# ChantalMP/RaDialog

Measured on AMD Instinct MI355X. Metric: reports_per_sec (448px CXR encode + 160-tok prefill + 256-tok greedy decode), higher is better.
Workload: dtype bf16; 1 GPU; configs[1]: per-GPU batch 1 BioViL-T(ResNet-50)+Q-Former encode 448px, Vicuna-7B prefill T=160, 256-token greedy decode (LoRA r=8 un-merged, hipGraph ; per_gpu_batch=1, global_batch=1, prompt_len=160, parallelism=dp1

## Files before the change

### include/rdx_hooks.h

```cpp
#ifndef RDX_HOOKS_H
#define RDX_HOOKS_H
#include "rdx.h"
#ifdef __cplusplus
extern "C" {
#endif

int rdx_attn_trace(rdx_ctx* ctx, int layer, long long* host);
int rdx_quant_test(rdx_ctx* ctx, const void* X, int M, int K, int groups, int mode, const void* norm_w, float eps, void* out8, float* scales);
int rdx_gemv_trace(rdx_ctx* ctx, int what, int layer, long long* host, int max_tiles);

int rdx_gemm_test(rdx_ctx* ctx, const void* X, const float* W, const float* bias, const void* resid, void* out, int M, int N,
                  int K, int epi, const void* norm_w, float eps, int force);

int rdx_kernel_bench(rdx_ctx* ctx, int rows, int N, int K, int H, int ksize, int stride, int epi, int iters, float* ms_host,
                     long long* trace_host , int trace_wgs);

int rdx_conv_test(rdx_ctx* ctx, const void* X, const float* W, const float* bias, const void* resid, void* out, int B, int H, int Cin, int Cout,
                  int ksize, int stride, int epi, int path, int iters, float* ms_host);

int rdx_l2_bench(rdx_ctx* ctx, int mode, long long bytes_per_wg, int shared, int reps, int wgs, float* gbps_host);

int rdx_logits_test(rdx_ctx* ctx, const void* X, const float* W, int M, int N, int n_valid, int K, void* out_logits,
                    int32_t* argmax_host, int fp8);

#ifdef __cplusplus
}
#endif
#endif
```

### radialog_amd/_lib.py

```python
from __future__ import annotations

import ctypes as C
import os

import torch

HERE = os.path.dirname(os.path.abspath(__file__))
LIB_PATH = os.environ.get("RDX_LIB_PATH") or os.path.join(HERE, "librdx.so")
HOOKS_PATH = os.environ.get("RDX_HOOKS_PATH") or os.path.join(HERE, "librdx_hooks.so")

RDX_DTYPE_F16, RDX_DTYPE_BF16 = 0, 1
RDX_W_GEMM, RDX_W_TENSOR, RDX_W_F32, RDX_W_GEMM_FP8 = 0, 1, 2, 3
RDX_SRC_F32, RDX_SRC_F16, RDX_SRC_BF16 = 0, 1, 2


class RdxLibraryError(RuntimeError):
    pass


class RdxError(RuntimeError):
    pass


class RdxLogitsRules(C.Structure):
    _fields_ = [("repetition_penalty", C.c_float), ("no_repeat_ngram_size", C.c_int), ("min_new_tokens", C.c_int)]


class RdxConfig(C.Structure):
    _fields_ = [
        ("dtype", C.c_int),
        ("vocab", C.c_int), ("hidden", C.c_int), ("inter", C.c_int), ("layers", C.c_int), ("heads", C.c_int),
        ("max_pos", C.c_int),
        ("rms_eps", C.c_float),
        ("lora_r", C.c_int), ("lora_scale", C.c_float),
        ("qformer_dim", C.c_int),
        ("q_hidden", C.c_int), ("q_layers", C.c_int), ("q_heads", C.c_int), ("q_inter", C.c_int),
        ("q_enc_width", C.c_int), ("q_nquery", C.c_int), ("q_cross_freq", C.c_int),
        ("q_ln_eps", C.c_float),
        ("v_img", C.c_int), ("v_stem", C.c_int), ("v_planes", C.c_int * 4), ("v_blocks", C.c_int * 4),
        ("v_b2v", C.c_int), ("v_proj", C.c_int),
        ("v_ln_eps", C.c_float),
        ("max_batch", C.c_int), ("max_len", C.c_int),
        ("enable_vision", C.c_int), ("enable_llama", C.c_int),
        ("enable_cls", C.c_int), ("cls_hidden", C.c_int), ("cls_classes", C.c_int), ("cls_pool", C.c_int),
    ]


_P = C.c_void_p
SYMBOLS = {
    "rdx_create": (C.c_int, [C.POINTER(_P), C.c_int, C.POINTER(RdxConfig)]),
    "rdx_destroy": (None, [_P]),
    "rdx_last_error": (C.c_char_p, [_P]),
    "rdx_build_hash": (C.c_char_p, []),
    "rdx_sync": (C.c_int, [_P]),
    "rdx_stream": (_P, [_P]),
    "rdx_set_weight": (C.c_int, [_P, C.c_char_p, _P, C.c_int64, C.c_int64, C.c_int]),
    "rdx_set_weight_typed": (C.c_int, [_P, C.c_char_p, _P, C.c_int, C.c_int64, C.c_int64, C.c_int]),
    "rdx_finalize_weights": (C.c_int, [_P]),
    "rdx_transform_image": (C.c_int, [_P, _P, C.c_int, C.c_int, C.c_int, C.c_int, _P]),
    "rdx_encode_image": (C.c_int, [_P, _P, C.c_int, _P, _P]),
    "rdx_encode_image2": (C.c_int, [_P, _P, _P, C.c_int, _P, _P]),
    "rdx_classify_findings": (C.c_int, [_P, _P, C.c_int, _P]),
    "rdx_generate": (C.c_int, [_P, _P, _P, C.c_int, C.c_int, _P, C.c_int, C.c_int, C.c_int, _P, _P,
                               C.POINTER(C.c_int), C.c_int]),
    "rdx_prefill": (C.c_int, [_P, _P, _P, C.c_int, C.c_int, _P, C.c_int, C.c_int, C.c_int, _P, _P]),
    "rdx_decode_step": (C.c_int, [_P, _P]),
    "rdx_decode_step_ids": (C.c_int, [_P, _P, _P]),
    "rdx_set_logits_rules": (C.c_int, [_P, C.POINTER(RdxLogitsRules)]),
    "rdx_prefill_append": (C.c_int, [_P, _P, C.c_int, C.c_int, C.c_int, C.c_int, C.c_int, C.c_int, _P, _P]),
    "rdx_generate_append": (C.c_int, [_P, _P, C.c_int, C.c_int, C.c_int, C.c_int, C.c_int, C.c_int, _P, _P,
                                      C.POINTER(C.c_int), C.c_int]),
    "rdx_beam_search": (C.c_int, [_P, _P, _P, C.c_int, C.c_int, C.c_int, _P, C.c_int, C.c_int, C.c_int, C.c_float, C.c_int, _P, _P, _P, _P,
                                  C.POINTER(C.c_int)]),
    "rdx_comm_unique_id": (C.c_int, [_P]),
    "rdx_comm_init": (C.c_int, [_P, _P, C.c_int, C.c_int]),
    "rdx_allgather_tokens": (C.c_int, [_P, _P, _P, C.c_int, C.c_int]),
    "rdx_comm_world": (C.c_int, [_P]),
    "rdx_kv_read": (C.c_int, [_P, C.c_int, C.c_int, _P]),
    "rdx_hidden_read": (C.c_int, [_P, _P]),
    "rdx_time": (C.c_int, [_P, C.c_int, C.c_int, C.POINTER(C.c_float)]),
    "rdx_set_option": (C.c_int, [_P, C.c_char_p, C.c_int]),
}

HOOK_SYMBOLS = {
    "rdx_attn_trace": (C.c_int, [_P, C.c_int, _P]),
    "rdx_quant_test": (C.c_int, [_P, _P, C.c_int, C.c_int, C.c_int, C.c_int, _P, C.c_float, _P, _P]),
    "rdx_gemv_trace": (C.c_int, [_P, C.c_int, C.c_int, _P, C.c_int]),
    "rdx_gemm_test": (C.c_int, [_P, _P, _P, _P, _P, _P, C.c_int, C.c_int, C.c_int, C.c_int, _P, C.c_float, C.c_int]),
    "rdx_kernel_bench": (C.c_int, [_P, C.c_int, C.c_int, C.c_int, C.c_int, C.c_int, C.c_int, C.c_int, C.c_int, C.POINTER(C.c_float), _P, C.c_int]),
    "rdx_conv_test": (C.c_int, [_P, _P, _P, _P, _P, _P, C.c_int, C.c_int, C.c_int, C.c_int, C.c_int, C.c_int, C.c_int, C.c_int, C.c_int, C.POINTER(C.c_float)]),
    "rdx_l2_bench": (C.c_int, [_P, C.c_int, C.c_longlong, C.c_int, C.c_int, C.c_int, C.POINTER(C.c_float)]),
    "rdx_logits_test": (C.c_int, [_P, _P, _P, C.c_int, C.c_int, C.c_int, C.c_int, _P, _P, C.c_int]),
}

ENC_HOOK_SYMBOLS = {
    "rdx_stem_test": (C.c_int, [_P, _P, _P, _P, _P, C.c_int, C.c_int, C.c_int, C.c_int]),
    "rdx_norm_test": (C.c_int, [_P, C.c_int, _P, _P, _P, _P, _P, _P, C.c_int, C.c_int, C.c_longlong, C.c_longlong, C.c_int, C.c_int, C.c_float]),
    "rdx_attn_test": (C.c_int, [_P, _P, _P, _P, _P, _P, C.c_int, C.c_int, C.c_int, C.c_int, C.c_int, C.c_int, _P, C.c_longlong, C.c_int, C.c_int]),
}

_F = C.c_float
DEC_HOOK_SYMBOLS = {
    "rdx_xstat16_test": (C.c_int, [_P, _P, _P, _F, _P, C.c_int, C.c_int, C.c_int, C.c_int, _P, C.c_int, C.c_int, _P]),
    "rdx_xrow16_test": (C.c_int, [_P, _P, C.c_int, _P, _P, C.c_int, C.c_int, C.c_int, _P, C.c_int]),
    "rdx_xstat_blk_test": (C.c_int, [_P, _P, _P, _F, _P, _P, C.c_int, C.c_int, C.c_int, C.c_int, _P, C.c_int, C.c_int, _P, _P]),
    "rdx_xsplit_blk_test": (C.c_int, [_P, _P, _P, _P, _P, _F, C.c_int, C.c_int, _P, _P]),
    "rdx_xstat_blk8_test": (C.c_int, [_P, _P, _P, _F, _P, C.c_int, C.c_int, C.c_int, C.c_int, _P, C.c_int, C.c_int, _P, _P, _P]),
    "rdx_xsplit_blk8_test": (C.c_int, [_P, _P, _P, _P, _P, _F, C.c_int, C.c_int, C.c_int, _P, _P, _P]),
    "rdx_rmsnorm_test": (C.c_int, [_P, _P, _P, _F, C.c_int, C.c_int, C.c_int, C.c_int, _P, C.c_int, _P, C.c_longlong, _P, C.c_int]),
    "rdx_select_test": (C.c_int, [_P, _P, C.c_int, C.c_int, _P, _P, _P, C.c_int, C.POINTER(RdxLogitsRules), C.c_int, _P]),
}
ALL_HOOK_SYMBOLS = {**HOOK_SYMBOLS, **ENC_HOOK_SYMBOLS, **DEC_HOOK_SYMBOLS}

_lib = None
_hooks = None


def hooks_enabled() -> bool:
    return os.environ.get("RDX_DEBUG_HOOKS", "0") not in ("", "0")


def _missing_hook(name):
    def raiser(*_a, **_k):
        raise RdxLibraryError(f"{name} is a kernel-test hook of librdx_hooks.so (include/rdx_hooks.h, rdx_enc_hooks.h, rdx_dec_hooks.h), not part of the product library: "
                              "set RDX_DEBUG_HOOKS=1 before radialog_amd is loaded (tests/conftest.py and the tools/ scripts do)")
    return raiser


def load_hooks(lib):
    global _hooks
    if not hooks_enabled():
        for name in ALL_HOOK_SYMBOLS:
            setattr(lib, name, _missing_hook(name))
        return
    src = lib
    if not hasattr(lib, next(iter(HOOK_SYMBOLS))):
        if os.environ.get("RDX_LIB_PATH") and os.path.realpath(LIB_PATH) != os.path.realpath(os.path.join(HERE, "librdx.so")):
            raise RdxLibraryError(f"RDX_DEBUG_HOOKS is set, but RDX_LIB_PATH={LIB_PATH} does not link the hooks in and {HOOKS_PATH} would load a "
                                  "second librdx.so next to it: build the alternative library with api_debug.hip (tools/sanitize_host.sh does)")
        if not os.path.exists(HOOKS_PATH):
            raise RdxLibraryError(f"RDX_DEBUG_HOOKS is set but {HOOKS_PATH} is missing: build it with `python -m radialog_amd.build`")
        try:
            src = C.CDLL(HOOKS_PATH, mode=C.RTLD_GLOBAL)
        except OSError as e:
            raise RdxLibraryError(f"cannot load {HOOKS_PATH}: {e}") from e
        _hooks = src
    for name, (res, args) in ALL_HOOK_SYMBOLS.items():
        try:
            fn = getattr(src, name)
        except AttributeError as e:
            raise RdxLibraryError(f"{HOOKS_PATH} does not export {name}") from e
        fn.restype = res
        fn.argtypes = args
        if src is not lib:
            setattr(lib, name, fn)


def load():
    global _lib
    if _lib is not None:
        return _lib
    if not os.path.exists(LIB_PATH):
        raise RdxLibraryError(
            f"{LIB_PATH} not found: build it with `python -m radialog_amd.build` (hipcc, gfx950). "
            "There is no CPU fallback for the RaDialog hot path.")
    try:
        lib = C.CDLL(LIB_PATH, mode=C.RTLD_GLOBAL if hooks_enabled() else C.RTLD_LOCAL)
    except OSError as e:
        raise RdxLibraryError(f"cannot load {LIB_PATH}: {e}") from e
    for name, (res, args) in SYMBOLS.items():
        try:
            fn = getattr(lib, name)
        except AttributeError as e:
            raise RdxLibraryError(f"{LIB_PATH} does not export {name}") from e
        fn.restype = res
        fn.argtypes = args
    check_build_hash(lib)
    load_hooks(lib)
    _lib = lib
    return lib


def build_hash() -> str:
    return load().rdx_build_hash().decode()


def check_build_hash(lib):
    from . import build as _b
    try:
        want = _b.source_hash()
    except OSError:
        return
    got = lib.rdx_build_hash().decode()
    if got != want:
        msg = (f"{LIB_PATH} was built from sources with hash {got}, the tree's radialog_amd/csrc hashes to {want}: the library is stale -- "
               "rebuild it with `python -m radialog_amd.build`")
        if os.environ.get("RDX_ALLOW_STALE_LIB", "0") not in ("", "0"):
            import warnings
            warnings.warn(msg)
        else:
            raise RdxLibraryError(msg)


def check(ctx, rc: int, what: str):
    if rc != 0:
        msg = load().rdx_last_error(ctx)
        raise RdxError(f"{what} failed ({rc}): {msg.decode() if msg else '?'}")
```

### radialog_amd/csrc/api.hip

```cpp
#include "rdx_ctx.h"

static std::string g_create_err;

int fail(rdx_ctx* c, int code, const char* fmt, ...) {
    char buf[512];
    va_list ap;
    va_start(ap, fmt);
    vsnprintf(buf, sizeof(buf), fmt, ap);
    va_end(ap);
    if (c) c->err = buf; else g_create_err = buf;
    return code;
}

const char* create_error() { return g_create_err.c_str(); }

int dalloc(rdx_ctx* c, void** p, size_t bytes) {
    if (bytes == 0) bytes = 16;
    hipError_t e = hipMalloc(p, bytes);
    if (e != hipSuccess) return fail(c, -3, "hipMalloc(%zu bytes) failed: %s", bytes, hipGetErrorString(e));
    c->allocs.push_back(*p);
    return 0;
}

extern "C" int rdx_create(rdx_ctx** out, int device_id, const rdx_config* cfg) {
    if (!out || !cfg) return fail(nullptr, -1, "rdx_create: null argument");
    if (cfg->dtype != RDX_DTYPE_F16 && cfg->dtype != RDX_DTYPE_BF16) return fail(nullptr, -1, "rdx_create: bad dtype %d", cfg->dtype);
    int ndev = 0;
    hipError_t e = hipGetDeviceCount(&ndev);
    if (e != hipSuccess || ndev <= 0) return fail(nullptr, -2, "rdx_create: no HIP device (%s)", hipGetErrorString(e));
    if (device_id < 0 || device_id >= ndev) return fail(nullptr, -1, "rdx_create: device %d out of range (%d devices)", device_id, ndev);
    if (cfg->enable_llama) {
        if (cfg->hidden % cfg->heads || cfg->hidden / cfg->heads != 128)
            return fail(nullptr, -1, "rdx_create: Llama head_dim must be 128 (hidden %d / heads %d)", cfg->hidden, cfg->heads);
        if (cfg->hidden % 32 || cfg->inter % 32 || cfg->inter % 8 || cfg->qformer_dim % 32)
            return fail(nullptr, -1, "rdx_create: hidden/inter/qformer_dim must be multiples of 32");
        if (cfg->max_len % 32 || cfg->max_len <= 0 || cfg->max_len > 1536)
            return fail(nullptr, -1, "rdx_create: max_len must be a multiple of 32 in (0, 1536]");
        if (cfg->max_batch <= 0 || cfg->max_batch > RDX_MAX_ROWS) return fail(nullptr, -1, "rdx_create: max_batch must be in [1, %d]", RDX_MAX_ROWS);
        if (cfg->lora_r != 0 && cfg->lora_r != 8) return fail(nullptr, -1, "rdx_create: lora_r must be 0 or 8");
    }
    if (cfg->enable_vision) {
        if (cfg->q_hidden / cfg->q_heads != 64 || cfg->q_hidden % cfg->q_heads)
            return fail(nullptr, -1, "rdx_create: Q-Former head_dim must be 64");
    }
    if (cfg->enable_vision || cfg->enable_cls) {
        if (cfg->v_img % 4 || cfg->v_img < 32) return fail(nullptr, -1, "rdx_create: image size must be a multiple of 4, >= 32");
    }
    if (cfg->enable_cls) {
        if (cfg->enable_vision) return fail(nullptr, -1, "rdx_create: a classifier context has enable_vision = 0 (its projector differs)");
        if (cfg->cls_pool <= 0 || cfg->cls_hidden % 32 || cfg->cls_classes <= 0 || cfg->cls_classes > 16)
            return fail(nullptr, -1, "rdx_create: classifier needs pool > 0, hidden %% 32 == 0, 1..16 classes");
    }
    rdx_ctx* c = new rdx_ctx();
    c->cfg = *cfg;
    c->device = device_id;
    if (const char* e = getenv("RDX_FUSE_AO")) c->fuse_attn_oproj = atoi(e) != 0;
    if (const char* e = getenv("RDX_CHAIN")) c->chain_mlp = atoi(e) != 0;
    if (hipSetDevice(device_id) != hipSuccess || hipStreamCreateWithFlags(&c->stream, hipStreamNonBlocking) != hipSuccess) {
        delete c;
        return fail(nullptr, -2, "rdx_create: cannot create stream on device %d", device_id);
    }
    { const char* e = getenv("RDX_FLASH_MIN"); if (e) c->flash_min = atoi(e); }
    { const char* e = getenv("RDX_XS16"); if (e) c->xs16 = atoi(e) != 0; }
    { const char* e = getenv("RDX_PBLK"); if (e) c->prompt_blk = atoi(e) != 0; }
    { const char* e = getenv("RDX_BLK_DOWN"); c->blk_down = !(e && atoi(e) == 0); }
    { const char* e = getenv("RDX_PCONV_KSPLIT"); c->pconv_noks = e && atoi(e) == 0; }
    { const char* e = getenv("RDX_PCONV"); c->trunk_packed = !(e && atoi(e) == 0); }
    if (hipMalloc(&c->zero16, 64) == hipSuccess) { hipMemset(c->zero16, 0, 64); c->allocs.push_back(c->zero16); } else c->zero16 = nullptr;
    c->gemm_ws_floats = (size_t)16 << 20;
    if (hipMalloc((void**)&c->gemm_ws, c->gemm_ws_floats * sizeof(float)) != hipSuccess) { c->gemm_ws = nullptr; c->gemm_ws_floats = 0; }
    else c->allocs.push_back(c->gemm_ws);
    *out = c;
    return 0;
}

void rdx_comm_release(rdx_ctx* c);

extern "C" void rdx_destroy(rdx_ctx* c) {
    if (!c) return;
    hipSetDevice(c->device);
    hipStreamSynchronize(c->stream);
    rdx_comm_release(c);
    if (c->graph) hipGraphExecDestroy(c->graph);
    for (void* p : c->allocs) hipFree(p);
    hipStreamDestroy(c->stream);
    delete c;
}

extern "C" const char* rdx_last_error(rdx_ctx* c) { return c ? c->err.c_str() : g_create_err.c_str(); }

#ifndef RDX_BUILD_HASH
#define RDX_BUILD_HASH "unstamped"
#endif
extern "C" const char* rdx_build_hash(void) { return RDX_BUILD_HASH; }

extern "C" int rdx_sync(rdx_ctx* c) {
    if (!c) return -1;
    HIPCHK(c, hipStreamSynchronize(c->stream));
    HIPCHK(c, hipGetLastError());
    return 0;
}

extern "C" void* rdx_stream(rdx_ctx* c) { return c ? (void*)c->stream : nullptr; }

extern "C" int rdx_set_weight(rdx_ctx* c, const char* name, const float* data, int64_t rows, int64_t cols, int kind) {
    if (!c || !name || !data) return fail(c, -1, "rdx_set_weight: null argument");
    if (c->finalized) return fail(c, -1, "rdx_set_weight(%s): weights already finalized", name);
    if (rows <= 0 || cols <= 0) return fail(c, -1, "rdx_set_weight(%s): bad shape [%lld,%lld]", name, (long long)rows, (long long)cols);
    HIPCHK(c, hipSetDevice(c->device));
    const std::string key(name);
    if (kind == RDX_W_GEMM) {
        if (cols % 32) return fail(c, -1, "rdx_set_weight(%s): GEMM K=%lld must be a multiple of 32", name, (long long)cols);
        if (c->gemm.count(key)) return fail(c, -1, "rdx_set_weight(%s): duplicate", name);
        GemmW w;
        w.N = (int)rows; w.K = (int)cols; w.Npad = (int)((rows + 15) / 16 * 16);
        ALLOC(c, w.w, (size_t)w.Npad * w.K * esz(c));
        launch_pack_weight(c->cfg.dtype, data, w.w, w.N, w.K, w.Npad, nullptr, c->stream);
        c->gemm[key] = w;
    } else if (kind == RDX_W_GEMM_FP8) {
        if (cols % 64) return fail(c, -1, "rdx_set_weight(%s): fp8 GEMM K=%lld must be a multiple of 64", name, (long long)cols);
        if (c->gemm.count(key)) return fail(c, -1, "rdx_set_weight(%s): duplicate", name);
        GemmW w;
        w.N = (int)rows; w.K = (int)cols; w.Npad = (int)((rows + 15) / 16 * 16);
        ALLOC(c, w.w8, (size_t)w.Npad * w.K);
        ALLOC(c, w.scale, (size_t)w.Npad * sizeof(float));
        launch_pack_weight_fp8(c->cfg.dtype, data, w.w8, w.scale, nullptr, w.N, w.K, w.Npad, c->stream);
        c->gemm[key] = w;
    } else if (kind == RDX_W_TENSOR) {
        if (c->tens.count(key)) return fail(c, -1, "rdx_set_weight(%s): duplicate", name);
        RawW r; r.rows = rows; r.cols = cols;
        ALLOC(c, r.p, (size_t)rows * cols * esz(c) + 16);
        launch_from_f32(c->cfg.dtype, data, r.p, (size_t)rows * cols, c->stream);
        c->tens[key] = r;
    } else if (kind == RDX_W_F32) {
        if (c->f32.count(key)) return fail(c, -1, "rdx_set_weight(%s): duplicate", name);
        RawW r; r.rows = rows; r.cols = cols;
        ALLOC(c, r.p, (size_t)rows * cols * sizeof(float));
        HIPCHK(c, hipMemcpyAsync(r.p, data, (size_t)rows * cols * sizeof(float), hipMemcpyDeviceToDevice, c->stream));
        c->f32[key] = r;
    } else {
        return fail(c, -1, "rdx_set_weight(%s): unknown kind %d", name, kind);
    }
    HIPCHK(c, hipStreamSynchronize(c->stream));
    HIPCHK(c, hipGetLastError());
    return 0;
}

extern "C" int rdx_set_weight_typed(rdx_ctx* c, const char* name, const void* data, int src_dtype, int64_t rows, int64_t cols, int kind) {
    if (src_dtype == RDX_SRC_F32) return rdx_set_weight(c, name, (const float*)data, rows, cols, kind);
    if (!c || !name || !data) return fail(c, -1, "rdx_set_weight_typed: null argument");
    if (src_dtype != RDX_SRC_F16 && src_dtype != RDX_SRC_BF16) return fail(c, -1, "rdx_set_weight_typed(%s): unknown source dtype %d", name, src_dtype);
    if (rows <= 0 || cols <= 0) return fail(c, -1, "rdx_set_weight_typed(%s): bad shape [%lld,%lld]", name, (long long)rows, (long long)cols);
    HIPCHK(c, hipSetDevice(c->device));
    float* wide = nullptr;
    const size_t n = (size_t)rows * cols;
    hipError_t e = hipMalloc((void**)&wide, n * sizeof(float));
    if (e != hipSuccess) return fail(c, -3, "rdx_set_weight_typed(%s): hipMalloc(%zu bytes) failed: %s", name, n * sizeof(float), hipGetErrorString(e));
    launch_to_f32(src_dtype == RDX_SRC_F16 ? DT_F16 : DT_BF16, data, wide, n, c->stream);
    const int rc = rdx_set_weight(c, name, wide, rows, cols, kind);
    hipFree(wide);
    return rc;
}

namespace {
struct Resolver {
    rdx_ctx* c;
    int rc = 0;
    GemmW g(const std::string& n, int N, int K) {
        auto it = c->gemm.find(n);
        if (it == c->gemm.end()) { if (!rc) rc = fail(c, -4, "missing GEMM weight '%s'", n.c_str()); return GemmW(); }
        if (it->second.N != N || it->second.K != K) {
            if (!rc) rc = fail(c, -4, "weight '%s' has shape [%d,%d], expected [%d,%d]", n.c_str(), it->second.N, it->second.K, N, K);
        }
        return it->second;
    }
    const void* t(const std::string& n, int64_t elems) {
        auto it = c->tens.find(n);
        if (it == c->tens.end()) { if (!rc) rc = fail(c, -4, "missing tensor '%s'", n.c_str()); return nullptr; }
        if (it->second.rows * it->second.cols != elems) { if (!rc) rc = fail(c, -4, "tensor '%s' has %lld elements, expected %lld", n.c_str(), (long long)(it->second.rows * it->second.cols), (long long)elems); }
        return it->second.p;
    }
    const float* f(const std::string& n, int64_t elems) {
        auto it = c->f32.find(n);
        if (it == c->f32.end()) { if (!rc) rc = fail(c, -4, "missing fp32 tensor '%s'", n.c_str()); return nullptr; }
        if (it->second.rows * it->second.cols != elems) { if (!rc) rc = fail(c, -4, "fp32 tensor '%s' has %lld elements, expected %lld", n.c_str(), (long long)(it->second.rows * it->second.cols), (long long)elems); }
        return (const float*)it->second.p;
    }
};
std::string S(const char* fmt, ...) {
    char buf[128];
    va_list ap; va_start(ap, fmt); vsnprintf(buf, sizeof(buf), fmt, ap); va_end(ap);
    return buf;
}
}

extern "C" int rdx_finalize_weights(rdx_ctx* c) {
    if (!c) return -1;
    if (c->finalized) return fail(c, -1, "rdx_finalize_weights: already finalized");
    HIPCHK(c, hipSetDevice(c->device));
    const rdx_config& f = c->cfg;
    Resolver R{c};
    if (f.enable_llama) {
        const int H = f.hidden, I = f.inter, r2 = 2 * f.lora_r;
        c->embed = R.t("embed", (int64_t)f.vocab * H);
        c->final_norm = R.t("final_norm", H);
        c->rope_cos = R.t("rope.cos", (int64_t)f.max_pos * 128);
        c->rope_sin = R.t("rope.sin", (int64_t)f.max_pos * 128);
        c->lm_head = R.g("lm_head", f.vocab, H);
        c->img_proj_w = R.g("img_proj.w", H, f.qformer_dim);
        c->img_proj_b = R.f("img_proj.b", H);
        c->ll.resize(f.layers);
        for (int l = 0; l < f.layers; ++l) {
            LlamaLayer& L = c->ll[l];
            L.attn_norm = R.t(S("l%d.attn_norm", l), H);
            L.mlp_norm = R.t(S("l%d.mlp_norm", l), H);
            L.wqkv = R.g(S("l%d.wqkv", l), 3 * H + r2, H);
            L.wo = R.g(S("l%d.wo", l), H, H);
            L.wgu = R.g(S("l%d.wgu", l), 2 * I, H);
            L.wdown = R.g(S("l%d.wdown", l), H, I);
            L.lora_bq = L.lora_bv = nullptr;
            if (f.lora_r) {
                L.lora_bq = R.t(S("l%d.lora_bq", l), (int64_t)H * f.lora_r);
                L.lora_bv = R.t(S("l%d.lora_bv", l), (int64_t)H * f.lora_r);
            }
        }
        if (R.rc) return R.rc;
        c->ld.hidden = H; c->ld.heads = f.heads; c->ld.head_dim = 128; c->ld.qkv_ld = c->ll[0].wqkv.Npad;
        c->ld.lora_r = f.lora_r; c->ld.lora_scale = f.lora_scale; c->ld.max_len = f.max_len; c->ld.max_pos = f.max_pos;
        c->ld.k_perm = (getenv("RDX_KPERM") ? atoi(getenv("RDX_KPERM")) : (f.max_batch * f.heads <= 256)) ? 1 : 0;
        const int B = f.max_batch;
        c->kv_layer_elems = (size_t)B * f.heads * f.max_len * 128;
        ALLOC(c, c->kcache, c->kv_layer_elems * f.layers * 2);
        ALLOC(c, c->vcache, c->kv_layer_elems * f.layers * 2);
        HIPCHK(c, hipMemset(c->kcache, 0, c->kv_layer_elems * f.layers * 2));
        HIPCHK(c, hipMemset(c->vcache, 0, c->kv_layer_elems * f.layers * 2));
        ALLOC(c, c->key_mask, (size_t)B * f.max_len);
        HIPCHK(c, hipMemset(c->key_mask, 0, (size_t)B * f.max_len));
        ALLOC(c, c->d_img_pos, B * sizeof(int)); ALLOC(c, c->d_pos, B * sizeof(int)); ALLOC(c, c->d_slot, B * sizeof(int));
        ALLOC(c, c->d_step, B * sizeof(int)); ALLOC(c, c->d_unf, B * sizeof(int));
        ALLOC(c, c->d_ctr, ((size_t)f.layers * 256 + chain_ctr_ints(f.layers)) * sizeof(int)); ALLOC(c, c->d_err, sizeof(int));
        HIPCHK(c, hipMemset(c->d_ctr, 0, ((size_t)f.layers * 256 + chain_ctr_ints(f.layers)) * sizeof(int)));
        c->d_cctr = c->d_ctr + (size_t)f.layers * 256;
        HIPCHK(c, hipMemset(c->d_err, 0, sizeof(int)));
        {
            std::vector<ChainLayer> cl(f.layers);
            for (int l = 0; l < f.layers; ++l) {
                const LlamaLayer& L = c->ll[l];
                cl[l] = ChainLayer{L.wqkv.w, L.wdown.w, L.attn_norm, L.wqkv.w8, L.wdown.w8, L.wqkv.scale, L.wdown.scale};
            }
            ALLOC(c, c->d_clayers, cl.size() * sizeof(ChainLayer));
            HIPCHK(c, hipMemcpy(c->d_clayers, cl.data(), cl.size() * sizeof(ChainLayer), hipMemcpyHostToDevice));
        }
        ALLOC(c, c->d_cur_rope, (size_t)B * 256 * 2);
        ALLOC(c, c->d_pos_ids, (size_t)B * f.max_len * sizeof(int));
        c->n_vtiles = c->lm_head.Npad / 16;
        ALLOC(c, c->part_val, (size_t)B * c->n_vtiles * sizeof(float));
        ALLOC(c, c->part_idx, (size_t)B * c->n_vtiles * sizeof(int));
        const int Bp = B > 2 ? (B + 31) / 32 * 32 : B;
        ALLOC(c, c->dx, (size_t)B * H * 2); ALLOC(c, c->dxn, (size_t)Bp * H * 2);
        if (B > 2) ALLOC(c, c->kslab, (size_t)4 * Bp * H * sizeof(float));
        ALLOC(c, c->dqkv, (size_t)B * c->ld.qkv_ld * 2);
        ALLOC(c, c->dxs, (size_t)std::max(32, Bp) * sizeof(float));
        ALLOC(c, c->datt, (size_t)Bp * H * 2); ALLOC(c, c->dgu, (size_t)Bp * I * 2);
        ALLOC(c, c->pqe, (size_t)B * 32 * f.qformer_dim * 2); ALLOC(c, c->pimg, (size_t)B * 32 * H * 2);
        if (B > 32 && !blk64_ok(c, B))
            return fail(c, -1, "rdx_finalize_weights: max_batch %d > 32 needs the Vicuna-7B widths (hidden 4096, inter 11008: the row-block decode family, model-dtype "
                               "or fp8 weights); this model (hidden %d, inter %d) holds at most 32 rows per context", B, H, I);
    }
    if (f.enable_vision) {
        const int H = f.q_hidden, I = f.q_inter;
        c->q_query_ln = R.t("q.query_ln", (int64_t)f.q_nquery * H);
        c->n_cross = 0;
        c->ql.resize(f.q_layers);
        for (int l = 0; l < f.q_layers; ++l) {
            QLayer& L = c->ql[l];
            L.s_wqkv = R.g(S("q%d.self.wqkv", l), 3 * H, H); L.s_bqkv = R.f(S("q%d.self.bqkv", l), 3 * H);
            L.s_wo = R.g(S("q%d.self.wo", l), H, H); L.s_bo = R.f(S("q%d.self.bo", l), H);
            L.s_g = R.f(S("q%d.self.ln_g", l), H); L.s_b = R.f(S("q%d.self.ln_b", l), H);
            L.cross_idx = -1;
            if (l % f.q_cross_freq == 0) {
                L.cross_idx = c->n_cross++;
                L.c_wq = R.g(S("q%d.cross.wq", l), H, H); L.c_bq = R.f(S("q%d.cross.bq", l), H);
                L.c_wo = R.g(S("q%d.cross.wo", l), H, H); L.c_bo = R.f(S("q%d.cross.bo", l), H);
                L.c_g = R.f(S("q%d.cross.ln_g", l), H); L.c_b = R.f(S("q%d.cross.ln_b", l), H);
            }
            L.w1 = R.g(S("q%d.ffn.w1", l), I, H); L.b1 = R.f(S("q%d.ffn.b1", l), I);
            L.w2 = R.g(S("q%d.ffn.w2", l), H, I); L.b2 = R.f(S("q%d.ffn.b2", l), H);
            L.f_g = R.f(S("q%d.ffn.ln_g", l), H); L.f_b = R.f(S("q%d.ffn.ln_b", l), H);
        }
        c->q_wkv = R.g("q.cross.wkv", c->n_cross * 2 * H, f.q_enc_width);
        c->q_bkv = R.f("q.cross.bkv", (int64_t)c->n_cross * 2 * H);
    }
    if (f.enable_vision || f.enable_cls) {
        c->v_conv1 = R.g("v.conv1.w", f.v_stem, 7 * 8 * 4); c->v_conv1_b = R.f("v.conv1.b", f.v_stem);
        int cin = f.v_stem;
        for (int li = 0; li < 4; ++li) {
            for (int b = 0; b < f.v_blocks[li]; ++b) {
                VBlock vb;
                vb.planes = f.v_planes[li];
                vb.stride = (b == 0 && li > 0) ? 2 : 1;
                vb.has_ds = (b == 0);
                const std::string p = S("v.l%d.%d.", li + 1, b);
                vb.c1 = R.g(p + "c1.w", vb.planes, cin); vb.b1 = R.f(p + "c1.b", vb.planes);
                vb.c2 = R.g(p + "c2.w", vb.planes, 9 * vb.planes); vb.b2 = R.f(p + "c2.b", vb.planes);
                vb.c3 = R.g(p + "c3.w", 4 * vb.planes, vb.planes); vb.b3 = R.f(p + "c3.b", 4 * vb.planes);
                vb.bds = nullptr;
                if (vb.has_ds) { vb.ds = R.g(p + "ds.w", 4 * vb.planes, cin); vb.bds = R.f(p + "ds.b", 4 * vb.planes); }
                cin = 4 * vb.planes;
                c->vb.push_back(vb);
            }
        }
        c->v_b2v = R.g("v.b2v.w", f.v_b2v, cin);
        c->v_p1 = R.g("v.proj1.w", f.v_proj, f.v_b2v); c->v_p1_b = R.f("v.proj1.b", f.v_proj);
        c->v_p2 = R.g("v.proj2.w", f.v_proj, f.v_proj); c->v_p2_b = R.f("v.proj2.b", f.v_proj);
    }
    if (f.enable_cls) {
        const int gp = v_grid(f) / f.cls_pool;
        if (gp <= 0 || (f.v_proj * gp * gp) % 32) return fail(c, -1, "classifier: pooled feature width %d must be a positive multiple of 32", f.v_proj * gp * gp);
        c->cls_fc1 = R.g("cls.fc1.w", f.cls_hidden, f.v_proj * gp * gp); c->cls_fc1_b = R.f("cls.fc1.b", f.cls_hidden);
        c->cls_fc2 = R.g("cls.fc2.w", f.cls_classes, f.cls_hidden); c->cls_fc2_b = R.f("cls.fc2.b", f.cls_classes);
    }
    if (f.enable_vision) {
        c->v_ln_g = R.f("v.ln.g", f.v_proj); c->v_ln_b = R.f("v.ln.b", f.v_proj);
        if (f.q_enc_width != f.v_proj) return fail(c, -1, "q_enc_width %d != v_proj %d", f.q_enc_width, f.v_proj);
        if (c->tens.count("v.pool.emb")) {
            const int Cv = f.v_b2v, Pn = v_grid(f) * v_grid(f);
            if (Cv % 32) return fail(c, -1, "ViT pooler needs b2v %% 32 == 0");
            c->pool_emb = R.t("v.pool.emb", (int64_t)2 * Pn * Cv);
            c->pool_ng = R.f("v.pool.norm_g", Cv); c->pool_nb = R.f("v.pool.norm_b", Cv);
            c->v_p1f = R.g("v.proj1f.w", f.v_proj, 2 * Cv); c->v_p1f_b = R.f("v.proj1f.b", f.v_proj);
            for (int i = 0; c->gemm.count(S("v.pool.%d.wqkv", i)); ++i) {
                PoolBlock pb;
                const std::string p = S("v.pool.%d.", i);
                pb.n1_g = R.f(p + "n1_g", Cv); pb.n1_b = R.f(p + "n1_b", Cv); pb.n2_g = R.f(p + "n2_g", Cv); pb.n2_b = R.f(p + "n2_b", Cv);
                pb.wqkv = R.g(p + "wqkv", 3 * Cv, Cv);
                pb.wo = R.g(p + "wo", Cv, Cv); pb.bo = R.f(p + "bo", Cv);
                pb.w1 = R.g(p + "w1", Cv, Cv); pb.b1 = R.f(p + "b1", Cv);
                pb.w2 = R.g(p + "w2", Cv, Cv); pb.b2 = R.f(p + "b2", Cv);
                c->pool.push_back(pb);
            }
        }
    }
    if (R.rc) return R.rc;
    c->finalized = true;
    return 0;
}

extern "C" int rdx_set_option(rdx_ctx* c, const char* name, int value) {
    if (!c || !name) return -1;
    if (!strcmp(name, "flash_min")) { c->flash_min = value; return 0; }
    if (!strcmp(name, "pconv")) { c->trunk_packed = value != 0; return 0; }
    if (!strcmp(name, "prompt_blk")) { c->prompt_blk = value != 0; return 0; }
    if (!strcmp(name, "xs16")) {
        c->xs16 = value != 0;
        if (c->graph) { hipGraphExecDestroy(c->graph); c->graph = nullptr; c->gkey = GraphKey(); }
        return 0;
    }
    return fail(c, -1, "rdx_set_option: unknown option '%s'", name);
}
```

### radialog_amd/csrc/api_debug.hip

```cpp
#include "rdx_ctx.h"
#include "../../include/rdx_hooks.h"
#include "../../include/rdx_enc_hooks.h"

extern "C" int rdx_attn_trace(rdx_ctx* c, int layer, long long* host) {
    if (!c || !c->finalized || c->cur_B <= 0 || !host) return fail(c, -1, "rdx_attn_trace: run a prefill first");
    HIPCHK(c, hipSetDevice(c->device));
    long long* dtr = nullptr;
    HIPCHK(c, hipMalloc(&dtr, 8 * sizeof(long long)));
    HIPCHK(c, hipMemsetAsync(dtr, 0, 8 * sizeof(long long), c->stream));
    DecAttnArgs at = dec_attn_args(c, layer);
    at.trace = dtr;
    launch_decode_attention(c->cfg.dtype, at, c->cur_B, c->stream);
    hipError_t e = hipStreamSynchronize(c->stream);
    if (e == hipSuccess) e = hipMemcpy(host, dtr, 8 * sizeof(long long), hipMemcpyDeviceToHost);
    hipFree(dtr);
    HIPCHK(c, e);
    return 0;
}

extern "C" int rdx_quant_test(rdx_ctx* c, const void* X, int M, int K, int groups, int mode, const void* norm_w, float eps, void* out8, float* scales) {
    if (!c || !X || !out8 || !scales || M <= 0 || K <= 0 || K % 128) return fail(c, -1, "rdx_quant_test: bad arguments (K %% 128 == 0)");
    if (mode == 0 && (groups < 1 || groups > 4)) return fail(c, -1, "rdx_quant_test: 1..4 K groups");
    if (mode == 1 && !norm_w) return fail(c, -1, "rdx_quant_test: mode 1 needs the norm weight");
    HIPCHK(c, hipSetDevice(c->device));
    if (mode == 0) launch_quant_rows(c->cfg.dtype, X, K, out8, scales, M, K, groups, c->stream);
    else run_rmsnorm(c, NormArgs{const_cast<void*>(X), norm_w, out8, scales, M, K, eps, ACT_ROWS_E4M3, 0, nullptr, 0});
    HIPCHK(c, hipStreamSynchronize(c->stream));
    HIPCHK(c, hipGetLastError());
    return take_unsupported(c);
}

extern "C" int rdx_gemv_trace(rdx_ctx* c, int what, int layer, long long* host, int max_tiles) {
    if (!c || !c->finalized || c->cur_B <= 0 || !host) return fail(c, -1, "rdx_gemv_trace: run a prefill first");
    HIPCHK(c, hipSetDevice(c->device));
    const rdx_config& f = c->cfg;
    const int H = f.hidden, B = c->cur_B;
    if (what == 7) {
        if (layer < 0 || layer >= f.layers) return fail(c, -1, "rdx_gemv_trace(7): layer %d of %d", layer, f.layers);
        if (c->cur_T + c->cur_steps + 1 > f.max_len || c->cur_T + c->cur_steps + 1 > f.max_pos)
            return fail(c, -1, "rdx_gemv_trace(7): no room for one more decode step in the KV cache");
        const int wgs = H / 16 + ((c->ll[0].wqkv.Npad + 15) / 16 + 3) / 4;
        if (wgs > max_tiles) return fail(c, -1, "rdx_gemv_trace(7): need room for %d workgroups", wgs);
        long long* dtr = nullptr;
        const size_t bytes = (size_t)max_tiles * 8 * sizeof(long long);
        HIPCHK(c, hipMalloc(&dtr, bytes));
        HIPCHK(c, hipMemsetAsync(dtr, 0, bytes, c->stream));
        c->chain_trace = dtr; c->chain_trace_layer = layer;
        const bool chained = decode_step_launch(c, nullptr, nullptr, 0);
        c->chain_trace = nullptr; c->chain_trace_layer = -1;
        c->cur_steps = std::max(c->cur_steps + 1, c->cur_max_new);
        hipError_t e = hipStreamSynchronize(c->stream);
        if (e == hipSuccess) e = hipMemcpy(host, dtr, bytes, hipMemcpyDeviceToHost);
        hipFree(dtr);
        HIPCHK(c, e);
        if (!chained) return fail(c, -1, "rdx_gemv_trace(7): the chained down -> QKV launch is not active in this configuration (batch > 2, RDX_CHAIN=0)");
        return 0;
    }
    const LlamaLayer& L = c->ll[layer];
    long long* dtr = nullptr;
    const size_t bytes = (size_t)max_tiles * 8 * sizeof(long long);
    HIPCHK(c, hipMalloc(&dtr, bytes));
    HIPCHK(c, hipMemsetAsync(dtr, 0, bytes, c->stream));
    GemmArgs a = unit_args(c, &L, what == 1 ? UNIT_GATE_UP : what == 2 ? UNIT_QKV : UNIT_DOWN, B);
    if (what != 1 && what != 2) { a.out = c->dqkv; a.resid = nullptr; a.ldr = 0; }
    if ((a.N + 15) / 16 > max_tiles) { hipFree(dtr); return fail(c, -1, "rdx_gemv_trace: need room for %d tiles", (a.N + 15) / 16); }
    a.trace = dtr;
    skinny(c, a, what == 1 ? EPI_SILU_MUL : EPI_NONE);
    hipError_t e = hipStreamSynchronize(c->stream);
    if (e == hipSuccess) e = hipMemcpy(host, dtr, bytes, hipMemcpyDeviceToHost);
    hipFree(dtr);
    HIPCHK(c, e);
    return 0;
}


extern "C" int rdx_kernel_bench(rdx_ctx* c, int rows, int N, int K, int H, int ksize, int stride, int epi, int iters, float* ms_host,
                                long long* trace_host, int trace_wgs) {
    if (!c || !ms_host || iters <= 0 || rows <= 0) return fail(c, -1, "rdx_kernel_bench: bad arguments");
    HIPCHK(c, hipSetDevice(c->device));
    const int Kg = ksize ? ksize * ksize * K : K;
    if (Kg % 32 || N % 16) return fail(c, -1, "rdx_kernel_bench: need K %% 32 == 0 and N %% 16 == 0");
    const int Ho = ksize ? (H + 2 * (ksize / 2) - ksize) / stride + 1 : 0;
    const size_t M = ksize ? (size_t)rows * Ho * Ho : (size_t)rows, Min = ksize ? (size_t)rows * H * H : (size_t)rows;
    char* buf = nullptr;
    const bool kb_wstat = getenv("RDX_KB_WSTAT") && atoi(getenv("RDX_KB_WSTAT")) && !ksize;
    const size_t xb = ((Min + 15) & ~(size_t)15) * K * 2 + 64, wb = (size_t)N * Kg * 2, ob = M * N * 2 + 64, bb = (size_t)N * 4;
    HIPCHK(c, hipMalloc((void**)&buf, xb + wb + 2 * ob + bb));
    HIPCHK(c, hipMemsetAsync(buf, 0, xb + wb + 2 * ob + bb, c->stream));
    GemmW w; w.N = N; w.K = Kg; w.Npad = N; w.w = buf + xb;
    void *out = buf + xb + wb, *res = buf + xb + wb + ob;
    const float* bias = (const float*)(buf + xb + wb + 2 * ob);
    const bool need_res = epi == EPI_RESID || epi == EPI_RESID_RELU;
    hipEvent_t e0, e1;
    HIPCHK(c, hipEventCreate(&e0)); HIPCHK(c, hipEventCreate(&e1));
    struct WsScope { rdx_ctx* c; ~WsScope() { c->ws_ok = false; } } ws_scope{c};
    c->ws_ok = true;
    long long* dtr = nullptr;
    if (trace_host && trace_wgs > 0) { HIPCHK(c, hipMalloc((void**)&dtr, (size_t)trace_wgs * 8 * sizeof(long long))); HIPCHK(c, hipMemset(dtr, 0, (size_t)trace_wgs * 64)); }
    auto once = [&]() {
        if (ksize) conv_gemm(c, buf, w, bias, need_res ? res : nullptr, out, rows, H, H, K, ksize, ksize, stride, ksize / 2, Ho, Ho, epi);
        else {
            GemmArgs a = gargs(buf, K, w, bias, out, N, (int)M); a.resid = need_res ? res : nullptr; a.ldr = N; a.trace = dtr;
            if (kb_wstat) {
                a.xpacked = ACT_TILES32; a.mtiles = (int)((M + 15) / 16); a.bias = nullptr;
                if (wstat_supported(a, epi)) { launch_wstat(c->cfg.dtype, a, epi, c->stream); return; }
            }
            run_gemm(c, a, epi);
        }
    };
    once();
    HIPCHK(c, hipEventRecord(e0, c->stream));
    for (int i = 0; i < iters; ++i) once();
    HIPCHK(c, hipEventRecord(e1, c->stream));
    HIPCHK(c, hipEventSynchronize(e1));
    float ms = 0.f;
    HIPCHK(c, hipEventElapsedTime(&ms, e0, e1));
    hipEventDestroy(e0); hipEventDestroy(e1);
    if (dtr) { hipMemcpy(trace_host, dtr, (size_t)trace_wgs * 64, hipMemcpyDeviceToHost); hipFree(dtr); }
    hipFree(buf);
    HIPCHK(c, hipGetLastError());
    *ms_host = ms / (float)iters;
    return 0;
}

extern "C" int rdx_conv_test(rdx_ctx* c, const void* X, const float* W, const float* bias, const void* resid, void* out, int B, int H, int Cin,
                             int Cout, int ksize, int stride, int epi, int path, int iters, float* ms_host) {
    if (!c || !X || !W || !out || B <= 0) return fail(c, -1, "rdx_conv_test: bad arguments");
    if (!(ksize == 1 || ksize == 3)) return fail(c, -1, "rdx_conv_test: ksize 1 or 3");
    HIPCHK(c, hipSetDevice(c->device));
    const int K = ksize * ksize * Cin, Ho = (H + 2 * (ksize / 2) - ksize) / stride + 1;
    const int M = B * Ho * Ho, Min = B * H * H, dt = c->cfg.dtype;
    if (K % 32 || Cout % 16) return fail(c, -1, "rdx_conv_test: need K %% 32 == 0 and Cout %% 16 == 0");
    const bool need_res = epi == EPI_RESID || epi == EPI_RESID_RELU;
    if (need_res && !resid) return fail(c, -1, "rdx_conv_test: epilogue needs a residual");
    const int mt_in = (Min + 15) / 16, mt_out = (M + 15) / 16;
    const size_t wb = (size_t)Cout * K * 2, xpb = (size_t)mt_in * 16 * Cin * 2, opb = (size_t)mt_out * 16 * Cout * 2;
    char* buf = nullptr;
    HIPCHK(c, hipMalloc((void**)&buf, wb + xpb + 2 * opb + 256));
    GemmW w; w.N = Cout; w.K = K; w.Npad = Cout; w.w = buf;
    launch_pack_weight(dt, W, buf, Cout, K, Cout, nullptr, c->stream);
    char *xp = buf + wb, *rp = xp + xpb, *op = rp + opb;
    struct WsScope { rdx_ctx* c; ~WsScope() { c->ws_ok = false; } } ws_scope{c};
    c->ws_ok = true;
    PConvArgs pa;
    memset(&pa, 0, sizeof(pa));
    if (path) {
        launch_pack_rows(dt, X, Cin, xp, Min, Cin, c->stream);
        if (need_res) launch_pack_rows(dt, resid, Cout, rp, M, Cout, c->stream);
        pa.X = xp; pa.W = buf; pa.bias = bias; pa.resid = need_res ? rp : nullptr; pa.out = path == 2 ? out : (void*)op; pa.zero16 = c->zero16;
        pa.Hin = H; pa.Win = H; pa.Cin = Cin; pa.Hout = Ho; pa.Wout = Ho; pa.N = Cout; pa.M = M; pa.mt_in = mt_in; pa.mt_out = mt_out; pa.ldo = Cout;
        pa.no_ksplit = c->pconv_noks;
        if (const char* e = getenv("RDX_PCONV_TILE")) {
            if (e[0] >= '1' && e[0] <= '8' && e[1] == 'x' && (e[2] == '2' || e[2] == '4')) {
                pa.tile_m = e[0] - '0'; pa.tile_n = e[2] - '0';
                if (e[3] == 'k' && (e[4] == '4' || e[4] == '8')) pa.tile_k = e[4] - '0';
            }
        }
        if (!c->zero16 || !pconv_supported(pa, ksize * ksize, stride, epi)) { hipFree(buf); return fail(c, -1, "rdx_conv_test: shape not supported by pconv"); }
    }
    bool refused = false;
    auto once = [&]() {
        if (path) { if (!launch_pconv(dt, pa, ksize * ksize, stride, epi, path == 2, c->stream)) refused = true; }
        else conv_gemm(c, X, w, bias, need_res ? resid : nullptr, out, B, H, H, Cin, ksize, ksize, stride, ksize / 2, Ho, Ho, epi);
    };
    once();
    if (refused) { hipStreamSynchronize(c->stream); hipFree(buf); return fail(c, -1, "rdx_conv_test: pconv refused the tiling (1 x 1 stride-1 with different input / output row tilings)"); }
    if (ms_host && iters > 0) {
        hipEvent_t e0, e1;
        hipEventCreate(&e0); hipEventCreate(&e1);
        hipEventRecord(e0, c->stream);
        for (int i = 0; i < iters; ++i) once();
        hipEventRecord(e1, c->stream);
        hipEventSynchronize(e1);
        float ms = 0.f;
        hipEventElapsedTime(&ms, e0, e1);
        hipEventDestroy(e0); hipEventDestroy(e1);
        *ms_host = ms / (float)iters;
    }
    if (path == 1) launch_unpack_rows(dt, op, out, Cout, M, Cout, c->stream);
    hipError_t e = hipStreamSynchronize(c->stream);
    hipFree(buf);
    HIPCHK(c, e);
    HIPCHK(c, hipGetLastError());
    return 0;
}

extern "C" int rdx_l2_bench(rdx_ctx* c, int mode, long long bytes_per_wg, int shared, int reps, int wgs, float* gbps_host) {
    if (!c || !gbps_host || bytes_per_wg < 65536 || wgs <= 0 || reps <= 0) return fail(c, -1, "rdx_l2_bench: bad arguments");
    HIPCHK(c, hipSetDevice(c->device));
    char* buf = nullptr;
    const size_t total = shared ? (size_t)bytes_per_wg : (size_t)bytes_per_wg * wgs;
    HIPCHK(c, hipMalloc((void**)&buf, total + 64));
    HIPCHK(c, hipMemsetAsync(buf, 1, total + 64, c->stream));
    hipEvent_t e0, e1;
    HIPCHK(c, hipEventCreate(&e0)); HIPCHK(c, hipEventCreate(&e1));
    launch_l2_bench(mode, buf, (size_t)bytes_per_wg, shared, 1, wgs, (unsigned*)(buf + total), c->stream);
    HIPCHK(c, hipEventRecord(e0, c->stream));
    launch_l2_bench(mode, buf, (size_t)bytes_per_wg, shared, reps, wgs, (unsigned*)(buf + total), c->stream);
    HIPCHK(c, hipEventRecord(e1, c->stream));
    HIPCHK(c, hipEventSynchronize(e1));
    float ms = 0.f;
    HIPCHK(c, hipEventElapsedTime(&ms, e0, e1));
    hipEventDestroy(e0); hipEventDestroy(e1);
    hipFree(buf);
    HIPCHK(c, hipGetLastError());
    *gbps_host = (float)((double)bytes_per_wg * wgs * reps / (ms * 1e-3) / 1e9);
    return 0;
}

static int fp8_block_for_test(rdx_ctx* c, GemmArgs& a, int epi, char** tmp) {
    *tmp = nullptr;
    if (!(a.W8 && a.wscale) || a.M < xs_min_rows()) return 0;
    GemmArgs t = a; t.norm_w = nullptr;
    if (!xstat32_supported(t, epi)) return 0;
    HIPCHK(c, hipMalloc((void**)tmp, (size_t)32 * a.K + 32 * sizeof(float)));
    float* xs = (float*)(*tmp + (size_t)32 * a.K);
    run_rmsnorm(c, NormArgs{const_cast<void*>(a.X), a.norm_w, *tmp, xs, a.M, a.K, a.eps, ACT_BLK64_E4M3, 0, nullptr, 0});
    a.X = *tmp; a.ldx = a.K; a.xpacked = ACT_BLK64_E4M3; a.xscale = xs; a.xgroups = 1; a.norm_w = nullptr;
    return 0;
}

extern "C" int rdx_gemm_test(rdx_ctx* c, const void* X, const float* W, const float* bias, const void* resid, void* out,
                             int M, int N, int K, int epi, const void* norm_w, float eps, int force) {
    if (!c || !X || !W || !out) return fail(c, -1, "rdx_gemm_test: null argument");
    if (K % 32 || N % 16) return fail(c, -1, "rdx_gemm_test: need K %% 32 == 0 and N %% 16 == 0");
    HIPCHK(c, hipSetDevice(c->device));
    GemmW w;
    w.N = N; w.K = K; w.Npad = N;
    void* wp = nullptr;
    HIPCHK(c, hipMalloc(&wp, (size_t)N * K * 2 + ((force == 4 || (force >= 9 && force <= 11)) ? (size_t)N * K + (size_t)N * 4 : 0)));
    w.w = wp;
    if (force >= 9 && force <= 11) {
        const int G = force == 9 ? 1 : (force == 10 ? 2 : 4);
        if (K % 64 || (norm_w && G != 1)) { hipFree(wp); return fail(c, -1, "rdx_gemm_test: gemm8 needs K %% 64 == 0 (and one K group behind an RMSNorm)"); }
        w.w = nullptr; w.w8 = (char*)wp + (size_t)N * K * 2; w.scale = (float*)((char*)wp + (size_t)N * K * 3);
        launch_pack_weight_fp8(c->cfg.dtype, W, w.w8, w.scale, nullptr, N, K, N, c->stream);
        char* tmp = nullptr;
        if (hipMalloc((void**)&tmp, (size_t)M * K + (size_t)M * 4 * sizeof(float)) != hipSuccess) { hipFree(wp); return fail(c, -2, "rdx_gemm_test: out of device memory"); }
        float* xs = (float*)(tmp + (size_t)M * K);
        if (norm_w) run_rmsnorm(c, NormArgs{const_cast<void*>(X), norm_w, tmp, xs, M, K, eps, ACT_ROWS_E4M3, 0, nullptr, 0});
        else launch_quant_rows(c->cfg.dtype, X, K, tmp, xs, M, K, G, c->stream);
        GemmArgs a = gargs(tmp, K, w, nullptr, out, epi == EPI_SILU_MUL ? N / 2 : N, M);
        a.resid = resid; a.ldr = N; a.xscale = xs; a.xgroups = G;
        int rc = 0;
        if (!gemm8_supported(a, epi)) rc = fail(c, -1, "rdx_gemm_test: shape / epilogue not supported by gemm8");
        else launch_gemm8(c->cfg.dtype, a, epi, c->stream);
        hipError_t se = hipStreamSynchronize(c->stream);
        hipFree(wp); hipFree(tmp);
        if (rc) return rc;
        if (int urc = take_unsupported(c)) return urc;
        HIPCHK(c, se);
        HIPCHK(c, hipGetLastError());
        return 0;
    }
    if (force == 4) {
        if (K % 64) { hipFree(wp); return fail(c, -1, "rdx_gemm_test: fp8 needs K %% 64 == 0"); }
        w.w = nullptr;
        w.w8 = (char*)wp + (size_t)N * K * 2;
        w.scale = (float*)((char*)wp + (size_t)N * K * 3);
        launch_pack_weight_fp8(c->cfg.dtype, W, w.w8, w.scale, nullptr, N, K, N, c->stream);
        force = 1;
    } else
    launch_pack_weight(c->cfg.dtype, W, wp, N, K, N, nullptr, c->stream);
    GemmArgs a = gargs(X, K, w, bias, out, epi == EPI_SILU_MUL ? N / 2 : N, M);
    a.resid = resid; a.ldr = N;
    a.norm_w = norm_w; a.eps = eps;
    void* xn = nullptr;
    bool split8 = false;
    if (force == 6) {
        if (K % 64) { hipFree(wp); return fail(c, -1, "rdx_gemm_test: fp8 needs K %% 64 == 0"); }
        hipFree(wp);
        HIPCHK(c, hipMalloc(&wp, (size_t)N * K * 3 + (size_t)N * 4));
        w.w = nullptr; w.w8 = (char*)wp + (size_t)N * K * 2; w.scale = (float*)((char*)wp + (size_t)N * K * 3);
        launch_pack_weight_fp8(c->cfg.dtype, W, w.w8, w.scale, nullptr, N, K, N, c->stream);
        a = gargs(X, K, w, bias, out, N, M);
        a.resid = resid; a.ldr = N; a.eps = eps;
        split8 = true; force = 5;
    }
    if (force == 5) {
        if (epi != EPI_RESID || !resid || M <= 16 || M > 32) { hipFree(wp); return fail(c, -1, "rdx_gemm_test: force 5 needs epi 3 and 16 < M <= 32"); }
        char* tmp = nullptr;
        const size_t xb = (size_t)32 * K * 2, sb = (size_t)4 * 32 * N * 4;
        if (hipMalloc((void**)&tmp, 2 * xb + sb) != hipSuccess) { hipFree(wp); return fail(c, -2, "rdx_gemm_test: out of device memory"); }
        a.X = tmp; a.xpacked = split8 ? ACT_BLK64 : ACT_BLK32; a.norm_w = nullptr;
        run_rmsnorm(c, NormArgs{const_cast<void*>(X), nullptr, tmp, nullptr, M, K, eps, a.xpacked, 0, nullptr, 0});
        const int kg = xsplit32_groups(a);
        if (!kg) { hipFree(wp); hipFree(tmp); return fail(c, -1, "rdx_gemm_test: shape not supported by xsplit32_k"); }
        launch_xsplit32(c->cfg.dtype, a, (float*)(tmp + 2 * xb), c->stream);
        HIPCHK(c, hipMemcpyAsync(out, resid, (size_t)M * N * 2, hipMemcpyDeviceToDevice, c->stream));
        run_rmsnorm(c, NormArgs{out, nullptr, tmp + xb, nullptr, M, N, eps, ACT_ROWS, 0, (const float*)(tmp + 2 * xb), kg});
        HIPCHK(c, hipStreamSynchronize(c->stream));
        HIPCHK(c, hipGetLastError());
        hipFree(wp); hipFree(tmp);
        return take_unsupported(c);
    }
    if (force == 8) {
        const int mtl = (M + 15) / 16;
        char* tmp = nullptr;
        HIPCHK(c, hipMalloc((void**)&tmp, (size_t)mtl * 16 * K * 2));
        run_rmsnorm(c, NormArgs{const_cast<void*>(X), norm_w, tmp, nullptr, M, K, eps, ACT_TILES32, mtl, nullptr, 0});
        a.X = tmp; a.xpacked = ACT_TILES32; a.mtiles = mtl; a.norm_w = nullptr;
        if (!wstat_supported(a, epi)) { hipFree(wp); hipFree(tmp); return fail(c, -1, "rdx_gemm_test: shape not supported by wstat_k"); }
        launch_wstat(c->cfg.dtype, a, epi, c->stream);
        HIPCHK(c, hipStreamSynchronize(c->stream));
        HIPCHK(c, hipGetLastError());
        hipFree(wp); hipFree(tmp);
        return take_unsupported(c);
    }
    if (force == 7) {
        ConvGeom cg0;
        memset(&cg0, 0, sizeof(cg0));
        a.norm_w = nullptr;
        if (!c->zero16 || a.K % 64 || a.N % 16) { hipFree(wp); return fail(c, -1, "rdx_gemm_test: shape not supported by wsgemm_k"); }
        launch_wsgemm(c->cfg.dtype, a, cg0, epi, c->zero16, c->stream);
        HIPCHK(c, hipStreamSynchronize(c->stream));
        HIPCHK(c, hipGetLastError());
        hipFree(wp);
        return 0;
    }
    const bool use_skinny = force == 1 || (force == 0 && M <= 32);
    if (use_skinny) {
        if (M > 32) { hipFree(wp); return fail(c, -1, "rdx_gemm_test: skinny path needs M <= 32"); }
        void* keep = c->dxn;
        char* blk = nullptr;
        int brc = fp8_block_for_test(c, a, epi, &blk);
        if (brc) { hipFree(wp); return brc; }
        if (a.norm_w && !skinny_fits_lds(M, K)) {
            HIPCHK(c, hipMalloc(&xn, (size_t)32 * K * 2));
            c->dxn = xn;
        }
        skinny(c, a, epi == EPI_RESID_RELU ? EPI_RESID : epi);
        c->dxn = keep;
        hipError_t se = hipStreamSynchronize(c->stream);
        if (blk) hipFree(blk);
        if (int urc = take_unsupported(c)) { hipFree(wp); if (xn) hipFree(xn); return urc; }
        HIPCHK(c, se);
    } else {
        if (a.norm_w) {
            HIPCHK(c, hipMalloc(&xn, (size_t)M * K * 2));
            run_rmsnorm(c, NormArgs{const_cast<void*>(X), norm_w, xn, nullptr, M, K, eps, ACT_ROWS, 0, nullptr, 0});
            a.X = xn; a.norm_w = nullptr;
        }
        ConvGeom cg;
        memset(&cg, 0, sizeof(cg));
        if (force == 3 || (force == 0 && gemm_dma_supported(a))) {
            if (!gemm_dma_supported(a)) { hipFree(wp); if (xn) hipFree(xn); return fail(c, -1, "rdx_gemm_test: shape not supported by gemm_dma_k"); }
            launch_gemm_dma(c->cfg.dtype, a, epi, c->gemm_ws, c->gemm_ws_floats, c->stream);
        } else {
            launch_tiled_gemm(c->cfg.dtype, a, cg, epi, c->stream);
        }
    }
    HIPCHK(c, hipStreamSynchronize(c->stream));
    HIPCHK(c, hipGetLastError());
    hipFree(wp);
    if (xn) hipFree(xn);
    return take_unsupported(c);
}

// ... 176 lines not shown
```

### radialog_amd/csrc/api_llama.hip

```cpp
#include <cmath>

#include "rdx_ctx.h"

static int ensure_prefill_ws(rdx_ctx* c, size_t rows) {
    rows = (rows + 15) & ~(size_t)15;
    if (rows <= c->prefill_rows) return 0;
    const rdx_config& f = c->cfg;
    HIPCHK(c, hipStreamSynchronize(c->stream));
    c->prefill_rows = 0;
    dfree(c, c->px); dfree(c, c->pxn); dfree(c, c->pqkv); dfree(c, c->pq); dfree(c, c->patt); dfree(c, c->pgu); dfree(c, c->pxq); dfree(c, c->pxs); dfree(c, c->pslab);
    if (fp8_weights(c->ll[0].wqkv)) {
        ALLOC(c, c->pxq, rows * (size_t)std::max(f.hidden, f.inter));
        ALLOC(c, c->pxs, rows * 4 * sizeof(float));
    }
    ALLOC(c, c->px, rows * f.hidden * 2); ALLOC(c, c->pxn, rows * f.hidden * 2);
    ALLOC(c, c->pslab, (size_t)4 * std::min<size_t>(rows, 192) * f.hidden * sizeof(float));
    ALLOC(c, c->pqkv, rows * c->ld.qkv_ld * 2); ALLOC(c, c->pq, rows * f.hidden * 2);
    ALLOC(c, c->patt, rows * f.hidden * 2); ALLOC(c, c->pgu, rows * f.inter * 2);
    c->prefill_rows = rows;
    return 0;
}

static const char* const k_need_blk = "more than 32 decoder rows need hidden 4096 / inter 11008 (the row-block family)";

static void lm_head_and_greedy(rdx_ctx* c, const void* x, int B, void* logits, const int* out_step, long step_stride,
                               int advance) {
    const rdx_config& f = c->cfg;
    if (c->rules_on && !logits) { logits = c->rule_logits; out_step = nullptr; }
    auto lm = [&](GemmArgs a) { a.X = x; a.out = logits; a.out_step = out_step; a.out_step_stride = step_stride; return a; };
    switch (decode_family(c, B)) {
    case DEC_UNSUPPORTED: c->unsupported = k_need_blk; return;
    case DEC_BLK: launch_xstat_blk(f.dtype, norm_in_front(c, lm(blk_unit(c, nullptr, UNIT_LM_HEAD, B))), EPI_LOGITS, c->stream); break;
    case DEC_BLK8: launch_xstat_blk8(f.dtype, norm_in_front(c, lm(blk8_unit(c, nullptr, UNIT_LM_HEAD, B))), EPI_LOGITS, c->stream); break;
    case DEC_XS16:
        if (x == c->dx) { launch_xstat16(f.dtype, lm(xs16_unit(c, nullptr, UNIT_LM_HEAD, B)), EPI_LOGITS, c->stream); break; }
        [[fallthrough]];
    default: skinny(c, lm(unit_args(c, nullptr, UNIT_LM_HEAD, B)), EPI_LOGITS);
    }
    StepTail t = {};
    t.eos_id = c->cur_eos; t.pad_id = c->cur_pad; t.max_new = c->cur_max_new; t.out_tokens = c->cur_tokens; t.unfinished = c->d_unf;
    t.pos = advance ? c->d_pos : nullptr; t.slot_b = advance ? c->d_slot : nullptr; t.step_b = c->d_step;
    t.embed = c->embed; t.vocab = f.vocab; t.x_next = c->dx; t.H = f.hidden; t.pos_ro = c->d_pos; t.cos_t = c->rope_cos; t.sin_t = c->rope_sin;
    t.cur_rope = c->d_cur_rope;
    t.ctr_zero = (c->fuse_attn_oproj || c->chain_mlp) ? c->d_ctr : nullptr;
    t.n_zero = f.layers * 256 + (c->chain_mlp ? (int)chain_ctr_ints(f.layers) : 0);
    if (!c->rules_on) { launch_greedy_step(f.dtype, c->part_val, c->part_idx, c->n_vtiles, B, t, c->stream); return; }
    t.hist = c->d_hist; t.hist_len = c->d_hist_len; t.hist_ld = f.max_len;
    SelectArgs sa;
    sa.logits = logits; sa.step_stride = out_step ? step_stride : 0; sa.n_gen = c->d_step;
    sa.penalty = c->rules.repetition_penalty; sa.ngram = c->rules.no_repeat_ngram_size; sa.min_new = c->rules.min_new_tokens; sa.sel_out = nullptr;
    launch_select_step(f.dtype, sa, t, B, c->stream);
}

static const rdx_logits_rules k_neutral_rules = {1.0f, 0, 0};

extern "C" int rdx_set_logits_rules(rdx_ctx* c, const rdx_logits_rules* rules) {
    if (!c) return -1;
    const rdx_logits_rules r = rules ? *rules : k_neutral_rules;
    if (!(r.repetition_penalty > 0.f) || !std::isfinite(r.repetition_penalty))
        return fail(c, -1, "rdx_set_logits_rules: repetition_penalty must be a finite float > 0 (1.0 = off)");
    if (r.no_repeat_ngram_size < 0) return fail(c, -1, "rdx_set_logits_rules: no_repeat_ngram_size %d is negative (0 = off)", r.no_repeat_ngram_size);
    if (r.min_new_tokens < 0) return fail(c, -1, "rdx_set_logits_rules: min_new_tokens %d is negative (0 = off)", r.min_new_tokens);
    const bool on = r.repetition_penalty != 1.0f || r.no_repeat_ngram_size != 0 || r.min_new_tokens != 0;
    if (on) {
        if (!c->finalized || !c->cfg.enable_llama) return fail(c, -1, "rdx_set_logits_rules: llama weights not finalized");
        const rdx_config& f = c->cfg;
        if (!select_step_supported(f.vocab)) return fail(c, -1, "rdx_set_logits_rules: vocab %d exceeds the LDS bitmaps of select_step_k", f.vocab);
        HIPCHK(c, hipSetDevice(c->device));
        if (!c->d_hist) ALLOC(c, c->d_hist, (size_t)f.max_batch * f.max_len * sizeof(int));
        if (!c->rule_logits) ALLOC(c, c->rule_logits, (size_t)f.max_batch * f.vocab * 2);
        if (!c->d_hist_len) {
            ALLOC(c, c->d_hist_len, (size_t)f.max_batch * sizeof(int));
            HIPCHK(c, hipMemset(c->d_hist_len, 0, (size_t)f.max_batch * sizeof(int)));
        }
    }
    if (on != c->rules_on) c->hist_ready = false;
    c->rules = on ? r : k_neutral_rules;
    c->rules_on = on;
    return 0;
}

static int rules_need_prefill(rdx_ctx* c, const char* who) {
    if (c->rules_on && !c->hist_ready) return fail(c, -1, "%s: logits rules were set after the last prefill; run a new prefill first", who);
    return 0;
}

int prefill_impl(rdx_ctx* c, const int32_t* ids, const int32_t* mask, int B, int T, const float* qformer_embs, int keep,
                        int max_new, int eos_id, int pad_id, int32_t* out_tokens, void* logits) {
    if (!c) return -1;
    if (!c->finalized || !c->cfg.enable_llama) return fail(c, -1, "rdx_prefill: llama weights not finalized");
    const rdx_config& f = c->cfg;
    if (!ids || !out_tokens || B <= 0 || B > f.max_batch) return fail(c, -1, "rdx_prefill: batch %d outside [1, %d]", B, f.max_batch);
    if (T <= 0 || keep + T + max_new > f.max_len) return fail(c, -1, "rdx_prefill: T (%d) + max_new (%d) exceeds max_len %d", keep + T, max_new, f.max_len);
    if (keep + T + max_new > f.max_pos) return fail(c, -1, "rdx_prefill: sequence exceeds max_position_embeddings %d", f.max_pos);
    if (qformer_embs && T < 32) return fail(c, -1, "rdx_prefill: image splice needs T >= 32");
    HIPCHK(c, hipSetDevice(c->device));
    if (keep > 0) {
        if (B != c->cur_B) return fail(c, -1, "rdx_prefill_append: batch %d differs from the cached conversation's %d", B, c->cur_B);
        std::vector<int> slot(B);
        HIPCHK(c, hipMemcpyAsync(slot.data(), c->d_slot, B * sizeof(int), hipMemcpyDeviceToHost, c->stream));
        HIPCHK(c, hipStreamSynchronize(c->stream));
        for (int b = 0; b < B; ++b)
            if (keep > slot[b]) return fail(c, -1, "rdx_prefill_append: keep_len %d exceeds the %d cached positions of row %d", keep, slot[b], b);
    }
    const size_t M = (size_t)B * T;
    int rc = ensure_prefill_ws(c, M);
    if (rc) return rc;
    const int dt = f.dtype, H = f.hidden;
    hipStream_t s = c->stream;
    c->cur_B = B; c->cur_T = keep + T; c->cur_max_new = max_new; c->cur_eos = eos_id; c->cur_pad = pad_id; c->cur_tokens = out_tokens;
    c->cur_steps = 1;

    if (keep > 0) {
        launch_prep_append(B, T, keep, c->d_img_pos, c->d_pos_ids, c->d_pos, c->d_slot, c->d_step, c->d_unf, s);
        qformer_embs = nullptr;
    } else {
        launch_prep_prompt(ids, mask, B, T, 32000, pad_id, c->d_img_pos, c->d_pos_ids, c->key_mask, f.max_len, c->d_pos, c->d_slot,
                           c->d_step, c->d_unf, s);
    }
    c->hist_ready = c->rules_on;
    if (c->rules_on) launch_hist_init(ids, B, T, c->d_hist, c->d_hist_len, f.max_len, s);
    if (qformer_embs) {
        launch_from_f32(dt, qformer_embs, c->pqe, (size_t)B * 32 * f.qformer_dim, s);
        GemmArgs a = gargs(c->pqe, f.qformer_dim, c->img_proj_w, c->img_proj_b, c->pimg, H, B * 32);
        run_gemm(c, a, EPI_NONE);
    }
    launch_embed_splice(dt, ids, c->d_img_pos, c->embed, f.vocab, c->pimg, 32, c->px, B, T, H, qformer_embs ? 1 : 0, s);

    const bool fp8 = fp8_weights(c->ll[0].wqkv);
    auto prompt_norm = [&](const void* w, void* out, ActLayout layout, int mtiles, int pend) {
        run_rmsnorm(c, NormArgs{c->px, w, out, c->pxs, (int)M, H, f.rms_eps, layout, mtiles, pend ? c->pslab : nullptr, pend});
    };
    if (B > 32 && !blk64_ok(c, B)) return fail(c, -8, "rdx_prefill: more than 32 rows per context need the Vicuna-7B widths (hidden 4096, inter 11008: the row-block decode family)");
    if (fp8) {
        for (int l = 0; l < f.layers; ++l) {
            const LlamaLayer& L = c->ll[l];
            void* kc = kv_ptr(c, c->kcache, l);
            void* vc = kv_ptr(c, c->vcache, l);
            auto g8 = [&](const GemmW& W, int K, int groups, void* out, int ldo, const void* resid, int epi) {
                GemmArgs a = gargs(c->pxq, K, W, nullptr, out, ldo, (int)M);
                a.N = W.Npad; a.xscale = c->pxs; a.xgroups = groups; a.resid = resid; a.ldr = H;
                if (!gemm8_supported(a, epi)) { c->unsupported = "fp8 weights: prefill projection shape not supported by gemm8 (N % 16, K % 64)"; return; }
                launch_gemm8(dt, a, epi, s);
            };
            prompt_norm(L.attn_norm, c->pxq, ACT_ROWS_E4M3, 0, 0);
            g8(L.wqkv, H, 1, c->pqkv, c->ld.qkv_ld, nullptr, EPI_NONE);
            launch_rope_kv_prefill(dt, c->ld, c->pqkv, L.lora_bq, L.lora_bv, c->rope_cos, c->rope_sin, c->d_pos_ids, c->pq, kc, vc, B, T, keep, s);
            launch_attention(dt, 128, prefill_attn_args(c, B, T, keep, l), s);
            launch_quant_rows(dt, c->patt, H, c->pxq, c->pxs, (int)M, H, 2, s);
            g8(L.wo, H, 2, c->px, H, c->px, EPI_RESID);
            prompt_norm(L.mlp_norm, c->pxq, ACT_ROWS_E4M3, 0, 0);
            g8(L.wgu, H, 1, c->pgu, f.inter, nullptr, EPI_SILU_MUL);
            launch_quant_rows(dt, c->pgu, f.inter, c->pxq, c->pxs, (int)M, f.inter, 4, s);
            g8(L.wdown, f.inter, 4, c->px, H, c->px, EPI_RESID);
        }
    } else {
    const int mtl = (int)((M + 15) / 16);
    constexpr int ws_maxm = 384;
    constexpr int ws_minpad = 24;
    bool ws = (int)M > 32 && (int)M <= ws_maxm && (int)((M + 127) / 128 * 128 - M) >= ws_minpad;
    if (ws) {
        GemmArgs p = gargs(c->pxn, H, c->ll[0].wqkv, nullptr, c->pqkv, c->ld.qkv_ld, (int)M); p.xpacked = ACT_TILES32; p.mtiles = mtl;
        GemmArgs d = gargs(c->pgu, f.inter, c->ll[0].wdown, nullptr, c->px, H, (int)M); d.xpacked = ACT_TILES32; d.mtiles = mtl;
        ws = wstat_supported(p, EPI_NONE) && wstat_supported(d, EPI_RESID);
    }
    auto prompt_gemm = [&](GemmArgs a, int epi, bool packed_out) {
        if (!ws) { run_gemm(c, a, epi); return; }
        a.xpacked = ACT_TILES32; a.mtiles = mtl; a.out_packed = packed_out ? ACT_TILES32 : ACT_ROWS;
        if (c->prompt_blk && xstat_blk_supported(a, epi)) { launch_xstat_blk(dt, a, epi, s); return; }
        launch_wstat(dt, a, epi, s);
    };
    int pend = 0;
    const ActLayout xl = ws ? ACT_TILES32 : ACT_ROWS;
    for (int l = 0; l < f.layers; ++l) {
        const LlamaLayer& L = c->ll[l];
        void* kc = kv_ptr(c, c->kcache, l);
        void* vc = kv_ptr(c, c->vcache, l);
        prompt_norm(L.attn_norm, c->pxn, xl, mtl, pend);
        pend = 0;
        { GemmArgs a = gargs(c->pxn, H, L.wqkv, nullptr, c->pqkv, c->ld.qkv_ld, (int)M); a.N = L.wqkv.Npad; prompt_gemm(a, EPI_NONE, false); }
        launch_rope_kv_prefill(dt, c->ld, c->pqkv, L.lora_bq, L.lora_bv, c->rope_cos, c->rope_sin, c->d_pos_ids, c->pq,
                               kc, vc, B, T, keep, s);
        AttnArgs at = prefill_attn_args(c, B, T, keep, l);
        at.o_packed_mt = ws ? mtl : 0;
        launch_attention(dt, 128, at, s);
        { GemmArgs a = gargs(c->patt, H, L.wo, nullptr, c->px, H, (int)M); a.resid = c->px; a.ldr = H; prompt_gemm(a, EPI_RESID, false); }
        prompt_norm(L.mlp_norm, c->pxn, xl, mtl, 0);
        { GemmArgs a = gargs(c->pxn, H, L.wgu, nullptr, c->pgu, f.inter, (int)M); prompt_gemm(a, EPI_SILU_MUL, true); }
        { GemmArgs a = gargs(c->pgu, f.inter, L.wdown, nullptr, c->px, H, (int)M); a.resid = c->px; a.ldr = H;
          GemmArgs b = a; b.xpacked = ACT_TILES32; b.mtiles = mtl;
          if (ws && c->prompt_blk && M <= 128 && xsplit_blk_supported(b)) { launch_xsplit_blk(dt, b, c->pslab, s); pend = 4; }
          else prompt_gemm(a, EPI_RESID, false); }
    }
    if (pend) prompt_norm(c->ll[0].attn_norm, c->pxn, xl, mtl, pend);
    }
    launch_gather_last(dt, c->px, c->datt, B, T, H, s);
    lm_head_and_greedy(c, c->datt, B, logits, nullptr, 0, 0);
    HIPCHK(c, hipGetLastError());
    return take_unsupported(c);
}

extern "C" int rdx_prefill(rdx_ctx* c, const int32_t* ids, const int32_t* mask, int B, int T, const float* qformer_embs,
                           int max_new, int eos_id, int pad_id, int32_t* out_tokens, void* logits) {
    return prefill_impl(c, ids, mask, B, T, qformer_embs, 0, max_new, eos_id, pad_id, out_tokens, logits);
}

extern "C" int rdx_prefill_append(rdx_ctx* c, const int32_t* ids_tail, int B, int T_tail, int keep_len, int max_new, int eos_id,
                                  int pad_id, int32_t* out_tokens, void* logits) {
    if (!c) return -1;
    if (c->rules_on) return fail(c, -1, "rdx_prefill_append: not available under logits rules (the token history is not carried across calls); rdx_set_logits_rules(ctx, NULL) first");
    if (keep_len <= 0 || c->cur_B <= 0) return fail(c, -1, "rdx_prefill_append: no cached conversation to continue (keep_len %d)", keep_len);
    return prefill_impl(c, ids_tail, nullptr, B, T_tail, nullptr, keep_len, max_new, eos_id, pad_id, out_tokens, logits);
}

static int decode_loop(rdx_ctx* c, int B, int max_new, int eos_id, void* scores, int* n_steps_host, int use_graph);

static void step_blk(rdx_ctx* c, int B) {
    const int dt = c->cfg.dtype;
    hipStream_t s = c->stream;
    for (int l = 0; l < c->cfg.layers; ++l) {
        const LlamaLayer* L = &c->ll[l];
        launch_xstat_blk(dt, norm_in_front(c, blk_unit(c, L, UNIT_QKV, B)), EPI_NONE, s);
        DecAttnArgs at = dec_attn_args(c, l);
        at.out_packed = ACT_TILES32; at.out_mt = (B + 15) / 16;
        launch_decode_attention(dt, at, B, s);
        launch_xstat_blk(dt, blk_unit(c, L, UNIT_O, B), EPI_RESID, s);
        launch_xstat_blk(dt, norm_in_front(c, blk_unit(c, L, UNIT_GATE_UP, B)), EPI_SILU_MUL, s);
        const GemmArgs d = blk_unit(c, L, UNIT_DOWN, B);
        if (c->blk_down && xsplit_blk_supported(d)) { launch_xsplit_blk(dt, d, c->kslab, s); c->pend_groups = 4; }
        else launch_wstat(dt, d, EPI_RESID, s);
    }
}

static void step_blk8(rdx_ctx* c, int B) {
    const int dt = c->cfg.dtype;
    hipStream_t s = c->stream;
    auto ksplit = [&](const GemmArgs& a) { launch_xsplit_blk8(dt, a, c->kslab, s); c->pend_groups = xsplit_blk8_groups(a); };
    for (int l = 0; l < c->cfg.layers; ++l) {
        const LlamaLayer* L = &c->ll[l];
        launch_xstat_blk8(dt, norm_in_front(c, blk8_unit(c, L, UNIT_QKV, B)), EPI_NONE, s);
        DecAttnArgs at = dec_attn_args(c, l);
        at.out_packed = ACT_BLK64;
        launch_decode_attention(dt, at, B, s);
        ksplit(blk8_unit(c, L, UNIT_O, B));
        launch_xstat_blk8(dt, norm_in_front(c, blk8_unit(c, L, UNIT_GATE_UP, B)), EPI_SILU_MUL, s);
        ksplit(blk8_unit(c, L, UNIT_DOWN, B));
    }
}

static void step_xs16(rdx_ctx* c, int B) {
    const int dt = c->cfg.dtype;
    hipStream_t s = c->stream;
    for (int l = 0; l < c->cfg.layers; ++l) {
        const LlamaLayer* L = &c->ll[l];
        launch_xstat16(dt, xs16_unit(c, L, UNIT_QKV, B), EPI_NONE, s);
        DecAttnArgs at = dec_attn_args(c, l);
        at.out_packed = ACT_BLK32;
        launch_decode_attention(dt, at, B, s);
        launch_xrow16(dt, xs16_unit(c, L, UNIT_O, B), s);
        launch_xstat16(dt, xs16_unit(c, L, UNIT_GATE_UP, B), EPI_SILU_MUL, s);
        launch_xrow16(dt, xs16_unit(c, L, UNIT_DOWN, B), s);
    }
}

static void attn_oproj(rdx_ctx* c, int l, int B) {
    const int dt = c->cfg.dtype;
    const LlamaLayer& L = c->ll[l];
    DecAttnArgs at = dec_attn_args(c, l);
    const GemmArgs ao = unit_args(c, &L, UNIT_O, B);
    if (c->fuse_attn_oproj && attn_oproj16_supported(c->ld, L.wo.N, L.wo.K, B)) {
        launch_attn_oproj16(dt, at, ao, B, c->d_ctr + (size_t)l * 256, c->d_err, c->stream);
        return;
    }
    const GemmArgs ap = ksplit_args(ao);
    const int kg = (B >= xs_min_rows() && c->kslab) ? xsplit32_groups(ap) : 0;
    at.out_packed = kg > 0 ? ap.xpacked : ACT_ROWS;
    launch_decode_attention(dt, at, B, c->stream);
    if (kg) launch_ksplit(c, ap);
    else skinny(c, ao, EPI_RESID);
}

static void step_generic(rdx_ctx* c, int B) {
    for (int l = 0; l < c->cfg.layers; ++l) {
        const LlamaLayer& L = c->ll[l];
        skinny(c, unit_args(c, &L, UNIT_QKV, B), EPI_NONE);
        attn_oproj(c, l, B);
        const bool split = down_split_ok(c, L, B);
        GemmArgs gu = unit_args(c, &L, UNIT_GATE_UP, B);
        gu.out_packed = split ? ksplit_args(unit_args(c, &L, UNIT_DOWN, B)).xpacked : ACT_ROWS;
        skinny(c, gu, EPI_SILU_MUL);
        launch_down(c, L, B, split);
    }
}

static void step_chained(rdx_ctx* c, int B, std::vector<hipEvent_t>* evs) {
    const rdx_config& f = c->cfg;
    hipStream_t s = c->stream;
    ChainArgs ca;
    memset(&ca, 0, sizeof(ca));
    ca.layers = c->d_clayers; ca.hidden = f.hidden; ca.inter = f.inter; ca.qkv_n = c->ll[0].wqkv.Npad; ca.qkv_ld = c->ld.qkv_ld; ca.B = B; ca.eps = f.rms_eps;
    ca.dx = c->dx; ca.dqkv = c->dqkv; ca.dgu = c->dgu; ca.ctr = c->d_cctr; ca.err = c->d_err; ca.naps = c->chain_naps;
    const LlamaLayer& L0 = c->ll[0];
    ca.w8 = (L0.wqkv.w8 && L0.wdown.w8 && f.hidden % 64 == 0 && f.inter % 64 == 0) ? 1 : 0;
    auto mark = [&] { if (evs) { hipEvent_t e; hipEventCreate(&e); hipEventRecord(e, s); evs->push_back(e); } };
    skinny(c, unit_args(c, &L0, UNIT_QKV, B), EPI_NONE);
    for (int l = 0; l < f.layers; ++l) {
        attn_oproj(c, l, B);
        skinny(c, unit_args(c, &c->ll[l], UNIT_GATE_UP, B), EPI_SILU_MUL);
        mark();
        ca.layer = l;
        ca.trace = l == c->chain_trace_layer ? c->chain_trace : nullptr;
        launch_decode_chain(f.dtype, ca, l + 1 < f.layers, s);
        mark();
    }
}

bool decode_step_launch(rdx_ctx* c, void* logits, const int* out_step, long step_stride, std::vector<hipEvent_t>* evs) {
    const int B = c->cur_B;
    const DecFamily fam = decode_family(c, B);
    switch (fam) {
    case DEC_UNSUPPORTED: c->unsupported = k_need_blk; return false;
    case DEC_BLK: step_blk(c, B); break;
    case DEC_BLK8: step_blk8(c, B); break;
    case DEC_XS16: step_xs16(c, B); break;
    case DEC_CHAINED: step_chained(c, B, evs); break;
    case DEC_GENERIC: step_generic(c, B); break;
    }
    lm_head_and_greedy(c, c->dx, B, logits, out_step, step_stride, 1);
    return fam == DEC_CHAINED;
}

extern "C" int rdx_decode_step(rdx_ctx* c, void* logits) {
    if (!c) return -1;
    if (!c->finalized || c->cur_B <= 0) return fail(c, -1, "rdx_decode_step: no prefill has run");
    if (c->cur_steps >= c->cur_max_new)
        return fail(c, -1, "rdx_decode_step: all %d tokens of this prompt (max_new) have been generated; run a new prefill", c->cur_max_new);
    if (c->cur_T + c->cur_steps > c->cfg.max_len || c->cur_T + c->cur_steps > c->cfg.max_pos)
        return fail(c, -1, "rdx_decode_step: KV cache full (%d prompt + %d generated slots of %d)", c->cur_T, c->cur_steps, c->cfg.max_len);
    if (int rrc = rules_need_prefill(c, "rdx_decode_step")) return rrc;
    HIPCHK(c, hipSetDevice(c->device));
    decode_step_launch(c, logits, nullptr, 0);
    ++c->cur_steps;
    HIPCHK(c, hipGetLastError());
    return take_unsupported(c);
}

extern "C" int rdx_decode_step_ids(rdx_ctx* c, const int32_t* ids, void* logits) {
    if (!c) return -1;
    if (!ids) return fail(c, -1, "rdx_decode_step_ids: null ids");
    if (!c->finalized || c->cur_B <= 0) return fail(c, -1, "rdx_decode_step_ids: no prefill has run");
    if (c->cur_steps >= c->cur_max_new)
        return fail(c, -1, "rdx_decode_step_ids: all %d tokens of this prompt (max_new) have been generated; run a new prefill", c->cur_max_new);
    if (c->cur_T + c->cur_steps > c->cfg.max_len || c->cur_T + c->cur_steps > c->cfg.max_pos)
        return fail(c, -1, "rdx_decode_step_ids: KV cache full (%d prompt + %d generated slots of %d)", c->cur_T, c->cur_steps, c->cfg.max_len);
    if (int rrc = rules_need_prefill(c, "rdx_decode_step_ids")) return rrc;
    HIPCHK(c, hipSetDevice(c->device));
    launch_embed_rows(c->cfg.dtype, ids, c->embed, c->cfg.vocab, c->dx, c->cur_B, c->cfg.hidden, c->stream);
    if (c->rules_on) launch_hist_set_last(ids, c->d_hist, c->d_hist_len, c->cfg.max_len, c->cur_B, c->stream);
    decode_step_launch(c, logits, nullptr, 0);
    ++c->cur_steps;
    HIPCHK(c, hipGetLastError());
    return take_unsupported(c);
}

int build_graph(rdx_ctx* c, void* scores, bool fixed) {
    const rdx_config& f = c->cfg;
    GraphKey k;
    k.B = c->cur_B; k.max_new = c->cur_max_new; k.eos = c->cur_eos; k.pad = c->cur_pad; k.tokens = c->cur_tokens; k.scores = scores; k.fixed = fixed;
    k.rules = c->rules;
    if (int rrc = rules_need_prefill(c, "decode step graph")) return rrc;
    if (c->graph && k == c->gkey) return 0;
    if (c->graph) { hipGraphExecDestroy(c->graph); c->graph = nullptr; }
    hipGraph_t g = nullptr;
    HIPCHK(c, hipStreamBeginCapture(c->stream, hipStreamCaptureModeThreadLocal));
    decode_step_launch(c, scores, (scores && !fixed) ? c->d_step : nullptr, (long)c->cur_B * f.vocab);
    HIPCHK(c, hipStreamEndCapture(c->stream, &g));
    if (int urc = take_unsupported(c)) { hipGraphDestroy(g); return urc; }
    HIPCHK(c, hipGraphInstantiate(&c->graph, g, nullptr, nullptr, 0));
    HIPCHK(c, hipGraphDestroy(g));
    c->gkey = k;
    return 0;
}

extern "C" int rdx_generate(rdx_ctx* c, const int32_t* ids, const int32_t* mask, int B, int T, const float* qformer_embs,
                            int max_new, int eos_id, int pad_id, int32_t* out_tokens, void* scores, int* n_steps_host,
                            int use_graph) {
    if (!c) return -1;
    if (max_new <= 0) return fail(c, -1, "rdx_generate: max_new must be positive");
    int rc = rdx_prefill(c, ids, mask, B, T, qformer_embs, max_new, eos_id, pad_id, out_tokens, scores);
    if (rc) return rc;
    return decode_loop(c, B, max_new, eos_id, scores, n_steps_host, use_graph);
}

extern "C" int rdx_generate_append(rdx_ctx* c, const int32_t* ids_tail, int B, int T_tail, int keep_len, int max_new, int eos_id,
                                   int pad_id, int32_t* out_tokens, void* scores, int* n_steps_host, int use_graph) {
    if (!c) return -1;
    if (max_new <= 0) return fail(c, -1, "rdx_generate_append: max_new must be positive");
    if (c->rules_on) return fail(c, -1, "rdx_generate_append: not available under logits rules (the token history is not carried across calls); rdx_set_logits_rules(ctx, NULL) first");
    int rc = rdx_prefill_append(c, ids_tail, B, T_tail, keep_len, max_new, eos_id, pad_id, out_tokens, scores);
    if (rc) return rc;
    return decode_loop(c, B, max_new, eos_id, scores, n_steps_host, use_graph);
}

static int decode_loop(rdx_ctx* c, int B, int max_new, int eos_id, void* scores, int* n_steps_host, int use_graph) {
    int rc = 0;
    const rdx_config& f = c->cfg;
    int done = 1;
    std::vector<int> unf(B, 1);
    auto all_finished = [&]() -> int {
        if (eos_id < 0) return 0;
        if (hipMemcpyAsync(unf.data(), c->d_unf, B * sizeof(int), hipMemcpyDeviceToHost, c->stream) != hipSuccess) return 0;
        if (hipStreamSynchronize(c->stream) != hipSuccess) return 0;
        for (int b = 0; b < B; ++b) if (unf[b]) return 0;
        return 1;
    };
    if (max_new > 1 && !all_finished()) {
        if (use_graph) {
            rc = build_graph(c, scores);
            if (rc) return rc;
        }
        static const int check_every = [] { const char* e = getenv("RDX_EOS_POLL"); const int v = e ? atoi(e) : 4; return v > 0 ? v : 4; }();
        while (done < max_new) {
            if (use_graph) {
                HIPCHK(c, hipGraphLaunch(c->graph, c->stream));
            } else {
                void* lg = scores ? (char*)scores + (size_t)done * B * f.vocab * 2 : nullptr;
                decode_step_launch(c, lg, nullptr, 0);
            }
            ++done;
            if (eos_id >= 0 && (done % check_every == 0) && done < max_new && all_finished()) break;
        }
    }
    HIPCHK(c, hipStreamSynchronize(c->stream));
    HIPCHK(c, hipGetLastError());
    if (n_steps_host) *n_steps_host = done;
    c->cur_steps = std::max(done, c->cur_max_new);
    int herr = 0;
    HIPCHK(c, hipMemcpy(&herr, c->d_err, sizeof(int), hipMemcpyDeviceToHost));
    if (herr) {
        hipMemset(c->d_err, 0, sizeof(int));
        return fail(c, -5, "rdx_generate: a workgroup hand-off timed out inside a fused/chained launch (results invalid)");
    }
    return 0;
}


namespace {
struct BeamHyp { float score; std::vector<int> toks; };
struct BeamHyps {
    int num_beams; float length_penalty; int early_stopping;
    std::vector<BeamHyp> beams; float worst = 1e9f;
    void add(const std::vector<int>& gen, int full_len, float sum_logprobs) {
        const float score = sum_logprobs / powf((float)full_len, length_penalty);
        if ((int)beams.size() < num_beams || score > worst) {
            beams.push_back(BeamHyp{score, gen});
            if ((int)beams.size() > num_beams) {
                int lo = 0;
                for (int i = 1; i < (int)beams.size(); ++i) if (beams[i].score < beams[lo].score) lo = i;
                beams.erase(beams.begin() + lo);
                float w = beams[0].score;
                for (const BeamHyp& h : beams) w = std::min(w, h.score);
                worst = w;
            } else {
                worst = std::min(score, worst);
            }
        }
    }
    bool is_done(float best_sum_logprobs, int cur_len) const {
        if ((int)beams.size() < num_beams) return false;
        if (early_stopping) return true;
        return worst >= best_sum_logprobs / powf((float)cur_len, length_penalty);
    }
};
}

extern "C" int rdx_beam_search(rdx_ctx* c, const int32_t* ids, const int32_t* mask, int groups, int num_beams, int T,
                               const float* qformer_embs, int max_new, int eos_id, int pad_id, float length_penalty,
                               int early_stopping, int32_t* out_tokens_host, int32_t* out_len_host, float* out_score_host,
                               void* step_scores, int* n_steps_host) {
    if (!c) return -1;
    if (!c->finalized || !c->cfg.enable_llama) return fail(c, -1, "rdx_beam_search: llama weights not finalized");
    const rdx_config& f = c->cfg;
    if (c->rules_on) return fail(c, -1, "rdx_beam_search: not available under logits rules (beam search applies them to log-softmax scores and reorders histories); rdx_set_logits_rules(ctx, NULL) first");
    const int rows = groups * num_beams;
    if (groups <= 0 || num_beams < 2 || num_beams > RDX_MAX_BEAMS) return fail(c, -1, "rdx_beam_search: num_beams must be in [2, %d]", RDX_MAX_BEAMS);
    if (rows > f.max_batch) return fail(c, -1, "rdx_beam_search: batch %d x %d beams exceeds max_batch %d", groups, num_beams, f.max_batch);
    if (max_new <= 0 || !out_tokens_host || !out_len_host) return fail(c, -1, "rdx_beam_search: bad arguments");
    HIPCHK(c, hipSetDevice(c->device));
    hipStream_t s = c->stream;
    const int K2 = 2 * num_beams, V = f.vocab;
    const int p_lo = T / 16 * 16, span = (T + max_new + 15) / 16 * 16 - p_lo;
    if (rows > c->bm_rows || max_new > c->bm_new) {
        HIPCHK(c, hipStreamSynchronize(s));
        dfree(c, c->bm_logits); dfree(c, c->bm_scores); dfree(c, c->bm_cand_s); dfree(c, c->bm_cand_i); dfree(c, c->bm_tok); dfree(c, c->bm_src); dfree(c, c->bm_out);
        const int R = std::max(rows, c->bm_rows), N = std::max(max_new, c->bm_new);
        c->bm_rows = 0;
        ALLOC(c, c->bm_logits, (size_t)R * V * 2); ALLOC(c, c->bm_scores, (size_t)R * 4);
        ALLOC(c, c->bm_cand_s, (size_t)R * 2 * 4); ALLOC(c, c->bm_cand_i, (size_t)R * 2 * 4);
        ALLOC(c, c->bm_tok, (size_t)R * 4); ALLOC(c, c->bm_src, (size_t)R * 2 * 4); ALLOC(c, c->bm_out, (size_t)R * N * 4);
        c->bm_rows = R; c->bm_new = N;
    }
    const size_t need = (size_t)f.layers * 2 * rows * f.heads * span * 256;
    if (need > c->bm_scratch_bytes) {
        HIPCHK(c, hipStreamSynchronize(s));
        dfree(c, c->bm_scratch); c->bm_scratch_bytes = 0;
        ALLOC(c, c->bm_scratch, need);
        c->bm_scratch_bytes = need;
    }
    int rc = prefill_impl(c, ids, mask, rows, T, qformer_embs, 0, max_new, -1, pad_id, c->bm_out, c->bm_logits);
    if (rc) return rc;
    rc = build_graph(c, c->bm_logits, true);
    if (rc) return rc;

    std::vector<float> beam_scores(rows, -1e9f), cs((size_t)groups * K2);
    for (int g = 0; g < groups; ++g) beam_scores[(size_t)g * num_beams] = 0.f;
    std::vector<int> ci((size_t)groups * K2), next_tok(rows), src(2 * (size_t)rows);
    std::vector<std::vector<int>> hist(rows), nh(rows);
    std::vector<BeamHyps> hyps(groups);
    for (BeamHyps& h : hyps) { h.num_beams = num_beams; h.length_penalty = length_penalty; h.early_stopping = early_stopping; }
    std::vector<char> done(groups, 0);
    const bool full_copy = getenv("RDX_BEAM_FULLCOPY") && atoi(getenv("RDX_BEAM_FULLCOPY"));
    int cur_len = T, steps = 0;
    for (int step = 0; step < max_new; ++step) {
        HIPCHK(c, hipMemcpyAsync(c->bm_scores, beam_scores.data(), rows * sizeof(float), hipMemcpyHostToDevice, s));
        void* lp = step_scores ? (char*)step_scores + (size_t)step * rows * V * 2 : nullptr;
        launch_beam_topk(f.dtype, c->bm_logits, c->bm_scores, groups, num_beams, V, c->bm_cand_s, c->bm_cand_i, lp, s);
        HIPCHK(c, hipMemcpyAsync(cs.data(), c->bm_cand_s, cs.size() * sizeof(float), hipMemcpyDeviceToHost, s));
        HIPCHK(c, hipMemcpyAsync(ci.data(), c->bm_cand_i, ci.size() * sizeof(int), hipMemcpyDeviceToHost, s));
        HIPCHK(c, hipStreamSynchronize(s));
        ++steps;
        for (int g = 0; g < groups; ++g) {
            const int r0 = g * num_beams;
            if (done[g]) {
                for (int b = 0; b < num_beams; ++b) { beam_scores[r0 + b] = 0.f; next_tok[r0 + b] = pad_id; src[r0 + b] = r0 + b; }
                continue;
            }
            int nb = 0;
            for (int rank = 0; rank < K2 && nb < num_beams; ++rank) {
                const float sc = cs[(size_t)g * K2 + rank];
                const int flat = ci[(size_t)g * K2 + rank], from = r0 + flat / V, tok = flat % V;
                if (eos_id >= 0 && tok == eos_id) {
                    if (rank >= num_beams) continue;
                    hyps[g].add(hist[from], cur_len, sc);
                } else {
                    beam_scores[r0 + nb] = sc; next_tok[r0 + nb] = tok; src[r0 + nb] = from;
                    ++nb;
                }
            }
            if (nb < num_beams) return fail(c, -7, "rdx_beam_search: fewer than %d live candidates in group %d (eos-only top-2k)", num_beams, g);
            done[g] = done[g] || hyps[g].is_done(cs[(size_t)g * K2], cur_len);
        }
        for (int r = 0; r < rows; ++r) {
            const std::vector<int>& mine = hist[r];
            const std::vector<int>& par = hist[src[r]];
            size_t cpre = 0;
            while (cpre < mine.size() && cpre < par.size() && mine[cpre] == par[cpre]) ++cpre;
            src[rows + r] = full_copy ? 0 : (T + (int)cpre) / 16 * 16;
        }
        for (int r = 0; r < rows; ++r) { nh[r] = hist[src[r]]; nh[r].push_back(next_tok[r]); }
        hist.swap(nh);
        ++cur_len;
        bool all_done = true;
        for (int g = 0; g < groups; ++g) all_done = all_done && done[g];
        if (all_done || cur_len >= T + max_new) break;
        HIPCHK(c, hipMemcpyAsync(c->bm_src, src.data(), 2 * rows * sizeof(int), hipMemcpyHostToDevice, s));
        HIPCHK(c, hipMemcpyAsync(c->bm_tok, next_tok.data(), rows * sizeof(int), hipMemcpyHostToDevice, s));
        bool identity = true;
        for (int r = 0; r < rows; ++r) identity = identity && src[r] == r;
        if (step > 0 && !identity)
            launch_kv_beam_reorder(c->kcache, c->vcache, c->bm_scratch, c->bm_src, c->bm_src + rows, rows, f.heads, f.layers, f.max_len, c->kv_layer_elems * 2,
                                   p_lo, std::min((T + step + 15) / 16 * 16, p_lo + span), s);
        launch_embed_rows(f.dtype, c->bm_tok, c->embed, V, c->dx, rows, f.hidden, s);
        HIPCHK(c, hipGraphLaunch(c->graph, s));
    }
// ... 20 lines not shown
```

### radialog_amd/csrc/attn_body.h

```cpp
#pragma once
#include "rdx_common.h"
#include "rdx_kernels.h"
#include "handoff.h"

namespace rdx {

template <typename T>
__device__ __forceinline__ float rope_one(float x, float partner_signed, float c, float s) {
    return rnd<T>(rnd<T>(x * c) + rnd<T>(partner_signed * s));
}

__host__ __device__ inline size_t decode_attention_smem_floats(int waves, int max_len) { return (size_t)waves * 128 + 128 + max_len; }

template <int N> __device__ __forceinline__ float row_share(float v) { return dpp_mov<0x150 + N>(v); }

template <typename T> __device__ __forceinline__ float dot2(unsigned a, unsigned b, float c);
template <> __device__ __forceinline__ float dot2<bf16>(unsigned a, unsigned b, float c) {
    typedef __bf16 v2b __attribute__((ext_vector_type(2)));
    return __builtin_amdgcn_fdot2_f32_bf16(__builtin_bit_cast(v2b, a), __builtin_bit_cast(v2b, b), c, false);
}
template <> __device__ __forceinline__ float dot2<f16>(unsigned a, unsigned b, float c) {
    typedef _Float16 v2h __attribute__((ext_vector_type(2)));
    return __builtin_amdgcn_fdot2(__builtin_bit_cast(v2h, a), __builtin_bit_cast(v2h, b), c, false);
}

template <typename T, int WAVES, bool DED = (WAVES == 8), typename WaitFn = NoWait, bool V_EARLY_ = !DED, int KG_ = 0, bool COH = false>
__device__ __forceinline__ void decode_attention_body(const DecAttnArgs& a, const int h, const int b, float* dsm,
                                                      WaitFn wait_inputs = WaitFn()) {
    typedef typename Vec8<T>::type V8;
    constexpr int D = 128;
    constexpr int CW = DED ? WAVES - 1 : WAVES;
    constexpr int KG = KG_ ? KG_ : ((DED && WAVES == 8) ? 4 : 2);
    constexpr int VR = 4 * KG;
    constexpr int SPAN = CW * 4;
    constexpr bool V_EARLY = V_EARLY_;
    constexpr int KT = 2, VT = 4;
    const LlamaDims& d = a.d;
    const T* qkv = reinterpret_cast<const T*>(a.qkv);
    const T* lbq = reinterpret_cast<const T*>(a.lbq);
    const T* lbv = reinterpret_cast<const T*>(a.lbv);
    const T* cos_t = reinterpret_cast<const T*>(a.cos_t);
    const T* sin_t = reinterpret_cast<const T*>(a.sin_t);

    const int tid = threadIdx.x, lane = tid & 63, w = __builtin_amdgcn_readfirstlane(tid >> 6);
    float* part = dsm;
    T* qT = reinterpret_cast<T*>(dsm + WAVES * D);
    float* S = dsm + WAVES * D + D;

    const int jsub = lane >> 4, doct = lane & 15;
    const int g = lane >> 4, r = lane & 15;
    const int H = d.hidden;
    const T* x = qkv + (size_t)b * d.qkv_ld;
    T* kc = reinterpret_cast<T*>(a.kcache) + ((size_t)b * d.heads + h) * d.max_len * D;
    T* vc = reinterpret_cast<T*>(a.vcache) + ((size_t)b * d.heads + h) * d.max_len * D;
    const uint8_t* km = a.key_mask + (size_t)b * d.max_len;

    if (a.trace && h == 0 && b == 0 && tid == 0) a.trace[7] = (long long)__builtin_amdgcn_s_memrealtime();
    const int cw = DED ? w - 1 : w;
    const bool owns_rows = !DED || w > 0;
    u4 kr[KG][4], vr[VR];
    unsigned kmw[KG];
    constexpr int KG_LO = (KG + 1) / 2, VR_LO = 4 * KG_LO;
    auto load_k = [&](int u0, int u1, int limit) {
#pragma unroll
        for (int u = 0; u < KG; ++u) {
            const int gb = (u * CW + cw) * 16;
            if (u >= u0 && u < u1 && gb < limit) {
                const int j = min(gb + r, d.max_len - 1);
#pragma unroll
                for (int c = 0; c < 4; ++c) kr[u][c] = ldg16(kc + kperm(j, c * 32 + g * 8, d.k_perm));
                kmw[u] = *reinterpret_cast<const unsigned*>(km + min(gb + 4 * g, d.max_len - 4));
            }
        }
    };
    auto load_v = [&](int u0, int u1, int limit) {
#pragma unroll
        for (int u = 0; u < VR; ++u) {
            if (u >= u0 && u < u1 && (u & ~1) * SPAN + cw * 4 < limit) {
                const int j = min(u * SPAN + cw * 4 + jsub, d.max_len - 1);
                vr[u] = ldg16(vc + (size_t)j * D + doct * 8);
            }
        }
    };
    constexpr bool HAS_WAIT = !__is_same(WaitFn, NoWait);
    const int n0 = h * D + doct * 8;
    u4 nq, nk_, nv, ncos, nsin, naq, nav, nbq0, nbq1, nbv0, nbv1;
    auto load_newtok = [&]() {
        auto ldx = [&](const T* p) -> u4 {
            if (!COH) return ldg16(p);
            const unsigned long long lo = ld8_agent(p), hi = ld8_agent(p + 4);
            return (u4){(unsigned)lo, (unsigned)(lo >> 32), (unsigned)hi, (unsigned)(hi >> 32)};
        };
        nq = ldx(x + n0); nk_ = ldx(x + H + n0); nv = ldx(x + 2 * H + n0);
        const T* cs = reinterpret_cast<const T*>(a.cur_rope);
        const T* cp = cs ? cs + (size_t)b * 2 * D : cos_t + (size_t)a.pos[b] * D;
        const T* sp = cs ? cs + (size_t)b * 2 * D + D : sin_t + (size_t)a.pos[b] * D;
        ncos = ldg16(cp + doct * 8); nsin = ldg16(sp + doct * 8);
        if (d.lora_r == 8) {
            const int e0 = 2 * jsub;
            naq = ldx(x + 3 * H); nav = ldx(x + 3 * H + 8);
            nbq0 = ldg16(lbq + (size_t)(n0 + e0) * 8); nbq1 = ldg16(lbq + (size_t)(n0 + e0 + 1) * 8);
            nbv0 = ldg16(lbv + (size_t)(n0 + e0) * 8); nbv1 = ldg16(lbv + (size_t)(n0 + e0 + 1) * 8);
        }
    };
    if (!HAS_WAIT && w == 0) load_newtok();
    if (owns_rows) {
        load_k(0, KG_LO, 0x7fffffff);
        if (V_EARLY) load_v(0, VR_LO, 0x7fffffff);
    }
    const int slot = a.slot_b[b];
    const int nk = slot + 1;
    long long* trc = (a.trace && h == 0 && b == 0 && tid == 0) ? a.trace : nullptr;
#define ATT_T(i) do { if (trc) trc[i] = (long long)__builtin_amdgcn_s_memrealtime(); } while (0)
    ATT_T(0);
    wait_inputs();
    ATT_T(1);

    float s_new = 0.f;
    if (w == 0) {
        float q8n[8], k8[8], v8[8];
        if (HAS_WAIT) load_newtok();
        const V8 qv = as_vec8<T>(nq), kv = as_vec8<T>(nk_), vv = as_vec8<T>(nv), cv = as_vec8<T>(ncos), sv_ = as_vec8<T>(nsin);
#pragma unroll
        for (int e = 0; e < 8; ++e) { q8n[e] = tof<T>(qv[e]); k8[e] = tof<T>(kv[e]); v8[e] = tof<T>(vv[e]); }
        if (d.lora_r == 8) {
            const V8 aq = as_vec8<T>(naq), av = as_vec8<T>(nav);
            const V8 bq0 = as_vec8<T>(nbq0), bq1 = as_vec8<T>(nbq1), bv0 = as_vec8<T>(nbv0), bv1 = as_vec8<T>(nbv1);
            float sq0 = 0.f, sq1 = 0.f, sv0 = 0.f, sv1 = 0.f;
#pragma unroll
            for (int i = 0; i < 8; ++i) {
                sq0 += tof<T>(bq0[i]) * tof<T>(aq[i]); sq1 += tof<T>(bq1[i]) * tof<T>(aq[i]);
                sv0 += tof<T>(bv0[i]) * tof<T>(av[i]); sv1 += tof<T>(bv1[i]) * tof<T>(av[i]);
            }
            sq0 = rnd<T>(rnd<T>(sq0) * d.lora_scale); sq1 = rnd<T>(rnd<T>(sq1) * d.lora_scale);
            sv0 = rnd<T>(rnd<T>(sv0) * d.lora_scale); sv1 = rnd<T>(rnd<T>(sv1) * d.lora_scale);
#pragma unroll
            for (int e = 0; e < 8; ++e) {
                const int src = ((e >> 1) << 4) | doct;
                const float dq = __shfl((e & 1) ? sq1 : sq0, src, 64), dv = __shfl((e & 1) ? sv1 : sv0, src, 64);
                q8n[e] = rnd<T>(q8n[e] + dq);
                v8[e] = rnd<T>(v8[e] + dv);
            }
        }
        const bool lo = doct < 8;
#pragma unroll
        for (int e = 0; e < 8; ++e) {
            const float qo = dpp_mov<DPP_ROR8>(q8n[e]), ko = dpp_mov<DPP_ROR8>(k8[e]);
            const float c = tof<T>(cv[e]), sn = tof<T>(sv_[e]);
            q8n[e] = rope_one<T>(q8n[e], lo ? -qo : qo, c, sn);
            k8[e] = rope_one<T>(k8[e], lo ? -ko : ko, c, sn);
        }
        if (jsub == 0) {
            V8 qo, ko, vo;
#pragma unroll
            for (int e = 0; e < 8; ++e) { qo[e] = fromf<T>(q8n[e]); ko[e] = fromf<T>(k8[e]); vo[e] = fromf<T>(v8[e]); }
            *reinterpret_cast<u4*>(qT + doct * 8) = as_u4<T>(qo);
            stg16(kc + kperm(slot, doct * 8, d.k_perm), as_u4<T>(ko));
            stg16(vc + (size_t)slot * D + doct * 8, as_u4<T>(vo));
#pragma unroll
            for (int e = 0; e < 8; ++e) part[doct * 8 + e] = v8[e];
        }
        {
            float acc = 0.f;
#pragma unroll
            for (int e = 0; e < 8; ++e) acc += q8n[e] * k8[e];
            s_new = row16_sum(acc);
        }
    }
    if (owns_rows) {
        load_k(KG_LO, KG, slot);
        if (V_EARLY) load_v(VR_LO, VR, slot);
    }
    ATT_T(2);
    __syncthreads();
    ATT_T(3);

    const float div = sqrtf((float)D);
    const int km_new = km[min(slot, d.max_len - 1)];
    u4 qb[4];
#pragma unroll
    for (int c = 0; c < 4; ++c) qb[c] = *reinterpret_cast<const u4*>(qT + c * 32 + g * 8);
    auto score_group = [&](const u4 (&kf)[4], unsigned maskw, int gb) {
        v4f acc = (v4f){0.f, 0.f, 0.f, 0.f};
#pragma unroll
        for (int c = 0; c < 4; ++c) acc = mfma16(as_vec8<T>(kf[c]), as_vec8<T>(qb[c]), acc);
        if (r == 0) {
#pragma unroll
            for (int i = 0; i < 4; ++i) {
                const int j = gb + 4 * g + i;
                if (j < slot) S[j] = ((maskw >> (8 * i)) & 0xffu) ? rnd<T>(rnd<T>(acc[i]) / div) : -INFINITY;
            }
        }
    };
    if (owns_rows) {
#pragma unroll
        for (int u = 0; u < KG; ++u)
            if (u < KG_LO || (u * CW + cw) * 16 < slot) score_group(kr[u], kmw[u], (u * CW + cw) * 16);
        if (!V_EARLY) { load_v(0, VR_LO, 0x7fffffff); load_v(VR_LO, VR, slot); }
        for (int gi = KG * CW + cw; gi * 16 < slot; gi += KT * CW) {
            u4 kf[KT][4];
            unsigned mw[KT];
#pragma unroll
            for (int t = 0; t < KT; ++t) {
                if (t > 0 && !((gi + t * CW) * 16 < slot)) break;
                const int gb = (gi + t * CW) * 16;
                const int j = min(gb + r, d.max_len - 1);
#pragma unroll
                for (int c = 0; c < 4; ++c) kf[t][c] = ldg16(kc + kperm(j, c * 32 + g * 8, d.k_perm));
                mw[t] = *reinterpret_cast<const unsigned*>(km + min(gb + 4 * g, d.max_len - 4));
            }
#pragma unroll
            for (int t = 0; t < KT; ++t)
                if (t == 0 || (gi + t * CW) * 16 < slot) score_group(kf[t], mw[t], (gi + t * CW) * 16);
        }
    }
    if (w == 0 && lane == 0) S[slot] = km_new ? rnd<T>(rnd<T>(s_new) / div) : -INFINITY;
    __syncthreads();
    ATT_T(4);

    float mx = -INFINITY;
    for (int j = lane; j < nk; j += 64) mx = fmaxf(mx, S[j]);
    mx = wave_max(mx);
    float sum = 0.f;
    for (int j = lane; j < nk; j += 64) sum += expf(S[j] - mx);
    sum = wave_sum(sum);
    ATT_T(5);

    float o8[8];
#pragma unroll
    for (int e = 0; e < 8; ++e) o8[e] = 0.f;
    if (owns_rows) {
        float myp = 0.f;
        {
            const int j = doct * SPAN + cw * 4 + jsub;
            if (doct < VR && j < slot) myp = rnd<T>(expf(S[j] - mx) / sum);
        }
        float pu[16];
        pu[0] = row_share<0>(myp);   pu[1] = row_share<1>(myp);   pu[2] = row_share<2>(myp);   pu[3] = row_share<3>(myp);
        pu[4] = row_share<4>(myp);   pu[5] = row_share<5>(myp);   pu[6] = row_share<6>(myp);   pu[7] = row_share<7>(myp);
        pu[8] = row_share<8>(myp);   pu[9] = row_share<9>(myp);   pu[10] = row_share<10>(myp); pu[11] = row_share<11>(myp);
        pu[12] = row_share<12>(myp); pu[13] = row_share<13>(myp); pu[14] = row_share<14>(myp); pu[15] = row_share<15>(myp);
#pragma unroll
        for (int u = 0; u < VR; u += 2) {
            if (u >= VR_LO && u * SPAN + cw * 4 >= slot) continue;
            const unsigned pp = (unsigned)bits16<T>(fromf<T>(pu[u])) | ((unsigned)bits16<T>(fromf<T>(pu[u + 1])) << 16);
            const unsigned a0[4] = {vr[u].x, vr[u].y, vr[u].z, vr[u].w};
            const unsigned a1[4] = {vr[u + 1].x, vr[u + 1].y, vr[u + 1].z, vr[u + 1].w};
#pragma unroll
            for (int e = 0; e < 4; ++e) {
                const unsigned lo = __builtin_amdgcn_perm(a1[e], a0[e], 0x05040100u);
                const unsigned hi = __builtin_amdgcn_perm(a1[e], a0[e], 0x07060302u);
                o8[2 * e] = dot2<T>(lo, pp, o8[2 * e]);
                o8[2 * e + 1] = dot2<T>(hi, pp, o8[2 * e + 1]);
            }
        }
        for (int j0 = VR * SPAN; j0 < slot; j0 += VT * SPAN) {
            u4 vt[VT];
            float pt[VT];
#pragma unroll
            for (int t = 0; t < VT; ++t) {
                const int j = j0 + t * SPAN + cw * 4 + jsub;
                vt[t] = (j0 + t * SPAN + cw * 4 < slot) ? ldg16(vc + (size_t)min(j, d.max_len - 1) * D + doct * 8) : (u4){0u, 0u, 0u, 0u};
                pt[t] = j < slot ? rnd<T>(expf(S[j] - mx) / sum) : 0.f;
            }
#pragma unroll
            for (int t = 0; t < VT; t += 2) {
                const unsigned pp = (unsigned)bits16<T>(fromf<T>(pt[t])) | ((unsigned)bits16<T>(fromf<T>(pt[t + 1])) << 16);
                const unsigned a0[4] = {vt[t].x, vt[t].y, vt[t].z, vt[t].w};
                const unsigned a1[4] = {vt[t + 1].x, vt[t + 1].y, vt[t + 1].z, vt[t + 1].w};
#pragma unroll
                for (int e = 0; e < 4; ++e) {
                    const unsigned lo = __builtin_amdgcn_perm(a1[e], a0[e], 0x05040100u);
                    const unsigned hi = __builtin_amdgcn_perm(a1[e], a0[e], 0x07060302u);
                    o8[2 * e] = dot2<T>(lo, pp, o8[2 * e]);
                    o8[2 * e + 1] = dot2<T>(hi, pp, o8[2 * e + 1]);
                }
            }
        }
    }
    if (w == 0 && jsub == 0) {
        const float p = rnd<T>(expf(S[slot] - mx) / sum);
#pragma unroll
        for (int e = 0; e < 8; ++e) o8[e] += p * part[doct * 8 + e];
    }
#pragma unroll
    for (int e = 0; e < 8; ++e) o8[e] = xor32_sum(xor16_sum(o8[e]));
    if (jsub == 0) {
#pragma unroll
        for (int e = 0; e < 8; ++e) part[w * D + doct * 8 + e] = o8[e];
    }
    __syncthreads();
    ATT_T(6);
    if (!COH) {
        if (tid < D) {
            float v = 0.f;
#pragma unroll
            for (int i = 0; i < WAVES; ++i) v += part[i * D + tid];
            const int k = h * D + tid;
            const int pf = a.out_packed == ACT_BLK64 ? 2 * (k >> 6) + ((k & 15) >> 3) : (k >> 5), pg = a.out_packed == ACT_BLK64 ? ((k & 63) >> 4) : ((k & 31) >> 3);
            const size_t o = a.out_packed == ACT_BLK64 ? (size_t)(b >> 5) * (32 * H) + (((size_t)((pf * 2 + ((b >> 4) & 1)) * 64 + pg * 16 + (b & 15)) << 3) + (k & 7))
                           : a.out_packed != ACT_ROWS ? ((size_t)((pf * a.out_mt + (b >> 4)) * 64 + pg * 16 + (b & 15)) << 3) + (k & 7) : (size_t)b * H + k;
            reinterpret_cast<T*>(a.out)[o] = fromf<T>(v);
        }
    } else if (tid < D / 4) {
        unsigned long long pk = 0ull;
#pragma unroll
        for (int e = 0; e < 4; ++e) {
            float v = 0.f;
#pragma unroll
            for (int i = 0; i < WAVES; ++i) v += part[i * D + tid * 4 + e];
            pk |= (unsigned long long)bits16<T>(fromf<T>(v)) << (16 * e);
        }
        st8_agent(reinterpret_cast<T*>(a.out) + (size_t)b * H + h * D + tid * 4, pk);
    }
#undef ATT_T
}

}
```

### radialog_amd/csrc/chain.hip

```cpp
#include "rdx_common.h"
#include "rdx_kernels.h"
#include "attn_body.h"
#include "handoff.h"
#include "skinny_body.h"

namespace rdx {

constexpr int CH_WAVES = 16;
constexpr int CH_THREADS = CH_WAVES * 64;
constexpr int CH_MAXM = 2;

struct ChainGemm {
    const void* X; int ldx;
    const void* W;
    const void* resid; int ldr;
    void* out; int ldo;
    int M, N, K;
    const void* norm_w; float eps;
    const void* W8; const float* wscale;
};

template <typename T, int EPI, bool NORM, int SUB, int XL, typename WaitFn, int U = 4, bool RESID_EARLY = false, bool W8 = false>
__device__ __forceinline__ void chain_tile(const ChainGemm& a, const int wg, const int ntiles, unsigned char* smem, WaitFn wait_inputs,
                                           long long* trace = nullptr) {
    typedef typename Vec8<T>::type V8;
    constexpr int WPS = CH_WAVES / SUB;
    float* red = reinterpret_cast<float*>(smem);
    float* ssq = red + CH_WAVES * 256;
    float* rstd_s = ssq + CH_WAVES * CH_MAXM;
    T* xs = reinterpret_cast<T*>(rstd_s + 16);

    const int lane = threadIdx.x & 63, wa = __builtin_amdgcn_readfirstlane(threadIdx.x >> 6);
    const int sub = wa / WPS, w = wa - sub * WPS;
    const int tile = wg * SUB + sub;
    const int tile_c = min(tile, ntiles - 1);
    const int r = lane & 15, g = lane >> 4;
    const int K = a.K, KC = W8 ? (K >> 6) : (K >> 5);
    const int c0 = (KC * w) / WPS, c1 = (KC * (w + 1)) / WPS;
    const T* X = reinterpret_cast<const T*>(a.X);
    const u4* wbase = reinterpret_cast<const u4*>(W8 ? a.W8 : a.W) + (size_t)tile_c * KC * 64 + lane;
    const int clast = min(max(c1 - 1, c0), KC - 1);
    long long* trc = (trace && threadIdx.x == 0) ? trace : nullptr;
#define CH_T(i) do { if (trc) trc[i] = (long long)__builtin_amdgcn_s_memrealtime(); } while (0)
    CH_T(0);

    u4 wa_[U], wb_[U];
#pragma unroll
    for (int u = 0; u < U; ++u) wa_[u] = ldg16_nt(wbase + (size_t)min(c0 + u, clast) * 64);
#pragma unroll
    for (int u = 0; u < U; ++u) wb_[u] = ldg16_nt(wbase + (size_t)min(c0 + U + u, clast) * 64);
    if (trace) {
        if (threadIdx.x < 64) asm volatile("s_waitcnt vmcnt(%0)" :: "n"(2 * U - 1) : "memory");
        CH_T(5);
    }

    constexpr int QPT_E = EPI == EPI_SILU_MUL ? 2 : 4;
    unsigned long long rs8_early = 0ull;
    if (RESID_EARLY && EPI == EPI_RESID && (int)threadIdx.x < SUB * a.M * QPT_E) {
        const int so = threadIdx.x / (a.M * QPT_E), rem = threadIdx.x - so * (a.M * QPT_E);
        const int m = rem / QPT_E, q = rem - m * QPT_E;
        const int n = (wg * SUB + so) * 16 + q * 4;
        if (wg * SUB + so < ntiles && n < a.N) rs8_early = ld8_agent(reinterpret_cast<const T*>(a.resid) + (size_t)m * a.ldr + n);
    }

    wait_inputs();
    CH_T(3);

    const int K4 = K >> 2, total4 = a.M * K4;
    unsigned long long xr[XL];
#pragma unroll
    for (int i = 0; i < XL; ++i) {
        const int c = threadIdx.x + i * CH_THREADS;
        xr[i] = 0ull;
        if (c < total4) { const int m = c / K4, k4 = c - m * K4; xr[i] = ld8_agent(X + (size_t)m * a.ldx + (size_t)k4 * 4); }
    }
    if (NORM) {
        float ss[CH_MAXM];
#pragma unroll
        for (int m = 0; m < CH_MAXM; ++m) ss[m] = 0.f;
#pragma unroll
        for (int i = 0; i < XL; ++i) {
            const int c = threadIdx.x + i * CH_THREADS;
            float t = 0.f;
#pragma unroll
            for (int j = 0; j < 4; ++j) { const float f = tof<T>(from_bits16<T>((unsigned short)(xr[i] >> (16 * j)))); t += f * f; }
            const int m = c < total4 ? c / K4 : 0;
#pragma unroll
            for (int mm = 0; mm < CH_MAXM; ++mm) ss[mm] += (m == mm) ? t : 0.f;
        }
#pragma unroll
        for (int m = 0; m < CH_MAXM; ++m) {
            const float t = wave_sum(ss[m]);
            if (lane == 0) ssq[wa * CH_MAXM + m] = t;
        }
        __syncthreads();
        if (threadIdx.x < CH_MAXM) {
            float t = 0.f;
#pragma unroll
            for (int i = 0; i < CH_WAVES; ++i) t += ssq[i * CH_MAXM + threadIdx.x];
            rstd_s[threadIdx.x] = rsqrtf(t / (float)K + a.eps);
        }
        __syncthreads();
    }
    {
        const T* NW = reinterpret_cast<const T*>(a.norm_w);
#pragma unroll
        for (int i = 0; i < XL; ++i) {
            const int c = threadIdx.x + i * CH_THREADS;
            if (c < total4) {
                const int m = c / K4, k4 = c - m * K4;
                unsigned long long v = xr[i];
                if (NORM) {
                    const float rs = rstd_s[m];
                    const unsigned long long nw = *reinterpret_cast<const unsigned long long*>(NW + (size_t)k4 * 4);
                    v = 0ull;
#pragma unroll
                    for (int j = 0; j < 4; ++j) {
                        const float h = rnd<T>(tof<T>(from_bits16<T>((unsigned short)(xr[i] >> (16 * j)))) * rs);
                        const float wv_ = tof<T>(from_bits16<T>((unsigned short)(nw >> (16 * j))));
                        v |= (unsigned long long)bits16<T>(fromf<T>(wv_ * h)) << (16 * j);
                    }
                }
                *reinterpret_cast<unsigned long long*>(xs + (size_t)m * K + (size_t)k4 * 4) = v;
            }
        }
        __syncthreads();
    }

    const T* xrow = xs + (size_t)(r < a.M ? r : 0) * K + g * (W8 ? 16 : 8);
    v4f acc = (v4f){0.f, 0.f, 0.f, 0.f};
    CH_T(6);
    auto consume = [&](const u4 (&wreg)[U], int cb, bool guard) {
#pragma unroll
        for (int u = 0; u < U; ++u) {
            if (!guard || cb + u < c1) {
                if (W8) {
#pragma unroll
                    for (int h = 0; h < 2; ++h) {
                        const u4 wd = dequant8<T>(h ? wreg[u].z : wreg[u].x, h ? wreg[u].w : wreg[u].y);
                        const u4 xv = *reinterpret_cast<const u4*>(xrow + (size_t)(cb + u) * 64 + h * 8);
                        acc = mfma16(as_vec8<T>(wd), as_vec8<T>(xv), acc);
                    }
                } else {
                    const u4 xv = *reinterpret_cast<const u4*>(xrow + (size_t)(cb + u) * 32);
                    acc = mfma16(as_vec8<T>(wreg[u]), as_vec8<T>(xv), acc);
                }
            }
        }
    };
    auto consume1 = [&](const u4& wv, int c) {
        if (W8) {
#pragma unroll
            for (int h = 0; h < 2; ++h) {
                const u4 wd = dequant8<T>(h ? wv.z : wv.x, h ? wv.w : wv.y);
                const u4 xv = *reinterpret_cast<const u4*>(xrow + (size_t)c * 64 + h * 8);
                acc = mfma16(as_vec8<T>(wd), as_vec8<T>(xv), acc);
            }
        } else {
            const u4 xv = *reinterpret_cast<const u4*>(xrow + (size_t)c * 32);
            acc = mfma16(as_vec8<T>(wv), as_vec8<T>(xv), acc);
        }
    };
    int cb = c0;
    for (; cb + 2 * U < c1; cb += 2 * U) {
#pragma unroll
        for (int u = 0; u < 2 * U; ++u) {
            u4& wr = u < U ? wa_[u] : wb_[u - U];
            consume1(wr, cb + u);
            wr = ldg16_nt(wbase + (size_t)min(cb + 2 * U + u, clast) * 64);
            __builtin_amdgcn_sched_barrier(0);
        }
    }
    consume(wa_, cb, true);
    consume(wb_, cb + U, true);
    CH_T(1);
    *reinterpret_cast<float4*>(&red[wa * 256 + r * 16 + g * 4]) = make_float4(acc[0], acc[1], acc[2], acc[3]);
    __syncthreads();

    T* out = reinterpret_cast<T*>(a.out);
    constexpr int QPT = EPI == EPI_SILU_MUL ? 2 : 4;
    const int items = SUB * a.M * QPT;
    if ((int)threadIdx.x < items) {
        const int so = threadIdx.x / (a.M * QPT), rem = threadIdx.x - so * (a.M * QPT);
        const int m = rem / QPT, q = rem - m * QPT;
        const int t_o = wg * SUB + so;
        const int n = t_o * 16 + q * 4;
        const bool ok = (t_o < ntiles) && (n < a.N);
        float v[4];
#pragma unroll
        for (int j = 0; j < 4; ++j) {
            v[j] = 0.f;
#pragma unroll
            for (int i = 0; i < WPS; ++i) v[j] += red[(so * WPS + i) * 256 + m * 16 + q * 4 + j];
            if (W8) v[j] *= a.wscale[t_o * 16 + q * 4 + j];
        }
        unsigned long long pk = 0ull;
        if (EPI == EPI_NONE) {
#pragma unroll
            for (int j = 0; j < 4; ++j) pk |= (unsigned long long)bits16<T>(fromf<T>(v[j])) << (16 * j);
            if (ok) st8_agent(out + (size_t)m * a.ldo + n, pk);
        } else if (EPI == EPI_RESID) {
            if (ok) {
                const unsigned long long rs8 = RESID_EARLY ? rs8_early : ld8_agent(reinterpret_cast<const T*>(a.resid) + (size_t)m * a.ldr + n);
#pragma unroll
                for (int j = 0; j < 4; ++j) {
                    const float rsd = tof<T>(from_bits16<T>((unsigned short)(rs8 >> (16 * j))));
                    pk |= (unsigned long long)bits16<T>(fromf<T>(rsd + rnd<T>(v[j]))) << (16 * j);
                }
                st8_agent(out + (size_t)m * a.ldo + n, pk);
            }
        } else if (EPI == EPI_SILU_MUL) {
#pragma unroll
            for (int j = 0; j < 4; ++j) {
                float u = 0.f;
#pragma unroll
                for (int i = 0; i < WPS; ++i) u += red[(so * WPS + i) * 256 + m * 16 + 8 + q * 4 + j];
                if (W8) u *= a.wscale[t_o * 16 + 8 + q * 4 + j];
                pk |= (unsigned long long)bits16<T>(fromf<T>(swiglu<T>(v[j], u))) << (16 * j);
            }
            if (ok) st8_agent(out + (size_t)m * a.ldo + t_o * 8 + q * 4, pk);
        }
    }
    CH_T(7);
#undef CH_T
}

template <typename T, bool W8>
__global__ __launch_bounds__(CH_THREADS, 4) void decode_chain_k(ChainArgs ca) {
    extern __shared__ __attribute__((aligned(16))) unsigned char msm[];
    const ChainLayer& L = ca.layers[ca.layer];
    int* ctr = ca.ctr + (size_t)ca.layer * HO_CTR_INTS;
    const int H = ca.hidden, B = ca.B;
    long long* trace = ca.trace ? ca.trace + (size_t)blockIdx.x * 8 : nullptr;
    if ((int)blockIdx.x < ca.nwg_down) {
        ChainGemm g = {ca.dgu, ca.inter, L.wdown, ca.dx, H, ca.dx, H, B, H, ca.inter, nullptr, 0.f, L.wdown8, L.sdown};
        chain_tile<T, EPI_RESID, false, 1, 6, WaitSharded, 4, false, W8>(g, blockIdx.x, ca.nwg_down, msm, WaitSharded{ctr, 0, ca.err, ca.naps, nullptr}, trace);
        publish_sc1(ctr, blockIdx.x);
        if (trace && threadIdx.x == 0) trace[2] = (long long)__builtin_amdgcn_s_memrealtime();
        return;
    }
    const ChainLayer& Ln = ca.layers[ca.layer + 1];
    ChainGemm g = {ca.dx, H, Ln.wqkv, nullptr, 0, ca.dqkv, ca.qkv_ld, B, ca.qkv_n, H, Ln.attn_norm, ca.eps, Ln.wqkv8, Ln.sqkv};
    chain_tile<T, EPI_NONE, true, 4, 2, WaitSharded, W8 ? 4 : 8, false, W8>(g, blockIdx.x - ca.nwg_down, (ca.qkv_n + 15) / 16, msm,
                                                                             WaitSharded{ctr, ca.nwg_down, ca.err, ca.naps, nullptr}, trace);
}

template <typename T, bool W8>
__global__ __launch_bounds__(CH_THREADS, 4) void attn_oproj16_k(DecAttnArgs at, ChainGemm g, int n_attn, int ntiles, int* counter, int* err) {
    extern __shared__ __attribute__((aligned(16))) unsigned char msm[];
    if ((int)blockIdx.x < n_attn) {
        const int b = blockIdx.x / at.d.heads, h = blockIdx.x - b * at.d.heads;
        decode_attention_body<T, CH_WAVES, true, NoWait, true, 0, true>(at, h, b, reinterpret_cast<float*>(msm));
        publish_sc1(counter, blockIdx.x);
    } else {
        chain_tile<T, EPI_RESID, false, 2, 2, WaitSharded, W8 ? 4 : 8, true, W8>(g, blockIdx.x - n_attn, ntiles, msm, WaitSharded{counter, n_attn, err, 1, nullptr});
    }
}

bool attn_oproj16_supported(const LlamaDims& d, int N, int K, int B) {
    const int ntiles = (N + 15) / 16;
    return B <= CH_MAXM && d.head_dim == 128 && K % 32 == 0 && N % 4 == 0 && (size_t)B * K <= 8192 &&
           d.heads * B + (ntiles + 1) / 2 <= 256;
}

void launch_attn_oproj16(int dtype, const DecAttnArgs& a, const GemmArgs& ga, int B, int* counter, int* err, hipStream_t s) {
    const int n_attn = a.d.heads * B, ntiles = (ga.N + 15) / 16;
    const bool w8 = ga.W8 && ga.wscale && ga.K % 64 == 0;
    ChainGemm g = {ga.X, ga.ldx, ga.W, ga.resid, ga.ldr, ga.out, ga.ldo, ga.M, ga.N, ga.K, nullptr, 0.f, ga.W8, ga.wscale};
    const size_t sm_gemm = (size_t)(CH_WAVES * 256 + CH_WAVES * CH_MAXM + 16) * 4 + (size_t)B * ga.K * 2;
    const size_t sm_att = decode_attention_smem_floats(CH_WAVES, a.d.max_len) * sizeof(float);
    const size_t smem = sm_gemm > sm_att ? sm_gemm : sm_att;
    dim3 grid(n_attn + (ntiles + 1) / 2), block(CH_THREADS);
    RDX_DISPATCH_T(dtype, T, {
        if (w8) hipLaunchKernelGGL((attn_oproj16_k<T, true>), grid, block, smem, s, a, g, n_attn, ntiles, counter, err);
        else hipLaunchKernelGGL((attn_oproj16_k<T, false>), grid, block, smem, s, a, g, n_attn, ntiles, counter, err);
    });
}

bool chain_supported(const LlamaDims& d, int inter, int B) {
    if (B > CH_MAXM || d.head_dim != 128 || d.hidden % 32 || inter % 32 || d.hidden % 16) return false;
    const size_t stage = (size_t)B * (inter > d.hidden ? inter : d.hidden) * 2;
    return stage <= 48 * 1024 && inter % 4 == 0 && (size_t)B * d.hidden <= 8192 && (size_t)B * inter <= 24576;
}

size_t chain_ctr_ints(int layers) { return (size_t)layers * HO_CTR_INTS; }

void launch_decode_chain(int dtype, ChainArgs ca, bool with_next_qkv, hipStream_t s) {
    ca.nwg_down = ca.hidden / 16;
    const int nwg_qkv = with_next_qkv ? ((ca.qkv_n + 15) / 16 + 3) / 4 : 0;
    const int kmax = ca.inter > ca.hidden ? ca.inter : ca.hidden;
    const size_t sm_gemm = (size_t)(CH_WAVES * 256 + CH_WAVES * CH_MAXM + 16) * 4 + (size_t)ca.B * kmax * 2;
    const size_t smem = sm_gemm > (size_t)84 * 1024 ? sm_gemm : (size_t)84 * 1024;
    dim3 grid(ca.nwg_down + nwg_qkv), block(CH_THREADS);
    RDX_DISPATCH_T(dtype, T, {
        static DevOnce attr_set;
        if (attr_set.first()) {
            hipFuncSetAttribute((const void*)decode_chain_k<T, false>, hipFuncAttributeMaxDynamicSharedMemorySize, 100 * 1024);
            hipFuncSetAttribute((const void*)decode_chain_k<T, true>, hipFuncAttributeMaxDynamicSharedMemorySize, 100 * 1024);
        }
        if (ca.w8) hipLaunchKernelGGL((decode_chain_k<T, true>), grid, block, smem, s, ca);
        else hipLaunchKernelGGL((decode_chain_k<T, false>), grid, block, smem, s, ca);
    });
}

}
```

### radialog_amd/csrc/elem.hip

```cpp
#include <algorithm>
#include "rdx_common.h"
#include "rdx_kernels.h"

namespace rdx {


template <typename T>
__global__ __launch_bounds__(256) void quant_rows_k(const T* __restrict__ x, long ldx, unsigned char* __restrict__ out8, float* __restrict__ xscale,
                                                    int K, int G) {
    typedef typename Vec8<T>::type V8;
    __shared__ float red[32];
    __shared__ float gmax[4];
    const size_t row = blockIdx.x;
    const T* xr = x + row * ldx;
    const int NB = K >> 7;
    int end[4];
#pragma unroll
    for (int q = 0; q < 4; ++q) end[q] = q < G ? ((NB * (q + 1)) / G) * 128 : K;
    auto group_of = [&](int i) { return (i >= end[0]) + (i >= end[1]) + (i >= end[2]); };
    float mx[4] = {0.f, 0.f, 0.f, 0.f};
    for (int i = threadIdx.x * 8; i < K; i += blockDim.x * 8) {
        const float m = amax8<T>(as_vec8<T>(ldg16(xr + i)));
        const int gq = group_of(i);
#pragma unroll
// ... 215 lines not shown
    const float rstd = rsqrtf(block_sum(v, red) / (float)H + eps);
    const T* er = emb ? emb + (size_t)(row % emb_rows) * H : nullptr;
    for (int i = threadIdx.x; i < H; i += blockDim.x) {
        float y = (tof<T>(xr[i]) - mean) * rstd * gamma[i] + beta[i];
        if (er) y += tof<T>(er[i]);
        out[row * ldo + i] = fromf<T>(y);
    }
}
void launch_layernorm_ex(int dtype, const void* x, long ldx, const float* gamma, const float* beta, const void* emb, int emb_rows,
                         void* out, long ldo, int rows, int H, float eps, hipStream_t s) {
    RDX_DISPATCH_T(dtype, T, hipLaunchKernelGGL((layernorm_ex_k<T>), dim3(rows), dim3(256), 0, s, (const T*)x, ldx, gamma, beta,
                                                (const T*)emb, emb_rows, (T*)out, ldo, H, eps));
}

template <typename T>
__global__ void pool_gather_k(const T* __restrict__ src, T* __restrict__ dst, int B, int L, int C) {
    const size_t i = (size_t)blockIdx.x * blockDim.x + threadIdx.x;
    const int C8 = C >> 3;
    if (i >= (size_t)B * 2 * L * C8) return;
    const int c8 = (int)(i % C8);
    const size_t tok = i / C8;
    const int j = (int)(tok % (2 * L)), b = (int)(tok / (2 * L));
    const size_t srow = (size_t)(j < L ? b : B + b) * L + (j % L);
    stg16(dst + tok * C + c8 * 8, ldg16(src + srow * C + c8 * 8));
}
void launch_pool_gather(int dtype, const void* src, void* dst, int B, int L, int C, hipStream_t s) {
    const size_t n = (size_t)B * 2 * L * (C >> 3);
    RDX_DISPATCH_T(dtype, T, hipLaunchKernelGGL((pool_gather_k<T>), dim3((unsigned)((n + 255) / 256)), dim3(256), 0, s, (const T*)src,
                                                (T*)dst, B, L, C));
}
template <typename T>
__global__ void pool_concat_k(const T* __restrict__ patch, const T* __restrict__ tokens, T* __restrict__ dst, int B, int L, int C) {
    const size_t i = (size_t)blockIdx.x * blockDim.x + threadIdx.x;
    const int C8 = C >> 3;
    if (i >= (size_t)B * L * 2 * C8) return;
    const int c8 = (int)(i % (2 * C8));
    const size_t row = i / (2 * C8);
    const int b = (int)(row / L), j = (int)(row % L);
    const T* srcp = c8 < C8 ? patch + row * C + c8 * 8 : tokens + ((size_t)b * 2 * L + j) * C + (c8 - C8) * 8;
    stg16(dst + row * 2 * C + c8 * 8, ldg16(srcp));
}
void launch_pool_concat(int dtype, const void* patch, const void* tokens, void* dst, int B, int L, int C, hipStream_t s) {
    const size_t n = (size_t)B * L * 2 * (C >> 3);
    RDX_DISPATCH_T(dtype, T, hipLaunchKernelGGL((pool_concat_k<T>), dim3((unsigned)((n + 255) / 256)), dim3(256), 0, s, (const T*)patch,
                                                (const T*)tokens, (T*)dst, B, L, C));
}

template <typename T>
__global__ __launch_bounds__(256) void scramble_layernorm_k(const T* __restrict__ pp, const float* __restrict__ gamma,
                                                            const float* __restrict__ beta, T* __restrict__ out,
                                                            float* __restrict__ out_f32, int P, int C, float eps) {
    __shared__ float red[32];
    extern __shared__ float rowbuf[];
    const int rrow = blockIdx.x, b = blockIdx.y;
    const T* src = pp + (size_t)b * P * C;
    float s = 0.f;
    if ((C & 7) == 0) {
        typedef typename Vec8<T>::type V8;
        const int f0 = rrow * C, ch_lo = (f0 / P) & ~7, ch_hi = (f0 + C - 1) / P;
        const int nch8 = ((ch_hi - ch_lo) >> 3) + 1;
        for (int it = threadIdx.x; it < P * nch8; it += blockDim.x) {
            const int pos = it / nch8, ch8 = ch_lo + (it - pos * nch8) * 8;
            if (ch8 >= C) continue;
            const V8 v = as_vec8<T>(ldg16(src + (size_t)pos * C + ch8));
#pragma unroll
            for (int j = 0; j < 8; ++j) {
                const int c = (ch8 + j) * P + pos - f0;
                if (c >= 0 && c < C) rowbuf[c] = tof<T>(v[j]);
            }
        }
        __syncthreads();
        for (int c = threadIdx.x; c < C; c += blockDim.x) s += rowbuf[c];
    } else {
        for (int c = threadIdx.x; c < C; c += blockDim.x) {
            const size_t f = (size_t)rrow * C + c;
            const int ch = (int)(f / P), pos = (int)(f % P);
            const float v = tof<T>(src[(size_t)pos * C + ch]);
            rowbuf[c] = v;
            s += v;
        }
    }
    const float mean = block_sum(s, red) / (float)C;
    float v2 = 0.f;
    for (int c = threadIdx.x; c < C; c += blockDim.x) { const float d = rowbuf[c] - mean; v2 += d * d; }
    const float rstd = rsqrtf(block_sum(v2, red) / (float)C + eps);
    const size_t o = ((size_t)b * P + rrow) * C;
    for (int c = threadIdx.x; c < C; c += blockDim.x) {
        const float y = (rowbuf[c] - mean) * rstd * gamma[c] + beta[c];
        if (out) out[o + c] = fromf<T>(y);
        if (out_f32) out_f32[o + c] = y;
    }
}

void launch_scramble_layernorm(int dtype, const void* pp_nhwc, const float* gamma, const float* beta, void* out,
                               float* out_f32, int B, int P, int C, float eps, hipStream_t s) {
    RDX_DISPATCH_T(dtype, T, hipLaunchKernelGGL((scramble_layernorm_k<T>), dim3(P, B), dim3(256), (size_t)C * sizeof(float), s,
                                                (const T*)pp_nhwc, gamma, beta, (T*)out, out_f32, P, C, eps));
}

template <typename T>
__global__ __launch_bounds__(256) void img_prep_k(const float* __restrict__ img, T* __restrict__ out, int S, int pad, int Hp,
                                                  int Wp) {
    const int b = blockIdx.z, y = blockIdx.y;
    const int x = blockIdx.x * blockDim.x + threadIdx.x;
    if (x >= Wp) return;
    typedef T T4 __attribute__((ext_vector_type(4)));
    T4 o;
    o[0] = o[1] = o[2] = o[3] = fromf<T>(0.f);
    const int iy = y - pad, ix = x - pad;
    if (iy >= 0 && iy < S && ix >= 0 && ix < S) {
        const size_t plane = (size_t)S * S;
        const float* p = img + (size_t)b * 3 * plane + (size_t)iy * S + ix;
        o[0] = fromf<T>(p[0]); o[1] = fromf<T>(p[plane]); o[2] = fromf<T>(p[2 * plane]);
    }
    *reinterpret_cast<T4*>(out + (((size_t)b * Hp + y) * Wp + x) * 4) = o;
}

void launch_img_prep(int dtype, const float* img, void* out, int B, int S, int pad, int Hp, int Wp, hipStream_t s) {
    dim3 grid((Wp + 255) / 256, Hp, B), block(256);
    RDX_DISPATCH_T(dtype, T, hipLaunchKernelGGL((img_prep_k<T>), grid, block, 0, s, img, (T*)out, S, pad, Hp, Wp));
}

template <typename T>
__global__ __launch_bounds__(256) void maxpool_k(const T* __restrict__ in, T* __restrict__ out, int H, int W, int C, int Ho,
                                                 int Wo, size_t total) {
    typedef typename Vec8<T>::type V8;
    const size_t idx = (size_t)blockIdx.x * blockDim.x + threadIdx.x;
    if (idx >= total) return;
    const int C8 = C >> 3;
    const int c8 = (int)(idx % C8);
    size_t rest = idx / C8;
    const int ow = (int)(rest % Wo); rest /= Wo;
    const int oh = (int)(rest % Ho);
    const int b = (int)(rest / Ho);
    float m[8];
#pragma unroll
    for (int j = 0; j < 8; ++j) m[j] = -INFINITY;
    for (int kh = 0; kh < 3; ++kh) {
        const int ih = oh * 2 - 1 + kh;
        if (ih < 0 || ih >= H) continue;
        for (int kw = 0; kw < 3; ++kw) {
            const int iw = ow * 2 - 1 + kw;
            if (iw < 0 || iw >= W) continue;
            V8 v = as_vec8<T>(ldg16(in + (((size_t)b * H + ih) * W + iw) * C + c8 * 8));
#pragma unroll
            for (int j = 0; j < 8; ++j) m[j] = fmaxf(m[j], tof<T>(v[j]));
        }
    }
    V8 o;
#pragma unroll
    for (int j = 0; j < 8; ++j) o[j] = fromf<T>(m[j]);
    stg16(out + (((size_t)b * Ho + oh) * Wo + ow) * C + c8 * 8, as_u4<T>(o));
}

void launch_maxpool(int dtype, const void* in, void* out, int B, int H, int W, int C, hipStream_t s) {
    const int Ho = (H + 2 - 3) / 2 + 1, Wo = (W + 2 - 3) / 2 + 1;
    const size_t total = (size_t)B * Ho * Wo * (C >> 3);
    RDX_DISPATCH_T(dtype, T, hipLaunchKernelGGL((maxpool_k<T>), dim3((unsigned)((total + 255) / 256)), dim3(256), 0, s,
                                                (const T*)in, (T*)out, H, W, C, Ho, Wo, total));
}

template <typename T>
__global__ void broadcast_rows_k(const T* __restrict__ src, T* __restrict__ dst, size_t per, size_t total) {
    const size_t i = (size_t)blockIdx.x * blockDim.x + threadIdx.x;
    if (i < total) dst[i] = src[i % per];
}
void launch_broadcast_rows(int dtype, const void* src, void* dst, int rows, int H, int B, hipStream_t s) {
    const size_t per = (size_t)rows * H, total = per * B;
    RDX_DISPATCH_T(dtype, T, hipLaunchKernelGGL((broadcast_rows_k<T>), dim3((unsigned)((total + 255) / 256)), dim3(256), 0, s,
                                                (const T*)src, (T*)dst, per, total));
}

template <typename T> __global__ void to_f32_k(const T* __restrict__ src, float* __restrict__ dst, size_t n) {
    const size_t i = (size_t)blockIdx.x * blockDim.x + threadIdx.x;
    if (i < n) dst[i] = tof<T>(src[i]);
}
template <typename T> __global__ void from_f32_k(const float* __restrict__ src, T* __restrict__ dst, size_t n) {
    const size_t i = (size_t)blockIdx.x * blockDim.x + threadIdx.x;
    if (i < n) dst[i] = fromf<T>(src[i]);
}
void launch_to_f32(int dtype, const void* src, float* dst, size_t n, hipStream_t s) {
    RDX_DISPATCH_T(dtype, T, hipLaunchKernelGGL((to_f32_k<T>), dim3((unsigned)((n + 255) / 256)), dim3(256), 0, s, (const T*)src, dst, n));
}
void launch_from_f32(int dtype, const float* src, void* dst, size_t n, hipStream_t s) {
    RDX_DISPATCH_T(dtype, T, hipLaunchKernelGGL((from_f32_k<T>), dim3((unsigned)((n + 255) / 256)), dim3(256), 0, s, src, (T*)dst, n));
}

__global__ void prep_prompt_k(const int* __restrict__ ids, const int* __restrict__ mask_in, int T_, int img_id, int pad_id,
                              int* __restrict__ img_pos, int* __restrict__ pos_ids, uint8_t* __restrict__ key_mask, long km_bs,
                              int max_len_fill, int* __restrict__ pos_next, int* __restrict__ slot_b, int* __restrict__ step_b,
                              int* __restrict__ unfinished) {
    const int b = blockIdx.x;
    const int* row = ids + (size_t)b * T_;
    uint8_t* km = key_mask + (size_t)b * km_bs;
    if (threadIdx.x == 0) {
        int first = -1, cum = 0;
        for (int t = 0; t < T_; ++t) {
            if (first < 0 && row[t] == img_id) first = t;
            const int m = mask_in ? (mask_in[(size_t)b * T_ + t] != 0) : (row[t] != pad_id);
            cum += m;
            pos_ids[(size_t)b * T_ + t] = m ? (cum - 1) : 1;
            km[t] = (uint8_t)m;
        }
        img_pos[b] = first < 0 ? 0 : first;
        pos_next[b] = cum;
        slot_b[b] = T_;
        step_b[b] = 0;
        unfinished[b] = 1;
    }
    for (int t = T_ + threadIdx.x; t < max_len_fill; t += blockDim.x) km[t] = 1;
}
void launch_prep_prompt(const int* ids, const int* mask_in, int B, int T_, int img_id, int pad_id, int* img_pos, int* pos_ids,
                        uint8_t* key_mask, long km_bs, int* pos_next, int* slot_b, int* step_b, int* unfinished, hipStream_t s) {
    hipLaunchKernelGGL(prep_prompt_k, dim3(B), dim3(256), 0, s, ids, mask_in, T_, img_id, pad_id, img_pos, pos_ids, key_mask,
                       km_bs, (int)km_bs, pos_next, slot_b, step_b, unfinished);
}

__global__ void prep_append_k(int T_, int keep_len, int* __restrict__ img_pos, int* __restrict__ pos_ids, int* __restrict__ pos_next,
                              int* __restrict__ slot_b, int* __restrict__ step_b, int* __restrict__ unfinished) {
    const int b = blockIdx.x;
    const int pads = slot_b[b] - pos_next[b];
    const int base = keep_len - pads;
    for (int t = threadIdx.x; t < T_; t += blockDim.x) pos_ids[(size_t)b * T_ + t] = base + t;
    __syncthreads();
    if (threadIdx.x == 0) {
        img_pos[b] = 0;
        pos_next[b] = base + T_;
        slot_b[b] = keep_len + T_;
        step_b[b] = 0;
        unfinished[b] = 1;
    }
}
void launch_prep_append(int B, int T_, int keep_len, int* img_pos, int* pos_ids, int* pos_next, int* slot_b, int* step_b,
                        int* unfinished, hipStream_t s) {
    hipLaunchKernelGGL(prep_append_k, dim3(B), dim3(256), 0, s, T_, keep_len, img_pos, pos_ids, pos_next, slot_b, step_b, unfinished);
}

template <typename T>
__global__ __launch_bounds__(256) void embed_splice_k(const int* __restrict__ ids, const int* __restrict__ img_pos,
                                                      const T* __restrict__ embed, int vocab, const T* __restrict__ img_emb,
                                                      int n_img, T* __restrict__ out, int T_, int H, int use_img) {
    const int t = blockIdx.x, b = blockIdx.y;
    const T* src;
    const int p = img_pos[b];
    if (use_img && t >= p && t < p + n_img) {
        src = img_emb + ((size_t)b * n_img + (t - p)) * H;
    } else {
        int id = ids[(size_t)b * T_ + t];
        id = id < 0 ? 0 : (id >= vocab ? vocab - 1 : id);
        src = embed + (size_t)id * H;
    }
    T* dst = out + ((size_t)b * T_ + t) * H;
    for (int i = threadIdx.x * 8; i < H; i += blockDim.x * 8) stg16(dst + i, ldg16(src + i));
}
void launch_embed_splice(int dtype, const int* ids, const int* img_pos, const void* embed, int vocab, const void* img_emb,
                         int n_img, void* out, int B, int T_, int H, int use_img, hipStream_t s) {
    RDX_DISPATCH_T(dtype, T, hipLaunchKernelGGL((embed_splice_k<T>), dim3(T_, B), dim3(256), 0, s, ids, img_pos, (const T*)embed,
                                                vocab, (const T*)img_emb, n_img, (T*)out, T_, H, use_img));
}

template <typename T>
__global__ void gather_last_k(const T* __restrict__ x, T* __restrict__ out, int T_, int H) {
    const int b = blockIdx.x;
    const T* src = x + ((size_t)b * T_ + (T_ - 1)) * H;
    for (int i = threadIdx.x * 8; i < H; i += blockDim.x * 8) stg16(out + (size_t)b * H + i, ldg16(src + i));
}
void launch_gather_last(int dtype, const void* x, void* out, int B, int T_, int H, hipStream_t s) {
    RDX_DISPATCH_T(dtype, T, hipLaunchKernelGGL((gather_last_k<T>), dim3(B), dim3(256), 0, s, (const T*)x, (T*)out, T_, H));
}


__device__ __forceinline__ void zero_handoff_counters(int* __restrict__ ctr_zero, int n_zero) {
    if (ctr_zero && blockIdx.x == 0) for (int i = threadIdx.x; i < n_zero; i += blockDim.x) ctr_zero[i] = 0;
}

__device__ __forceinline__ int block_argmax256(float bv, int bi) {
    __shared__ float sv[256];
    __shared__ int si[256];
    sv[threadIdx.x] = bv; si[threadIdx.x] = bi;
    __syncthreads();
    for (int o = 128; o > 0; o >>= 1) {
        if (threadIdx.x < o) {
            const float v = sv[threadIdx.x + o];
            const int ix = si[threadIdx.x + o];
            if (v > sv[threadIdx.x] || (v == sv[threadIdx.x] && ix < si[threadIdx.x])) { sv[threadIdx.x] = v; si[threadIdx.x] = ix; }
        }
        __syncthreads();
    }
    return si[0];
}

template <typename T>
__device__ __forceinline__ void step_tail(const StepTail& t, int b, int tok) {
    __shared__ int tok_s, pos_s;
    if (threadIdx.x == 0) {
        const int step = t.step_b[b];
        if (t.eos_id >= 0) {
            const int unf = t.unfinished[b];
            tok = unf ? tok : t.pad_id;
            if (tok == t.eos_id) t.unfinished[b] = 0;
        }
        if (step < t.max_new) t.out_tokens[(size_t)b * t.max_new + step] = tok;
        t.step_b[b] = step + 1;
        if (t.slot_b) t.slot_b[b] += 1;
        int pcur = t.pos_ro ? t.pos_ro[b] : 0;
        if (t.pos) { pcur = t.pos[b] + 1; t.pos[b] = pcur; }
        if (t.hist) {
            const int L = t.hist_len[b];
            if (L < t.hist_ld) { t.hist[(size_t)b * t.hist_ld + L] = tok; t.hist_len[b] = L + 1; }
        }
        pos_s = pcur;
        tok_s = tok;
    }
    __syncthreads();
    int id = tok_s;
    id = id < 0 ? 0 : (id >= t.vocab ? t.vocab - 1 : id);
    const T* src = (const T*)t.embed + (size_t)id * t.H;
    T* x_next = (T*)t.x_next;
    for (int i = threadIdx.x * 8; i < t.H; i += blockDim.x * 8) stg16(x_next + (size_t)b * t.H + i, ldg16(src + i));
    if (t.cur_rope && threadIdx.x < 32) {
        const int half = threadIdx.x >> 4, c8 = (threadIdx.x & 15) * 8;
        const T* tab = (const T*)(half ? t.sin_t : t.cos_t);
        stg16((T*)t.cur_rope + (size_t)b * 256 + half * 128 + c8, ldg16(tab + (size_t)pos_s * 128 + c8));
    }
}

template <typename T>
__global__ __launch_bounds__(256) void greedy_step_k(const float* __restrict__ part_val, const int* __restrict__ part_idx,
                                                     int n_tiles, StepTail t) {
    const int b = blockIdx.x;
    zero_handoff_counters(t.ctr_zero, t.n_zero);
    float bv = -INFINITY;
    int bi = 0x7fffffff;
    for (int i = threadIdx.x; i < n_tiles; i += blockDim.x) {
        const float v = part_val[(size_t)b * n_tiles + i];
        const int ix = part_idx[(size_t)b * n_tiles + i];
        if (v > bv || (v == bv && ix < bi)) { bv = v; bi = ix; }
    }
    step_tail<T>(t, b, block_argmax256(bv, bi));
}

__device__ __forceinline__ unsigned bits8(const unsigned* m, int i) {
    const int w = i >> 5, sh = i & 31;
    const unsigned long long lo = m[w], hi = sh > 24 ? m[w + 1] : 0u;
    return (unsigned)(((hi << 32) | lo) >> sh) & 0xffu;
}
template <typename T>
__device__ __forceinline__ T apply_rules(T v, bool seen, bool ban, float p) {
    if (seen) {
        const float f = tof<T>(v);
        v = fromf<T>(f < 0.f ? f * p : __fdiv_rn(f, p));
    }
    return ban ? fromf<T>(-INFINITY) : v;
}
template <typename T>
__global__ __launch_bounds__(256) void select_step_k(SelectArgs a, StepTail t) {
    extern __shared__ unsigned sel_bits[];
    const int b = blockIdx.x, V = t.vocab, W = (V + 31) >> 5;
    unsigned* seen = sel_bits;
    unsigned* ban = sel_bits + W;
    zero_handoff_counters(t.ctr_zero, t.n_zero);
    for (int i = threadIdx.x; i < 2 * W; i += blockDim.x) sel_bits[i] = 0u;
    __syncthreads();
    const int L = min(t.hist_len[b], t.hist_ld), gen = a.n_gen[b], n = a.ngram;
    const int* h = t.hist + (size_t)b * t.hist_ld;
    if (a.penalty != 1.0f)
        for (int j = threadIdx.x; j < L; j += blockDim.x) {
            const int id = h[j];
            if (id >= 0 && id < V) atomicOr(&seen[id >> 5], 1u << (id & 31));
        }
    if (n > 0 && L + 1 >= n)
        for (int j = threadIdx.x; j + n - 1 < L; j += blockDim.x) {
            bool same = true;
            for (int k = 0; k < n - 1 && same; ++k) same = h[j + k] == h[L - n + 1 + k];
            const int id = h[j + n - 1];
            if (same && id >= 0 && id < V) atomicOr(&ban[id >> 5], 1u << (id & 31));
        }
    if (threadIdx.x == 0 && a.min_new > 0 && t.eos_id >= 0 && t.eos_id < V && gen < a.min_new) atomicOr(&ban[t.eos_id >> 5], 1u << (t.eos_id & 31));
    __syncthreads();

    T* row = (T*)a.logits + (size_t)gen * a.step_stride + (size_t)b * V;
    const float p = a.penalty;
    float bv = -INFINITY;
    int bi = 0x7fffffff;
    auto one = [&](int i) {
        const T v0 = row[i];
        const bool s = (seen[i >> 5] >> (i & 31)) & 1u, x = (ban[i >> 5] >> (i & 31)) & 1u;
        const T v1 = apply_rules<T>(v0, s, x, p);
        if (s || x) row[i] = v1;
        const float f = tof<T>(v1);
        if (f > bv || (f == bv && i < bi)) { bv = f; bi = i; }
    };
    const int head = min(V, (int)(((16u - (unsigned)((uintptr_t)row & 15u)) & 15u) >> 1));
    const int nvec = (V - head) >> 3;
    if ((int)threadIdx.x < head) one(threadIdx.x);
    for (int i = head + nvec * 8 + threadIdx.x; i < V; i += blockDim.x) one(i);
    for (int q = threadIdx.x; q < nvec; q += blockDim.x) {
        const int i = head + q * 8;
        typename Vec8<T>::type v = as_vec8<T>(ldg16(row + i));
        const unsigned s = bits8(seen, i), x = bits8(ban, i);
        if (s | x) {
#pragma unroll
            for (int j = 0; j < 8; ++j) v[j] = apply_rules<T>(v[j], (s >> j) & 1u, (x >> j) & 1u, p);
            stg16(row + i, as_u4<T>(v));
        }
#pragma unroll
        for (int j = 0; j < 8; ++j) {
            const float f = tof<T>(v[j]);
            if (f > bv || (f == bv && i + j < bi)) { bv = f; bi = i + j; }
        }
    }
    const int tok = block_argmax256(bv, bi);
    if (a.sel_out) {
        if (threadIdx.x == 0) a.sel_out[b] = tok;
        return;
    }
    step_tail<T>(t, b, tok);
}
template <typename T>
__global__ void avgpool_flatten_k(const T* __restrict__ in, T* __restrict__ out, int B, int G, int C, int pool) {
    const int Gp = G / pool;
    const size_t total = (size_t)B * C * Gp * Gp;
    for (size_t i = blockIdx.x * (size_t)blockDim.x + threadIdx.x; i < total; i += (size_t)gridDim.x * blockDim.x) {
        const int w = (int)(i % Gp), h = (int)((i / Gp) % Gp), c = (int)((i / ((size_t)Gp * Gp)) % C), b = (int)(i / ((size_t)Gp * Gp * C));
        float acc = 0.f;
        for (int dy = 0; dy < pool; ++dy)
            for (int dx = 0; dx < pool; ++dx)
                acc += tof<T>(in[(((size_t)b * G + h * pool + dy) * G + w * pool + dx) * C + c]);
        out[i] = fromf<T>(acc / (float)(pool * pool));
    }
}
void launch_avgpool_flatten(int dtype, const void* in, void* out, int B, int G, int C, int pool, hipStream_t s) {
    const size_t total = (size_t)B * C * (G / pool) * (G / pool);
    const int blocks = (int)std::min<size_t>((total + 255) / 256, 4096);
    RDX_DISPATCH_T(dtype, T, hipLaunchKernelGGL((avgpool_flatten_k<T>), dim3(blocks), dim3(256), 0, s, (const T*)in, (T*)out, B, G, C, pool));
}

void launch_greedy_step(int dtype, const float* part_val, const int* part_idx, int n_tiles, int B, const StepTail& t, hipStream_t s) {
    RDX_DISPATCH_T(dtype, T, hipLaunchKernelGGL((greedy_step_k<T>), dim3(B), dim3(256), 0, s, part_val, part_idx, n_tiles, t));
}

bool select_step_supported(int vocab) { return vocab > 0 && select_step_lds(vocab) <= 48 * 1024; }

void launch_select_step(int dtype, const SelectArgs& a, const StepTail& t, int B, hipStream_t s) {
    RDX_DISPATCH_T(dtype, T, hipLaunchKernelGGL((select_step_k<T>), dim3(B), dim3(256), select_step_lds(t.vocab), s, a, t));
}

__global__ void hist_set_last_k(const int* __restrict__ ids, int* __restrict__ hist, const int* __restrict__ hist_len, int ld, int B) {
    const int b = blockIdx.x * blockDim.x + threadIdx.x;
    if (b >= B) return;
    const int L = hist_len[b];
    if (L > 0 && L <= ld) hist[(size_t)b * ld + L - 1] = ids[b];
}
void launch_hist_set_last(const int* ids, int* hist, const int* hist_len, int ld, int B, hipStream_t s) {
    hipLaunchKernelGGL(hist_set_last_k, dim3((B + 63) / 64), dim3(64), 0, s, ids, hist, hist_len, ld, B);
}

__global__ void hist_init_k(const int* __restrict__ ids, int T_, int* __restrict__ hist, int* __restrict__ hist_len, int ld) {
    const int b = blockIdx.x;
    for (int t = threadIdx.x; t < T_ && t < ld; t += blockDim.x) hist[(size_t)b * ld + t] = ids[(size_t)b * T_ + t];
    if (threadIdx.x == 0) hist_len[b] = min(T_, ld);
}
void launch_hist_init(const int* ids, int B, int T_, int* hist, int* hist_len, int ld, hipStream_t s) {
    hipLaunchKernelGGL(hist_init_k, dim3(B), dim3(256), 0, s, ids, T_, hist, hist_len, ld);
}

}
```

### radialog_amd/csrc/handoff.h

```cpp
#pragma once
#include "rdx_common.h"

namespace rdx {

typedef __attribute__((address_space(1))) int gint;

struct NoWait { __device__ __forceinline__ void operator()() const {} };

struct WaitCounter {
    int* counter; int target; int* err;
    __device__ __forceinline__ void operator()() const {
        if (threadIdx.x == 0) {
            bool ok = false;
            gint* gc = (gint*)counter;
            for (int it = 0; it < (1 << 16); ++it) {
                if (__hip_atomic_load(gc, __ATOMIC_RELAXED, __HIP_MEMORY_SCOPE_AGENT) >= target) { ok = true; break; }
                __builtin_amdgcn_s_sleep(4);
            }
            if (!ok) *err = 1;
            __builtin_amdgcn_fence(__ATOMIC_ACQUIRE, "agent");
        }
        __syncthreads();
    }
};

__device__ __forceinline__ void publish(int* counter) {
    asm volatile("s_waitcnt vmcnt(0)" ::: "memory");
    __syncthreads();
    if (threadIdx.x == 0) {
        __builtin_amdgcn_fence(__ATOMIC_RELEASE, "agent");
        asm volatile("s_waitcnt vmcnt(0)" ::: "memory");
        __hip_atomic_fetch_add((gint*)counter, 1, __ATOMIC_RELAXED, __HIP_MEMORY_SCOPE_AGENT);
    }
}

typedef __attribute__((address_space(1))) unsigned long long gu64;
__device__ __forceinline__ unsigned long long ld8_agent(const void* p) {
    return __hip_atomic_load((gu64*)p, __ATOMIC_RELAXED, __HIP_MEMORY_SCOPE_AGENT);
}
__device__ __forceinline__ void st8_agent(void* p, unsigned long long v) {
    __hip_atomic_store((gu64*)p, v, __ATOMIC_RELAXED, __HIP_MEMORY_SCOPE_AGENT);
}

constexpr int HO_SHARDS = 8, HO_SHARD_STRIDE = 16;
constexpr int HO_CTR_INTS = HO_SHARDS * HO_SHARD_STRIDE;

__device__ __forceinline__ void publish_sc1(int* ctr, int idx) {
    asm volatile("s_waitcnt vmcnt(0)" ::: "memory");
    __syncthreads();
    if (threadIdx.x == 0)
        __hip_atomic_fetch_add((gint*)(ctr + (idx & (HO_SHARDS - 1)) * HO_SHARD_STRIDE), 1, __ATOMIC_RELAXED, __HIP_MEMORY_SCOPE_AGENT);
}

struct WaitSharded {
    int* ctr; int n; int* err; int naps; long long* tr;
    __device__ __forceinline__ void operator()() const {
        if (n <= 0) {
            if (tr && threadIdx.x == 0) tr[1] = (long long)__builtin_amdgcn_s_memrealtime();
            return;
        }
        if (threadIdx.x < HO_SHARDS) {
            const int k = threadIdx.x;
            const int need = (n - k + HO_SHARDS - 1) / HO_SHARDS;
            gint* gc = (gint*)(ctr + k * HO_SHARD_STRIDE);
            bool ok = false;
            for (int it = 0; it < (1 << 16); ++it) {
                ok = __hip_atomic_load(gc, __ATOMIC_RELAXED, __HIP_MEMORY_SCOPE_AGENT) >= need;
                if (__all(ok)) break;
                for (int z = 0; z < naps; ++z) __builtin_amdgcn_s_sleep(8);
            }
            if (!__all(ok) && threadIdx.x == 0) *err = 1;
            if (tr && threadIdx.x == 0) tr[1] = (long long)__builtin_amdgcn_s_memrealtime();
        }
        __syncthreads();
    }
};

}
```

### radialog_amd/csrc/rdx_ctx.h

```cpp
#pragma once
#include <hip/hip_runtime.h>
#include <stdarg.h>
#include <stdio.h>
#include <stdlib.h>
#include <string.h>

#include <algorithm>
#include <map>
#include <string>
#include <vector>

#include "../../include/rdx.h"
#include "rdx_common.h"
#include "rdx_kernels.h"

using namespace rdx;

constexpr int RDX_MAX_ROWS = 128;

struct GemmW { void* w = nullptr; int N = 0, K = 0, Npad = 0; void* w8 = nullptr; float* scale = nullptr; };
struct RawW { void* p = nullptr; int64_t rows = 0, cols = 0; };

struct LlamaLayer {
    const void *attn_norm, *mlp_norm, *lora_bq, *lora_bv;
    GemmW wqkv, wo, wgu, wdown;
};
struct QLayer {
    GemmW s_wqkv, s_wo, c_wq, c_wo, w1, w2;
    const float *s_bqkv, *s_bo, *s_g, *s_b, *c_bq, *c_bo, *c_g, *c_b, *b1, *b2, *f_g, *f_b;
    int cross_idx;
};
struct VBlock {
    GemmW c1, c2, c3, ds;
    const float *b1, *b2, *b3, *bds;
    bool has_ds;
    int planes, stride;
};

struct PoolBlock {
    const float *n1_g, *n1_b, *n2_g, *n2_b, *bo, *b1, *b2;
    GemmW wqkv, wo, w1, w2;
};

struct GraphKey {
    int B = -1, max_new = 0, eos = 0, pad = 0;
    const void* tokens = nullptr; const void* scores = nullptr;
    bool fixed = false;
    rdx_logits_rules rules = {1.0f, 0, 0};
    bool operator==(const GraphKey& o) const {
        return B == o.B && max_new == o.max_new && eos == o.eos && pad == o.pad && tokens == o.tokens && scores == o.scores && fixed == o.fixed &&
               rules.repetition_penalty == o.rules.repetition_penalty && rules.no_repeat_ngram_size == o.rules.no_repeat_ngram_size &&
               rules.min_new_tokens == o.rules.min_new_tokens;
    }
};

struct rdx_ctx {
    rdx_config cfg;
    int device = 0;
    hipStream_t stream = nullptr;
    std::string err;
    bool finalized = false;
    std::vector<void*> allocs;

    std::map<std::string, GemmW> gemm;
    std::map<std::string, RawW> tens;
    std::map<std::string, RawW> f32;

    std::vector<LlamaLayer> ll;
    const void *embed = nullptr, *final_norm = nullptr, *rope_cos = nullptr, *rope_sin = nullptr;
    GemmW lm_head, img_proj_w;
    const float* img_proj_b = nullptr;
    LlamaDims ld;
    void *kcache = nullptr, *vcache = nullptr;
    size_t kv_layer_elems = 0;
    uint8_t* key_mask = nullptr;
    int *d_img_pos = nullptr, *d_pos_ids = nullptr, *d_pos = nullptr, *d_slot = nullptr, *d_step = nullptr, *d_unf = nullptr;
    float* part_val = nullptr; int* part_idx = nullptr; int n_vtiles = 0;
    void *dx = nullptr, *dxn = nullptr, *dqkv = nullptr, *datt = nullptr, *dgu = nullptr;
    float* dxs = nullptr;
    void* pxq = nullptr; float* pxs = nullptr;
    std::string unsupported;
    float* kslab = nullptr;
    int pend_groups = 0;
    void *px = nullptr, *pxn = nullptr, *pqkv = nullptr, *pq = nullptr, *patt = nullptr, *pgu = nullptr, *pqe = nullptr, *pimg = nullptr;
    size_t prefill_rows = 0;
    float* pslab = nullptr;
    int cur_B = 0, cur_T = 0, cur_max_new = 0, cur_eos = -1, cur_pad = 0;
    int cur_steps = 0;
    int32_t* cur_tokens = nullptr;
    hipGraphExec_t graph = nullptr;
    bool fuse_attn_oproj = true;
    bool chain_mlp = true;
    bool xs16 = true;
    bool prompt_blk = true;
    bool blk_down = true;
    int chain_naps = 1;
    long long* chain_trace = nullptr; int chain_trace_layer = -1;
    GemmW cls_fc1, cls_fc2; const float *cls_fc1_b = nullptr, *cls_fc2_b = nullptr;
    void *cls_pooled = nullptr, *cls_h = nullptr, *cls_out = nullptr;
    void* zero16 = nullptr;
    void* d_cur_rope = nullptr;
    ChainLayer* d_clayers = nullptr; int* d_cctr = nullptr;
    int *d_ctr = nullptr, *d_err = nullptr;
    int flash_min = 512;
    bool pconv_noks = false;
    bool trunk_packed = true;
    bool ws_ok = false;
    float* gemm_ws = nullptr; size_t gemm_ws_floats = 0;
    GraphKey gkey;
    rdx_logits_rules rules = {1.0f, 0, 0};
    bool hist_ready = false;
    bool rules_on = false;
    int *d_hist = nullptr, *d_hist_len = nullptr;
    void* rule_logits = nullptr;

    void* bm_logits = nullptr; float* bm_scores = nullptr; float* bm_cand_s = nullptr; int* bm_cand_i = nullptr;
    int *bm_tok = nullptr, *bm_src = nullptr; int32_t* bm_out = nullptr; void* bm_scratch = nullptr;
    size_t bm_scratch_bytes = 0; int bm_rows = 0, bm_new = 0;

    void* tf_ws = nullptr; size_t tf_bytes = 0;

    void* comm = nullptr; int comm_rank = 0, comm_world = 0;

    std::vector<QLayer> ql;
    const void* q_query_ln = nullptr;
    GemmW q_wkv; const float* q_bkv = nullptr; int n_cross = 0;
    GemmW v_conv1, v_b2v, v_p1, v_p2;
    const float *v_conv1_b = nullptr, *v_p1_b = nullptr, *v_p2_b = nullptr, *v_ln_g = nullptr, *v_ln_b = nullptr;
    std::vector<VBlock> vb;
    std::vector<PoolBlock> pool;
    const void* pool_emb = nullptr;
    const float *pool_ng = nullptr, *pool_nb = nullptr, *v_p1f_b = nullptr;
    GemmW v_p1f;
    float pool_eps = 1e-6f;
    int enc_batch = 0;
    void *vin = nullptr, *vbuf[4] = {nullptr, nullptr, nullptr, nullptr}, *v_imgemb = nullptr;
    void *qx = nullptr, *qt = nullptr, *qqkv = nullptr, *qctx = nullptr, *qh = nullptr, *qkvx = nullptr;
};

int fail(rdx_ctx* c, int code, const char* fmt, ...);
const char* create_error();

#define HIPCHK(c, call)                                                                         \
    do {                                                                                        \
        hipError_t e_ = (call);                                                                 \
        if (e_ != hipSuccess) return fail((c), -2, "%s failed: %s (%s:%d)", #call, hipGetErrorString(e_), __FILE__, __LINE__); \
    } while (0)

inline size_t esz(const rdx_ctx* c) { (void)c; return 2; }

int dalloc(rdx_ctx* c, void** p, size_t bytes);
#define ALLOC(c, ptr, bytes) do { int rc_ = dalloc((c), (void**)&(ptr), (bytes)); if (rc_) return rc_; } while (0)

template <typename P>
inline void dfree(rdx_ctx* c, P*& p) {
    if (!p) return;
    auto it = std::find(c->allocs.begin(), c->allocs.end(), (void*)p);
    if (it != c->allocs.end()) c->allocs.erase(it);
    hipFree((void*)p);
    p = nullptr;
}

GemmArgs gargs(const void* X, int ldx, const GemmW& W, const float* bias, void* out, int ldo, int M);
GemmArgs skinny_prenorm(rdx_ctx* c, GemmArgs a, int epi);
void skinny(rdx_ctx* c, GemmArgs a, int epi);
void launch_ksplit(rdx_ctx* c, const GemmArgs& a);
enum DecUnit { UNIT_QKV, UNIT_O, UNIT_GATE_UP, UNIT_DOWN, UNIT_LM_HEAD };
enum DecFamily { DEC_UNSUPPORTED, DEC_CHAINED, DEC_GENERIC, DEC_XS16, DEC_BLK, DEC_BLK8 };
DecFamily decode_family(rdx_ctx* c, int B);
DecAttnArgs dec_attn_args(rdx_ctx* c, int layer);
AttnArgs prefill_attn_args(rdx_ctx* c, int B, int T, int keep, int layer);
GemmArgs unit_args(rdx_ctx* c, const LlamaLayer* L, DecUnit u, int B);
GemmArgs xs16_unit(rdx_ctx* c, const LlamaLayer* L, DecUnit u, int B);
GemmArgs blk_unit(rdx_ctx* c, const LlamaLayer* L, DecUnit u, int B);
GemmArgs blk8_unit(rdx_ctx* c, const LlamaLayer* L, DecUnit u, int B);
GemmArgs ksplit_args(GemmArgs a);
GemmArgs prenormed(rdx_ctx* c, GemmArgs a);
GemmArgs norm_in_front(rdx_ctx* c, GemmArgs a);
void run_rmsnorm(rdx_ctx* c, const NormArgs& n);
bool down_split_ok(rdx_ctx* c, const LlamaLayer& L, int B);
void launch_down(rdx_ctx* c, const LlamaLayer& L, int B, bool split);
bool blk64_ok(rdx_ctx* c, int B);
bool blk64_fp8(rdx_ctx* c);
bool xs16_ok(rdx_ctx* c, int B);
void run_gemm(rdx_ctx* c, GemmArgs a, int epi);
void conv_gemm(rdx_ctx* c, const void* X, const GemmW& W, const float* bias, const void* resid, void* out, int B,
               int Hin, int Win, int Cin, int KH, int KW, int stride, int pad, int Hout, int Wout, int epi);
int run_stem_pool(rdx_ctx* c, const void* vin, const GemmW& W, const float* bias, void* out, int B, int S, bool packed);
int v_grid(const rdx_config& f);
inline bool fp8_weights(const GemmW& W) { return W.w8 && W.scale && !W.w; }
int take_unsupported(rdx_ctx* c);

inline void* kv_ptr(rdx_ctx* c, void* base, int layer) { return (char*)base + (size_t)layer * c->kv_layer_elems * 2; }
int prefill_impl(rdx_ctx* c, const int32_t* ids, const int32_t* mask, int B, int T, const float* qformer_embs, int keep,
                 int max_new, int eos_id, int pad_id, int32_t* out_tokens, void* logits);
bool decode_step_launch(rdx_ctx* c, void* logits, const int* out_step, long step_stride, std::vector<hipEvent_t>* evs = nullptr);
int build_graph(rdx_ctx* c, void* scores, bool fixed = false);
```

### radialog_amd/csrc/rdx_kernels.h

```cpp
#pragma once
#include <hip/hip_runtime.h>
#include <stdint.h>

namespace rdx {

enum Epilogue {
    EPI_NONE = 0,
    EPI_RELU = 1,
    EPI_GELU = 2,
    EPI_RESID = 3,
    EPI_SILU_MUL = 4,
    EPI_LOGITS = 5,
    EPI_RESID_RELU = 6,
};

enum ActLayout : int {
    ACT_ROWS = 0,
    ACT_BLK32 = 1,
    ACT_BLK64 = 2,
    ACT_TILES32 = 3,
    ACT_BLK64_E4M3 = 4,
    ACT_ROWS_E4M3 = 5,
};

struct GemmArgs {
    const void* X; int ldx;
    const void* W;
    const float* bias;
    const void* resid; int ldr;
    void* out; int ldo;
    int M, N, K;
    const void* norm_w; float eps;
    float* part_val; int* part_idx;
    int n_valid;
    const int* out_step; long out_step_stride;
    const void* W8; const float* wscale;
    ActLayout out_packed;
    ActLayout xpacked;
    int mtiles;
    int xdup_off;
    const float* xscale; int xgroups;
    long long* trace;
};

struct ConvGeom {
    int mode;
    int Hin, Win, Cin, Hout, Wout, KH, KW, stride, pad;
};

struct PConvArgs {
    const void* X; const void* W; const float* bias; const void* resid; void* out;
    const void* zero16;
    int Hin, Win, Cin, Hout, Wout, N;
    int M;
    int mt_in, mt_out;
    int ldo;
    int clog;
    int no_ksplit;
    int tile_m, tile_n, tile_k;
};

struct AttnArgs {
    const void* Q; const void* K; const void* V; void* O;
    long q_bs, q_ts, q_hs;
    long k_bs, k_ts, k_hs;
    long v_bs, v_ts, v_hs;
    long o_bs, o_ts, o_hs;
    int B, H, Tq, Tk;
    int causal;
    int k_perm;
    const uint8_t* key_mask; long km_bs;
    int flash_min;
    int o_packed_mt;
};


struct LlamaDims {
    int hidden, heads, head_dim, qkv_ld, lora_r;
    float lora_scale;
    int max_len;
    int max_pos;
    int k_perm;
};

void launch_pack_weight(int dtype, const float* src, void* dst, int N, int K, int Npad, const int* rowmap, hipStream_t s);
void launch_pack_weight_fp8(int dtype, const float* src, void* dst8, float* scale, void* dst, int N, int K, int Npad, hipStream_t s);
bool skinny_fits_lds(int M, int K);
void launch_skinny_gemm(int dtype, const GemmArgs& a, int epi, hipStream_t s);
bool xstat32_supported(const GemmArgs& a, int epi);
void launch_xstat32(int dtype, const GemmArgs& a, int epi, hipStream_t s);
int xsplit32_groups(const GemmArgs& a);
void launch_xsplit32(int dtype, const GemmArgs& a, float* slab, hipStream_t s);
int xs_min_rows();
bool xstat_blk_supported(const GemmArgs& a, int epi);
void launch_xstat_blk(int dtype, const GemmArgs& a, int epi, hipStream_t s);
bool xs16_rows_ok(int M);
bool xstat16_supported(const GemmArgs& a, int epi);
void launch_xstat16(int dtype, const GemmArgs& a, int epi, hipStream_t s);
bool xrow16_supported(const GemmArgs& a);
void launch_xrow16(int dtype, const GemmArgs& a, hipStream_t s);
void launch_tiled_gemm(int dtype, const GemmArgs& a, const ConvGeom& cg, int epi, hipStream_t s);
bool gemm_dma_supported(const GemmArgs& a);
void launch_gemm_dma(int dtype, const GemmArgs& a, int epi, float* ws, size_t ws_floats, hipStream_t s);
bool gemm_dma_conv_supported(const GemmArgs& a, const ConvGeom& cg, int epi);
void launch_gemm_dma_conv(int dtype, const GemmArgs& a, const ConvGeom& cg, int epi, const void* zero16, float* ws, size_t ws_floats,
                          hipStream_t s);

bool conv1x1_stream_supported(const GemmArgs& a, const ConvGeom& cg, int epi);
void launch_conv1x1_stream(int dtype, const GemmArgs& a, const ConvGeom& cg, int epi, hipStream_t s);

bool wstat_supported(const GemmArgs& a, int epi);
void launch_wstat(int dtype, const GemmArgs& a, int epi, hipStream_t s);
bool xsplit_blk_supported(const GemmArgs& a);
void launch_xsplit_blk(int dtype, const GemmArgs& a, float* slab, hipStream_t s);
bool xstat_blk8_supported(const GemmArgs& a, int epi);
void launch_xstat_blk8(int dtype, const GemmArgs& a, int epi, hipStream_t s);
int xsplit_blk8_groups(const GemmArgs& a);
void launch_xsplit_blk8(int dtype, const GemmArgs& a, float* slab, hipStream_t s);
bool wsgemm_supported(const GemmArgs& a, const ConvGeom& cg, int epi);
void launch_wsgemm(int dtype, const GemmArgs& a, const ConvGeom& cg, int epi, const void* zero16, hipStream_t s);

bool pconv_supported(const PConvArgs& a, int taps, int stride, int epi);
bool launch_pconv(int dtype, PConvArgs a, int taps, int stride, int epi, bool rowout, hipStream_t s);
bool layernorm_packed_supported(int H);
void launch_layernorm_packed(int dtype, const void* x, const float* gamma, const float* beta, void* out, float* out_f32, int M, int H, float eps, hipStream_t s);
void launch_broadcast_packed(int dtype, const void* src, void* dst, int rows, int H, int B, hipStream_t s);
void launch_pack_rows(int dtype, const void* X, int ldx, void* P, int M, int C, hipStream_t s);
void launch_unpack_rows(int dtype, const void* P, void* X, int ldx, int M, int C, hipStream_t s);

bool stem_pool_supported(int stem_channels);
void launch_stem_pool(int dtype, const void* in, const void* Wp, const float* bias, void* out, int B, int Hp, int Hc, int Ho, int stem,
                      int packed_mt, hipStream_t s);

void launch_l2_bench(int mode, const void* buf, size_t bytes_per_wg, int shared, int reps, int wgs, unsigned* sink, hipStream_t s);

void launch_attention(int dtype, int head_dim, const AttnArgs& a, hipStream_t s);
bool flash_prefill_supported(int head_dim, const AttnArgs& a);
void launch_flash_prefill(int dtype, const AttnArgs& a, hipStream_t s);
void launch_rope_kv_prefill(int dtype, const LlamaDims& d, const void* qkv, const void* lora_bq, const void* lora_bv,
                            const void* cos_t, const void* sin_t, const int* pos_ids, void* qout, void* kcache,
                            void* vcache, int B, int T, int slot0, hipStream_t s);
void launch_k_unperm(const void* kc, void* out, size_t slabs, int max_len, int perm, hipStream_t s);
struct DecAttnArgs {
    LlamaDims d;
    const void *qkv, *lbq, *lbv, *cos_t, *sin_t;
    const void* cur_rope = nullptr;
    const int *pos, *slot_b;
    const uint8_t* key_mask;
    void *kcache, *vcache, *out;
    long long* trace = nullptr;
    ActLayout out_packed = ACT_ROWS;
    int out_mt = 2;
};
void launch_decode_attention(int dtype, const DecAttnArgs& a, int B, hipStream_t s);
struct ChainLayer { const void *wqkv, *wdown, *attn_norm;
                    const void *wqkv8, *wdown8; const float *sqkv, *sdown; };
struct ChainArgs {
    const ChainLayer* layers;
    int layer;
    int hidden, inter, qkv_n, qkv_ld, B;
    int w8;
    float eps;
    void *dx, *dqkv, *dgu;
    int* ctr;
    int* err;
    int naps;
    int nwg_down;
    long long* trace;
};
bool chain_supported(const LlamaDims& d, int inter, int B);
size_t chain_ctr_ints(int layers);
void launch_decode_chain(int dtype, ChainArgs ca, bool with_next_qkv, hipStream_t s);
bool attn_oproj16_supported(const LlamaDims& d, int N, int K, int B);
void launch_attn_oproj16(int dtype, const DecAttnArgs& a, const GemmArgs& g, int B, int* counter, int* err, hipStream_t s);

struct NormArgs {
    void* x; const void* w;
    void* out; float* xscale;
    int rows, H; float eps;
    ActLayout layout; int mtiles;
    const float* slab; int groups;
};
bool rmsnorm_supported(const NormArgs& n);
bool launch_rmsnorm(int dtype, const NormArgs& n, hipStream_t s);
void launch_quant_rows(int dtype, const void* x, long ldx, void* out8, float* xscale, int rows, int K, int groups, hipStream_t s);
bool gemm8_supported(const GemmArgs& a, int epi);
void launch_gemm8(int dtype, const GemmArgs& a, int epi, hipStream_t s);
void launch_layernorm(int dtype, const void* x, const float* gamma, const float* beta, void* out, float* out_f32,
                      int rows, int H, float eps, hipStream_t s);
void launch_layernorm_ex(int dtype, const void* x, long ldx, const float* gamma, const float* beta, const void* emb, int emb_rows,
                         void* out, long ldo, int rows, int H, float eps, hipStream_t s);
void launch_pool_gather(int dtype, const void* src, void* dst, int B, int L, int C, hipStream_t s);
void launch_pool_concat(int dtype, const void* patch, const void* tokens, void* dst, int B, int L, int C, hipStream_t s);
void launch_scramble_layernorm(int dtype, const void* pp_nhwc, const float* gamma, const float* beta, void* out,
                               float* out_f32, int B, int P, int C, float eps, hipStream_t s);
void launch_img_prep(int dtype, const float* img, void* out, int B, int S, int pad, int Hp, int Wp, hipStream_t s);
void launch_maxpool(int dtype, const void* in, void* out, int B, int H, int W, int C, hipStream_t s);
void launch_broadcast_rows(int dtype, const void* src, void* dst, int rows, int H, int B, hipStream_t s);
void launch_avgpool_flatten(int dtype, const void* in, void* out, int B, int G, int C, int pool, hipStream_t s);
void launch_to_f32(int dtype, const void* src, float* dst, size_t n, hipStream_t s);
void launch_from_f32(int dtype, const float* src, void* dst, size_t n, hipStream_t s);

void launch_prep_prompt(const int* ids, const int* mask_in, int B, int T, int img_id, int pad_id, int* img_pos,
                        int* pos_ids, uint8_t* key_mask, long km_bs, int* pos_next, int* slot_b, int* step_b,
                        int* unfinished, hipStream_t s);
void launch_prep_append(int B, int T_, int keep_len, int* img_pos, int* pos_ids, int* pos_next, int* slot_b, int* step_b,
                        int* unfinished, hipStream_t s);
void launch_embed_splice(int dtype, const int* ids, const int* img_pos, const void* embed, int vocab, const void* img_emb,
                         int n_img, void* out, int B, int T, int H, int use_img, hipStream_t s);
void launch_gather_last(int dtype, const void* x, void* out, int B, int T, int H, hipStream_t s);
struct StepTail {
    int eos_id, pad_id, max_new, vocab, H, n_zero, hist_ld;
    int *out_tokens, *unfinished, *pos, *slot_b, *step_b, *ctr_zero, *hist, *hist_len;
    const int* pos_ro;
    const void *embed, *cos_t, *sin_t;
    void *x_next, *cur_rope;
};
void launch_greedy_step(int dtype, const float* part_val, const int* part_idx, int n_tiles, int B, const StepTail& t, hipStream_t s);
struct SelectArgs {
    void* logits; long step_stride;
    const int* n_gen;
    float penalty; int ngram, min_new;
    int* sel_out;
};
inline size_t select_step_lds(int vocab) { return (size_t)2 * ((vocab + 31) / 32) * sizeof(unsigned); }
bool select_step_supported(int vocab);
void launch_select_step(int dtype, const SelectArgs& a, const StepTail& t, int B, hipStream_t s);
void launch_hist_init(const int* ids, int B, int T, int* hist, int* hist_len, int ld, hipStream_t s);
void launch_hist_set_last(const int* ids, int* hist, const int* hist_len, int ld, int B, hipStream_t s);

#define RDX_MAX_BEAMS 8
void launch_beam_topk(int dtype, const void* logits, const float* beam_scores, int groups, int beams, int vocab, float* cand_score,
                      int* cand_idx, void* logp_out, hipStream_t s);
void launch_kv_beam_reorder(void* kcache, void* vcache, void* scratch, const int* src, const int* start, int rows, int heads, int layers, int max_len,
                            size_t layer_bytes, int p0, int p1, hipStream_t s);
void launch_embed_rows(int dtype, const int* tokens, const void* embed, int vocab, void* x, int rows, int H, hipStream_t s);

}
```

Measured before the change: 1.524 reports/s.

## Replace counter handoff in fused attention+o_proj with epoch-tagged granules

The fused attention + o_proj kernel used to signal completion through per-layer counters that the step tail had to zero every decode step. Attention blocks now write their output as 8-byte granules that carry a 32-bit tag built from the step epoch and layer index. The o_proj tiles spin on the tagged data itself, with a hint array as a coarse pre-wait, so the separate publish and counter-reset traffic goes away. The cost is twice the bytes for the attention output, retry sweeps over that data, and a hang-or-error risk if tags collide or epochs drift.

```diff
diff --git a/include/rdx_hooks.h b/include/rdx_hooks.h
--- a/include/rdx_hooks.h
+++ b/include/rdx_hooks.h
@@ -7,6 +7,8 @@
 
 int rdx_attn_trace(rdx_ctx* ctx, int layer, long long* host);
 int rdx_quant_test(rdx_ctx* ctx, const void* X, int M, int K, int groups, int mode, const void* norm_w, float eps, void* out8, float* scales);
+#define RDX_TRACE_CHAIN 7
+#define RDX_TRACE_ATTN_OPROJ 8
 int rdx_gemv_trace(rdx_ctx* ctx, int what, int layer, long long* host, int max_tiles);
 
 int rdx_gemm_test(rdx_ctx* ctx, const void* X, const float* W, const float* bias, const void* resid, void* out, int M, int N,
diff --git a/radialog_amd/_lib.py b/radialog_amd/_lib.py
--- a/radialog_amd/_lib.py
+++ b/radialog_amd/_lib.py
@@ -93,6 +93,9 @@
     "rdx_logits_test": (C.c_int, [_P, _P, _P, C.c_int, C.c_int, C.c_int, C.c_int, _P, _P, C.c_int]),
 }
 
+TRACE_CHAIN = 7
+TRACE_ATTN_OPROJ = 8
+
 ENC_HOOK_SYMBOLS = {
     "rdx_stem_test": (C.c_int, [_P, _P, _P, _P, _P, C.c_int, C.c_int, C.c_int, C.c_int]),
     "rdx_norm_test": (C.c_int, [_P, C.c_int, _P, _P, _P, _P, _P, _P, C.c_int, C.c_int, C.c_longlong, C.c_longlong, C.c_int, C.c_int, C.c_float]),
diff --git a/radialog_amd/csrc/api.hip b/radialog_amd/csrc/api.hip
--- a/radialog_amd/csrc/api.hip
+++ b/radialog_amd/csrc/api.hip
@@ -238,9 +238,13 @@
         HIPCHK(c, hipMemset(c->key_mask, 0, (size_t)B * f.max_len));
         ALLOC(c, c->d_img_pos, B * sizeof(int)); ALLOC(c, c->d_pos, B * sizeof(int)); ALLOC(c, c->d_slot, B * sizeof(int));
         ALLOC(c, c->d_step, B * sizeof(int)); ALLOC(c, c->d_unf, B * sizeof(int));
-        ALLOC(c, c->d_ctr, ((size_t)f.layers * 256 + chain_ctr_ints(f.layers)) * sizeof(int)); ALLOC(c, c->d_err, sizeof(int));
-        HIPCHK(c, hipMemset(c->d_ctr, 0, ((size_t)f.layers * 256 + chain_ctr_ints(f.layers)) * sizeof(int)));
-        c->d_cctr = c->d_ctr + (size_t)f.layers * 256;
+        ALLOC(c, c->d_ctr, chain_ctr_ints(f.layers) * sizeof(int)); ALLOC(c, c->d_err, sizeof(int));
+        HIPCHK(c, hipMemset(c->d_ctr, 0, chain_ctr_ints(f.layers) * sizeof(int)));
+        c->d_cctr = c->d_ctr;
+        ALLOC(c, c->d_gran, (size_t)2 * H * 4 + HO_HINT_INTS * sizeof(int)); ALLOC(c, c->d_epoch, sizeof(int));
+        HIPCHK(c, hipMemset(c->d_gran, 0, (size_t)2 * H * 4 + HO_HINT_INTS * sizeof(int)));
+        HIPCHK(c, hipMemset(c->d_epoch, 0, sizeof(int)));
+        c->d_hint = reinterpret_cast<int*>(reinterpret_cast<char*>(c->d_gran) + (size_t)2 * H * 4);
         HIPCHK(c, hipMemset(c->d_err, 0, sizeof(int)));
         {
             std::vector<ChainLayer> cl(f.layers);
diff --git a/radialog_amd/csrc/api_debug.hip b/radialog_amd/csrc/api_debug.hip
--- a/radialog_amd/csrc/api_debug.hip
+++ b/radialog_amd/csrc/api_debug.hip
@@ -35,25 +35,31 @@
     HIPCHK(c, hipSetDevice(c->device));
     const rdx_config& f = c->cfg;
     const int H = f.hidden, B = c->cur_B;
-    if (what == 7) {
-        if (layer < 0 || layer >= f.layers) return fail(c, -1, "rdx_gemv_trace(7): layer %d of %d", layer, f.layers);
+    if (what == 7 || what == 8) {
+        if (layer < 0 || layer >= f.layers) return fail(c, -1, "rdx_gemv_trace(%d): layer %d of %d", what, layer, f.layers);
         if (c->cur_T + c->cur_steps + 1 > f.max_len || c->cur_T + c->cur_steps + 1 > f.max_pos)
-            return fail(c, -1, "rdx_gemv_trace(7): no room for one more decode step in the KV cache");
-        const int wgs = H / 16 + ((c->ll[0].wqkv.Npad + 15) / 16 + 3) / 4;
-        if (wgs > max_tiles) return fail(c, -1, "rdx_gemv_trace(7): need room for %d workgroups", wgs);
+            return fail(c, -1, "rdx_gemv_trace(%d): no room for one more decode step in the KV cache", what);
+        const bool fused = c->fuse_attn_oproj && attn_oproj16_supported(c->ld, c->ll[layer].wo.N, c->ll[layer].wo.K, B);
+        if (what == 8 && !fused)
+            return fail(c, -1, "rdx_gemv_trace(8): the fused attention + o_proj launch is not active in this configuration (batch > 2, RDX_FUSE_AO=0)");
+        const int wgs = what == 7 ? H / 16 + ((c->ll[0].wqkv.Npad + 15) / 16 + 3) / 4
+                                  : f.heads * B + ((c->ll[layer].wo.N + 15) / 16 + 1) / 2;
+        if (wgs > max_tiles) return fail(c, -1, "rdx_gemv_trace(%d): need room for %d workgroups", what, wgs);
         long long* dtr = nullptr;
         const size_t bytes = (size_t)max_tiles * 8 * sizeof(long long);
         HIPCHK(c, hipMalloc(&dtr, bytes));
         HIPCHK(c, hipMemsetAsync(dtr, 0, bytes, c->stream));
-        c->chain_trace = dtr; c->chain_trace_layer = layer;
+        if (what == 7) { c->chain_trace = dtr; c->chain_trace_layer = layer; }
+        else { c->ao_trace = dtr; c->ao_trace_layer = layer; }
         const bool chained = decode_step_launch(c, nullptr, nullptr, 0);
         c->chain_trace = nullptr; c->chain_trace_layer = -1;
+        c->ao_trace = nullptr; c->ao_trace_layer = -1;
         c->cur_steps = std::max(c->cur_steps + 1, c->cur_max_new);
         hipError_t e = hipStreamSynchronize(c->stream);
         if (e == hipSuccess) e = hipMemcpy(host, dtr, bytes, hipMemcpyDeviceToHost);
         hipFree(dtr);
         HIPCHK(c, e);
-        if (!chained) return fail(c, -1, "rdx_gemv_trace(7): the chained down -> QKV launch is not active in this configuration (batch > 2, RDX_CHAIN=0)");
+        if (what == 7 && !chained) return fail(c, -1, "rdx_gemv_trace(7): the chained down -> QKV launch is not active in this configuration (batch > 2, RDX_CHAIN=0)");
         return 0;
     }
     const LlamaLayer& L = c->ll[layer];
diff --git a/radialog_amd/csrc/api_llama.hip b/radialog_amd/csrc/api_llama.hip
--- a/radialog_amd/csrc/api_llama.hip
+++ b/radialog_amd/csrc/api_llama.hip
@@ -42,8 +42,9 @@
     t.pos = advance ? c->d_pos : nullptr; t.slot_b = advance ? c->d_slot : nullptr; t.step_b = c->d_step;
     t.embed = c->embed; t.vocab = f.vocab; t.x_next = c->dx; t.H = f.hidden; t.pos_ro = c->d_pos; t.cos_t = c->rope_cos; t.sin_t = c->rope_sin;
     t.cur_rope = c->d_cur_rope;
-    t.ctr_zero = (c->fuse_attn_oproj || c->chain_mlp) ? c->d_ctr : nullptr;
-    t.n_zero = f.layers * 256 + (c->chain_mlp ? (int)chain_ctr_ints(f.layers) : 0);
+    t.ctr_zero = c->chain_mlp ? c->d_ctr : nullptr;
+    t.n_zero = (int)chain_ctr_ints(f.layers);
+    t.epoch = c->d_epoch;
     if (!c->rules_on) { launch_greedy_step(f.dtype, c->part_val, c->part_idx, c->n_vtiles, B, t, c->stream); return; }
     t.hist = c->d_hist; t.hist_len = c->d_hist_len; t.hist_ld = f.max_len;
     SelectArgs sa;
@@ -269,7 +270,11 @@
     DecAttnArgs at = dec_attn_args(c, l);
     const GemmArgs ao = unit_args(c, &L, UNIT_O, B);
     if (c->fuse_attn_oproj && attn_oproj16_supported(c->ld, L.wo.N, L.wo.K, B)) {
-        launch_attn_oproj16(dt, at, ao, B, c->d_ctr + (size_t)l * 256, c->d_err, c->stream);
+        at.trace = l == c->ao_trace_layer ? c->ao_trace : nullptr;
+        at.out = c->d_gran; at.epoch = c->d_epoch; at.layers = c->cfg.layers; at.layer = l;
+        GemmArgs ag = ao;
+        ag.X = c->d_gran;
+        launch_attn_oproj16(dt, at, ag, B, c->d_hint, c->d_err, c->stream);
         return;
     }
     const GemmArgs ap = ksplit_args(ao);
diff --git a/radialog_amd/csrc/attn_body.h b/radialog_amd/csrc/attn_body.h
--- a/radialog_amd/csrc/attn_body.h
+++ b/radialog_amd/csrc/attn_body.h
@@ -26,7 +26,7 @@
 
 template <typename T, int WAVES, bool DED = (WAVES == 8), typename WaitFn = NoWait, bool V_EARLY_ = !DED, int KG_ = 0, bool COH = false>
 __device__ __forceinline__ void decode_attention_body(const DecAttnArgs& a, const int h, const int b, float* dsm,
-                                                      WaitFn wait_inputs = WaitFn()) {
+                                                      WaitFn wait_inputs = WaitFn(), const unsigned tag = 0u, int* hint = nullptr) {
     typedef typename Vec8<T>::type V8;
     constexpr int D = 128;
     constexpr int CW = DED ? WAVES - 1 : WAVES;
@@ -55,7 +55,10 @@
     T* vc = reinterpret_cast<T*>(a.vcache) + ((size_t)b * d.heads + h) * d.max_len * D;
     const uint8_t* km = a.key_mask + (size_t)b * d.max_len;
 
-    if (a.trace && h == 0 && b == 0 && tid == 0) a.trace[7] = (long long)__builtin_amdgcn_s_memrealtime();
+    long long* trc = !(a.trace && tid == 0) ? nullptr : COH ? a.trace + ((size_t)b * d.heads + h) * 8 : (h == 0 && b == 0) ? a.trace : nullptr;
+#define ATT_T(i) do { constexpr int ts_ = COH ? ((i) == 7 ? 0 : (i) == 2 ? 1 : (i) == 4 ? 2 : (i) == 5 ? 3 : (i) == 6 ? 4 : (i) == 8 ? 5 : -1) : ((i) < 8 ? (i) : -1); \
+                      if (ts_ >= 0 && trc) trc[ts_] = (long long)__builtin_amdgcn_s_memrealtime(); } while (0)
+    ATT_T(7);
     const int cw = DED ? w - 1 : w;
     const bool owns_rows = !DED || w > 0;
     u4 kr[KG][4], vr[VR];
@@ -110,8 +113,6 @@
     }
     const int slot = a.slot_b[b];
     const int nk = slot + 1;
-    long long* trc = (a.trace && h == 0 && b == 0 && tid == 0) ? a.trace : nullptr;
-#define ATT_T(i) do { if (trc) trc[i] = (long long)__builtin_amdgcn_s_memrealtime(); } while (0)
     ATT_T(0);
     wait_inputs();
     ATT_T(1);
@@ -217,6 +218,7 @@
     if (w == 0 && lane == 0) S[slot] = km_new ? rnd<T>(rnd<T>(s_new) / div) : -INFINITY;
     __syncthreads();
     ATT_T(4);
+    if (COH && tid == 0) store_hint(hint, 0, tag);
 
     float mx = -INFINITY;
     for (int j = lane; j < nk; j += 64) mx = fmaxf(mx, S[j]);
@@ -302,16 +304,17 @@
                            : a.out_packed != ACT_ROWS ? ((size_t)((pf * a.out_mt + (b >> 4)) * 64 + pg * 16 + (b & 15)) << 3) + (k & 7) : (size_t)b * H + k;
             reinterpret_cast<T*>(a.out)[o] = fromf<T>(v);
         }
-    } else if (tid < D / 4) {
-        unsigned long long pk = 0ull;
-#pragma unroll
-        for (int e = 0; e < 4; ++e) {
+    } else if (tid < D / 2) {
+        unsigned pk = 0u;
+#pragma unroll
+        for (int e = 0; e < 2; ++e) {
             float v = 0.f;
 #pragma unroll
-            for (int i = 0; i < WAVES; ++i) v += part[i * D + tid * 4 + e];
-            pk |= (unsigned long long)bits16<T>(fromf<T>(v)) << (16 * e);
-        }
-        st8_agent(reinterpret_cast<T*>(a.out) + (size_t)b * H + h * D + tid * 4, pk);
+            for (int i = 0; i < WAVES; ++i) v += part[i * D + tid * 2 + e];
+            pk |= (unsigned)bits16<T>(fromf<T>(v)) << (16 * e);
+        }
+        store_granule(a.out, (((size_t)b * H + h * D) >> 1) + tid, pk, tag);
+        ATT_T(8);
     }
 #undef ATT_T
 }
diff --git a/radialog_amd/csrc/chain.hip b/radialog_amd/csrc/chain.hip
--- a/radialog_amd/csrc/chain.hip
+++ b/radialog_amd/csrc/chain.hip
@@ -64,15 +64,21 @@
     }
 
     wait_inputs();
-    CH_T(3);
+    if (!WaitFn::TAGGED) CH_T(3);
 
     const int K4 = K >> 2, total4 = a.M * K4;
     unsigned long long xr[XL];
-#pragma unroll
-    for (int i = 0; i < XL; ++i) {
-        const int c = threadIdx.x + i * CH_THREADS;
-        xr[i] = 0ull;
-        if (c < total4) { const int m = c / K4, k4 = c - m * K4; xr[i] = ld8_agent(X + (size_t)m * a.ldx + (size_t)k4 * 4); }
+    if constexpr (WaitFn::TAGGED) {
+        wait_inputs.template sweep<XL>(xr, a.X, a.ldx, K4, total4, CH_THREADS);
+        if (trace) __syncthreads();
+        CH_T(3);
+    } else {
+#pragma unroll
+        for (int i = 0; i < XL; ++i) {
+            const int c = threadIdx.x + i * CH_THREADS;
+            xr[i] = 0ull;
+            if (c < total4) { const int m = c / K4, k4 = c - m * K4; xr[i] = ld8_agent(X + (size_t)m * a.ldx + (size_t)k4 * 4); }
+        }
     }
     if (NORM) {
         float ss[CH_MAXM];
@@ -246,14 +252,19 @@
 }
 
 template <typename T, bool W8>
-__global__ __launch_bounds__(CH_THREADS, 4) void attn_oproj16_k(DecAttnArgs at, ChainGemm g, int n_attn, int ntiles, int* counter, int* err) {
+__global__ __launch_bounds__(CH_THREADS, 4) void attn_oproj16_k(DecAttnArgs at, ChainGemm g, int n_attn, int ntiles, int* hint, int* err) {
     extern __shared__ __attribute__((aligned(16))) unsigned char msm[];
+    long long* trace = at.trace ? at.trace + (size_t)blockIdx.x * 8 : nullptr;
+    const unsigned tag = handoff_tag(*at.epoch, at.layers, at.layer);
     if ((int)blockIdx.x < n_attn) {
         const int b = blockIdx.x / at.d.heads, h = blockIdx.x - b * at.d.heads;
-        decode_attention_body<T, CH_WAVES, true, NoWait, true, 0, true>(at, h, b, reinterpret_cast<float*>(msm));
-        publish_sc1(counter, blockIdx.x);
+        decode_attention_body<T, CH_WAVES, true, NoWait, true, 0, true>(at, h, b, reinterpret_cast<float*>(msm), NoWait(), tag, hint + blockIdx.x);
+        if (trace && threadIdx.x == 0) {
+            asm volatile("s_waitcnt vmcnt(0)" ::: "memory");
+            trace[6] = (long long)__builtin_amdgcn_s_memrealtime();
+        }
     } else {
-        chain_tile<T, EPI_RESID, false, 2, 2, WaitSharded, W8 ? 4 : 8, true, W8>(g, blockIdx.x - n_attn, ntiles, msm, WaitSharded{counter, n_attn, err, 1, nullptr});
+        chain_tile<T, EPI_RESID, false, 2, 2, WaitTagged, W8 ? 4 : 8, true, W8>(g, blockIdx.x - n_attn, ntiles, msm, WaitTagged{hint, n_attn, tag, err}, trace);
     }
 }
 
@@ -263,7 +274,7 @@
            d.heads * B + (ntiles + 1) / 2 <= 256;
 }
 
-void launch_attn_oproj16(int dtype, const DecAttnArgs& a, const GemmArgs& ga, int B, int* counter, int* err, hipStream_t s) {
+void launch_attn_oproj16(int dtype, const DecAttnArgs& a, const GemmArgs& ga, int B, int* hint, int* err, hipStream_t s) {
     const int n_attn = a.d.heads * B, ntiles = (ga.N + 15) / 16;
     const bool w8 = ga.W8 && ga.wscale && ga.K % 64 == 0;
     ChainGemm g = {ga.X, ga.ldx, ga.W, ga.resid, ga.ldr, ga.out, ga.ldo, ga.M, ga.N, ga.K, nullptr, 0.f, ga.W8, ga.wscale};
@@ -272,8 +283,8 @@
     const size_t smem = sm_gemm > sm_att ? sm_gemm : sm_att;
     dim3 grid(n_attn + (ntiles + 1) / 2), block(CH_THREADS);
     RDX_DISPATCH_T(dtype, T, {
-        if (w8) hipLaunchKernelGGL((attn_oproj16_k<T, true>), grid, block, smem, s, a, g, n_attn, ntiles, counter, err);
-        else hipLaunchKernelGGL((attn_oproj16_k<T, false>), grid, block, smem, s, a, g, n_attn, ntiles, counter, err);
+        if (w8) hipLaunchKernelGGL((attn_oproj16_k<T, true>), grid, block, smem, s, a, g, n_attn, ntiles, hint, err);
+        else hipLaunchKernelGGL((attn_oproj16_k<T, false>), grid, block, smem, s, a, g, n_attn, ntiles, hint, err);
     });
 }
 
diff --git a/radialog_amd/csrc/elem.hip b/radialog_amd/csrc/elem.hip
--- a/radialog_amd/csrc/elem.hip
+++ b/radialog_amd/csrc/elem.hip
@@ -541,6 +541,7 @@
         }
         if (step < t.max_new) t.out_tokens[(size_t)b * t.max_new + step] = tok;
         t.step_b[b] = step + 1;
+        if (b == 0 && t.epoch) *reinterpret_cast<unsigned*>(t.epoch) += 1u;
         if (t.slot_b) t.slot_b[b] += 1;
         int pcur = t.pos_ro ? t.pos_ro[b] : 0;
         if (t.pos) { pcur = t.pos[b] + 1; t.pos[b] = pcur; }
diff --git a/radialog_amd/csrc/handoff.h b/radialog_amd/csrc/handoff.h
--- a/radialog_amd/csrc/handoff.h
+++ b/radialog_amd/csrc/handoff.h
@@ -5,9 +5,10 @@
 
 typedef __attribute__((address_space(1))) int gint;
 
-struct NoWait { __device__ __forceinline__ void operator()() const {} };
+struct NoWait { static constexpr bool TAGGED = false; __device__ __forceinline__ void operator()() const {} };
 
 struct WaitCounter {
+    static constexpr bool TAGGED = false;
     int* counter; int target; int* err;
     __device__ __forceinline__ void operator()() const {
         if (threadIdx.x == 0) {
@@ -53,6 +54,7 @@
 }
 
 struct WaitSharded {
+    static constexpr bool TAGGED = false;
     int* ctr; int n; int* err; int naps; long long* tr;
     __device__ __forceinline__ void operator()() const {
         if (n <= 0) {
@@ -76,4 +78,55 @@
     }
 };
 
+__device__ __forceinline__ unsigned handoff_tag(int epoch, int layers, int layer) {
+    const unsigned t = (unsigned)epoch * (unsigned)layers + (unsigned)layer + 1u;
+    return t ? t : 0x80000000u;
 }
+__device__ __forceinline__ void store_hint(int* hint, int idx, unsigned tag) {
+    __hip_atomic_store((gint*)(hint + idx), (int)tag, __ATOMIC_RELAXED, __HIP_MEMORY_SCOPE_AGENT);
+}
+__device__ __forceinline__ void store_granule(void* gran, size_t i, unsigned pair, unsigned tag) {
+    st8_agent(reinterpret_cast<unsigned long long*>(gran) + i, ((unsigned long long)tag << 32) | pair);
+}
+
+struct WaitTagged {
+    static constexpr bool TAGGED = true;
+    const int* hint; int n; unsigned tag; int* err;
+    __device__ __forceinline__ void operator()() const {
+        if (threadIdx.x < 64) {
+            for (int it = 0; it < (1 << 16); ++it) {
+                bool ok = true;
+                for (int i = threadIdx.x; i < n; i += 64)
+                    ok = ok && (unsigned)__hip_atomic_load((gint*)(hint + i), __ATOMIC_RELAXED, __HIP_MEMORY_SCOPE_AGENT) == tag;
+                if (__all(ok)) break;
+                __builtin_amdgcn_s_sleep(8);
+            }
+        }
+        __syncthreads();
+    }
+    template <int XL>
+    __device__ __forceinline__ void sweep(unsigned long long (&xr)[XL], const void* gran, int ld, int K4, int total4, int nthreads) const {
+        const unsigned long long* g = reinterpret_cast<const unsigned long long*>(gran);
+        bool ok = false;
+        for (int it = 0; it < (1 << 14); ++it) {
+            ok = true;
+#pragma unroll
+            for (int i = 0; i < XL; ++i) {
+                const int c = threadIdx.x + i * nthreads;
+                xr[i] = 0ull;
+                if (c < total4) {
+                    const int m = c / K4, k4 = c - m * K4;
+                    const unsigned long long* p = g + (((size_t)m * ld) >> 1) + (size_t)k4 * 2;
+                    const unsigned long long lo = ld8_agent(p), hi = ld8_agent(p + 1);
+                    ok = ok && (unsigned)(lo >> 32) == tag && (unsigned)(hi >> 32) == tag;
+                    xr[i] = (lo & 0xffffffffull) | (hi << 32);
+                }
+            }
+            if (__all(ok)) break;
+            __builtin_amdgcn_s_sleep(2);
+        }
+        if (!__all(ok) && (threadIdx.x & 63) == 0) *err = 1;
+    }
+};
+
+}
diff --git a/radialog_amd/csrc/rdx_ctx.h b/radialog_amd/csrc/rdx_ctx.h
--- a/radialog_amd/csrc/rdx_ctx.h
+++ b/radialog_amd/csrc/rdx_ctx.h
@@ -96,12 +96,14 @@
     bool blk_down = true;
     int chain_naps = 1;
     long long* chain_trace = nullptr; int chain_trace_layer = -1;
+    long long* ao_trace = nullptr; int ao_trace_layer = -1;
     GemmW cls_fc1, cls_fc2; const float *cls_fc1_b = nullptr, *cls_fc2_b = nullptr;
     void *cls_pooled = nullptr, *cls_h = nullptr, *cls_out = nullptr;
     void* zero16 = nullptr;
     void* d_cur_rope = nullptr;
     ChainLayer* d_clayers = nullptr; int* d_cctr = nullptr;
     int *d_ctr = nullptr, *d_err = nullptr;
+    void* d_gran = nullptr; int *d_hint = nullptr, *d_epoch = nullptr;
     int flash_min = 512;
     bool pconv_noks = false;
     bool trunk_packed = true;
diff --git a/radialog_amd/csrc/rdx_kernels.h b/radialog_amd/csrc/rdx_kernels.h
--- a/radialog_amd/csrc/rdx_kernels.h
+++ b/radialog_amd/csrc/rdx_kernels.h
@@ -151,6 +151,8 @@
     long long* trace = nullptr;
     ActLayout out_packed = ACT_ROWS;
     int out_mt = 2;
+    const int* epoch = nullptr;
+    int layers = 0, layer = 0;
 };
 void launch_decode_attention(int dtype, const DecAttnArgs& a, int B, hipStream_t s);
 struct ChainLayer { const void *wqkv, *wdown, *attn_norm;
@@ -171,8 +173,9 @@
 bool chain_supported(const LlamaDims& d, int inter, int B);
 size_t chain_ctr_ints(int layers);
 void launch_decode_chain(int dtype, ChainArgs ca, bool with_next_qkv, hipStream_t s);
+constexpr int HO_HINT_INTS = 128;
 bool attn_oproj16_supported(const LlamaDims& d, int N, int K, int B);
-void launch_attn_oproj16(int dtype, const DecAttnArgs& a, const GemmArgs& g, int B, int* counter, int* err, hipStream_t s);
+void launch_attn_oproj16(int dtype, const DecAttnArgs& a, const GemmArgs& g, int B, int* hint, int* err, hipStream_t s);
 
 struct NormArgs {
     void* x; const void* w;
@@ -211,7 +214,7 @@
 void launch_gather_last(int dtype, const void* x, void* out, int B, int T, int H, hipStream_t s);
 struct StepTail {
     int eos_id, pad_id, max_new, vocab, H, n_zero, hist_ld;
-    int *out_tokens, *unfinished, *pos, *slot_b, *step_b, *ctr_zero, *hist, *hist_len;
+    int *out_tokens, *unfinished, *pos, *slot_b, *step_b, *ctr_zero, *hist, *hist_len, *epoch;
     const int* pos_ro;
     const void *embed, *cos_t, *sin_t;
     void *x_next, *cur_rope;
```

Measured after the change: 1.546 reports/s, median of 6. 1.4% higher.
